# k-sheridan/ekf_vio

Hardware: AMD Instinct MI355X
Metric: filter steps/sec (predict+update) (higher is better)
Workload: dtype f32

## Files before the change

### ekf_vio_amd/capi.py

```python
import ctypes as C
import os

from . import _build

OK, EINVAL, ENUMERIC, ECAPACITY, EDEVICE, ESTATE, EABORTED = range(7)
_ERR = {EINVAL: "EKFVIO_EINVAL", ENUMERIC: "EKFVIO_ENUMERIC", ECAPACITY: "EKFVIO_ECAPACITY",
        EDEVICE: "EKFVIO_EDEVICE", ESTATE: "EKFVIO_ESTATE", EABORTED: "EKFVIO_EABORTED"}
PREDICT_STRUCTURED, PREDICT_DENSE = 0, 1


class Config(C.Structure):
    _fields_ = [("max_features", C.c_int32), ("default_point_depth", C.c_float),
                ("default_point_depth_variance", C.c_float), ("default_point_homogenous_variance", C.c_float),
                ("predict_mode", C.c_int32), ("klt_window_size", C.c_int32), ("klt_max_pyramid_level", C.c_int32),
                ("klt_max_iterations", C.c_int32), ("klt_epsilon", C.c_float), ("klt_min_eigen", C.c_float),
                ("kill_pad", C.c_int32), ("max_image_width", C.c_int32), ("max_image_height", C.c_int32),
                ("use_principal_point", C.c_int32), ("inverse_image_scale", C.c_int32), ("fast_threshold", C.c_int32),
                ("min_new_feature_dist", C.c_int32), ("fast_blur_sigma", C.c_float), ("replenish", C.c_int32),
                ("sample_based_uncertainty", C.c_int32), ("use_imu", C.c_int32), ("imu_gyro_variance", C.c_float),
                ("imu_accel_variance", C.c_float), ("gravity", C.c_float * 3),
                ("klt_fb_max_px", C.c_float), ("remove_lost", C.c_int32)]


class EkfvioError(RuntimeError):
    def __init__(self, code, msg=""):
        super().__init__("%s %s" % (_ERR.get(code, str(code)), msg))
        self.code = code


SYMBOLS = ["ekfvio_default_config", "ekfvio_create", "ekfvio_destroy", "ekfvio_reset", "ekfvio_last_error",
           "ekfvio_add_features", "ekfvio_process", "ekfvio_linearize", "ekfvio_update", "ekfvio_measurement_map",
           "ekfvio_num_features", "ekfvio_dim", "ekfvio_get_base_mu", "ekfvio_get_features", "ekfvio_get_sigma",
           "ekfvio_get_feature_cov", "ekfvio_get_depth_variance", "ekfvio_set_feature_cov", "ekfvio_metric2pixel_map",
           "ekfvio_pixel2metric_map", "ekfvio_get_odometry", "ekfvio_get_points", "ekfvio_check_sigma", "ekfvio_set_state",
           "ekfvio_remove_features", "ekfvio_klt_push_frame", "ekfvio_klt_track", "ekfvio_klt_track_points", "ekfvio_klt_get_level",
           "ekfvio_klt_uncertainty_points", "ekfvio_step_image", "ekfvio_replenish", "ekfvio_fast_detect", "ekfvio_imu", "ekfvio_imu_update",
           "ekfvio_upload_measurements", "ekfvio_run_uploaded", "ekfvio_synchronize", "ekfvio_profile_enable",
           "ekfvio_profile_reset", "ekfvio_profile_count", "ekfvio_profile_name", "ekfvio_profile_get",
           "ekfvio_profile_update_gemms", "ekfvio_get_counters", "ekfvio_set_gate", "ekfvio_get_gate",
           "ekfvio_set_klt_fb", "ekfvio_get_klt_fb", "ekfvio_klt_track_points_fb", "ekfvio_set_distortion", "ekfvio_rectify_map"]
HOOK_SYMBOLS = ["ekfvio_test_klt_padded_level", "ekfvio_test_blurred_level0", "ekfvio_test_gemm", "ekfvio_test_gemm_bench", "ekfvio_test_potrf_stamps",
                "ekfvio_test_sweep_stamps", "ekfvio_test_sweep_fault", "ekfvio_test_sweep_delay", "ekfvio_test_cholesky_solve", "ekfvio_test_plan", "ekfvio_test_persist_grid", "ekfvio_test_t2_pair"]

_libs = {}


def lib_path():
    return _build.LIB_PATH


def load(build_if_missing=True, hooks=False):
    if hooks in _libs:
        return _libs[hooks]
    path = _build.HOOKS_LIB_PATH if hooks else _build.LIB_PATH
    if build_if_missing:
        _build.build(hooks=hooks)
    elif not os.path.exists(path):
        raise FileNotFoundError(path + " not built; run python -m ekf_vio_amd._build")
    lib = C.CDLL(path)
    vp, i32, f32 = C.c_void_p, C.c_int32, C.c_float
    fp, u8p, ip = C.POINTER(C.c_float), C.POINTER(C.c_uint8), C.POINTER(C.c_int32)
    sig = {
        "ekfvio_default_config": [C.POINTER(Config)],
        "ekfvio_create": [C.POINTER(Config), C.c_int, vp, C.POINTER(vp)],
        "ekfvio_destroy": [vp], "ekfvio_reset": [vp],
        "ekfvio_add_features": [vp, fp, i32], "ekfvio_process": [vp, f32], "ekfvio_linearize": [vp, f32, fp],
        "ekfvio_update": [vp, fp, fp, u8p, i32], "ekfvio_measurement_map": [vp, u8p, i32, ip, ip],
        "ekfvio_num_features": [vp], "ekfvio_dim": [vp], "ekfvio_get_base_mu": [vp, fp],
        "ekfvio_get_features": [vp, fp, fp, u8p], "ekfvio_get_sigma": [vp, fp, i32],
        "ekfvio_get_feature_cov": [vp, i32, fp], "ekfvio_get_depth_variance": [vp, i32, fp],
        "ekfvio_set_feature_cov": [vp, i32, fp], "ekfvio_metric2pixel_map": [fp, fp], "ekfvio_pixel2metric_map": [fp, fp],
        "ekfvio_get_odometry": [vp, fp, fp, fp, fp], "ekfvio_get_points": [vp, fp, fp],
        "ekfvio_check_sigma": [vp, fp, fp], "ekfvio_set_state": [vp, i32, fp, fp, fp, u8p, fp, i32],
        "ekfvio_remove_features": [vp, u8p, i32, ip],
        "ekfvio_klt_push_frame": [vp, u8p, i32, i32, i32, fp], "ekfvio_klt_track": [vp, fp, fp, u8p],
        "ekfvio_klt_track_points": [vp, fp, fp, i32, fp, u8p],
        "ekfvio_klt_uncertainty_points": [vp, fp, fp, i32, fp],
        "ekfvio_klt_get_level": [vp, i32, ip, ip, u8p, C.POINTER(C.c_int16)],
        "ekfvio_step_image": [vp, C.c_double, u8p, i32, i32, i32, fp], "ekfvio_imu": [vp, C.c_double, fp, fp], "ekfvio_imu_update": [vp, fp, fp],
        "ekfvio_replenish": [vp, ip, ip], "ekfvio_fast_detect": [vp, i32, i32, i32, ip, ip, ip],
        "ekfvio_upload_measurements": [vp, i32, fp, fp, u8p], "ekfvio_run_uploaded": [vp, i32, i32, f32],
        "ekfvio_synchronize": [vp], "ekfvio_profile_enable": [vp, i32], "ekfvio_profile_reset": [vp],
        "ekfvio_profile_count": [], "ekfvio_profile_name": [i32],
        "ekfvio_profile_get": [vp, i32, C.POINTER(C.c_double), C.POINTER(C.c_int64), C.POINTER(C.c_double)],
        "ekfvio_profile_update_gemms": [vp, i32, C.POINTER(C.c_double), C.POINTER(C.c_double)],
        "ekfvio_get_counters": [vp, C.POINTER(C.c_int64)],
        "ekfvio_set_gate": [vp, f32], "ekfvio_get_gate": [vp, fp, u8p, ip, ip, C.POINTER(C.c_int64)],
        "ekfvio_set_klt_fb": [vp, f32], "ekfvio_get_klt_fb": [vp, fp, u8p, ip, ip, C.POINTER(C.c_int64)],
        "ekfvio_klt_track_points_fb": [vp, fp, fp, i32, fp, u8p, fp, fp, u8p],
        "ekfvio_set_distortion": [vp, C.POINTER(C.c_double), i32],
        "ekfvio_rectify_map": [fp, C.POINTER(C.c_double), i32, i32, i32, ip, ip],
    }
    if hooks:
        sig.update({
            "ekfvio_test_klt_padded_level": [vp, i32, ip, u8p, C.POINTER(C.c_int16)],
            "ekfvio_test_blurred_level0": [vp, u8p],
            "ekfvio_test_gemm": [vp, i32, i32, i32, i32, f32, fp, i32, fp, i32, f32, fp, i32, i32],
            "ekfvio_test_cholesky_solve": [vp, i32, i32, fp, fp, fp, fp, ip],
            "ekfvio_test_potrf_stamps": [vp, C.POINTER(C.c_int64)],
            "ekfvio_test_sweep_stamps": [vp, C.c_int, C.POINTER(C.c_int64)],
            "ekfvio_test_sweep_fault": [vp, i32, i32],
            "ekfvio_test_sweep_delay": [vp, i32, i32, i32],
            "ekfvio_test_gemm_bench": [vp, i32, i32, i32, i32, i32, i32, i32, C.POINTER(C.c_double)],
            "ekfvio_test_plan": [i32] * 8 + [f32, ip],
            "ekfvio_test_persist_grid": [i32] * 8 + [f32, ip, i32, ip],
            "ekfvio_test_t2_pair": [i32, ip],
        })
    for name, args in sig.items():
        fn = getattr(lib, name)
        fn.argtypes = args
        fn.restype = C.c_int
    lib.ekfvio_last_error.argtypes = [vp]
    lib.ekfvio_last_error.restype = C.c_char_p
    lib.ekfvio_profile_name.restype = C.c_char_p
    _libs[hooks] = lib
    return lib
```

### ekf_vio_amd/csrc/api.hip

```cpp
#include <math.h>
#include <stdio.h>
#include <string.h>

#include <algorithm>
#include <atomic>
#include <chrono>

#include <unistd.h>

#include "common.h"

#define HIPC(f, expr)                                                                              \
    do {                                                                                           \
        hipError_t e__ = (expr);                                                                   \
        if (e__ != hipSuccess) {                                                                   \
            (f)->last_error = std::string(#expr) + ": " + hipGetErrorString(e__);                  \
            return EKFVIO_EDEVICE;                                                                 \
        }                                                                                          \
    } while (0)

namespace {
template <class T>
hipError_t dev_alloc(hipStream_t s, T** p, size_t count) {
    hipError_t e = hipMalloc((void**)p, sizeof(T) * (count ? count : 1));
// ... 138 lines not shown
    c->imu_accel_variance = 1e-2f;
    c->gravity[0] = 0.f;
    c->gravity[1] = 9.81f;
    c->gravity[2] = 0.f;
    c->klt_fb_max_px = 0.f;
    c->remove_lost = 0;
    return EKFVIO_OK;
}

static int create_body(ekfvio_filter* f, const ekfvio_config* cfg, int device, void* stream) {
    HIPC(f, hipSetDevice(device));
    if (stream) {
        f->stream = (hipStream_t)stream;
    } else {
        HIPC(f, hipStreamCreateWithFlags(&f->stream, hipStreamNonBlocking));
        f->own_stream = true;
    }
    const int maxf = cfg->max_features;
    const FilterDims dims = filter_dims(maxf);
    f->n_cap = dims.n_cap, f->ldp = dims.ldp, f->m_cap = dims.m_cap, f->ld_aug = dims.ld_aug, f->sweep_sync_words = dims.sweep_sync_words;
    f->tune = tuning_from_env();
    const size_t pp = (size_t)f->ldp * f->ldp, pm = (size_t)f->ldp * f->m_cap;
    HIPC(f, dev_alloc(f->stream, &f->mu, f->ldp));
    HIPC(f, dev_alloc(f->stream, &f->mu_next, f->ldp));
    HIPC(f, dev_alloc(f->stream, &f->last_klt, 2 * (size_t)maxf));
    HIPC(f, dev_alloc(f->stream, &f->del_flag, (size_t)maxf));
    HIPC(f, dev_alloc(f->stream, &f->P, pp));
    HIPC(f, dev_alloc(f->stream, &f->P2, pp));
    HIPC(f, dev_alloc(f->stream, &f->FA, EKF_BASE * EKF_BASE));
    HIPC(f, dev_alloc(f->stream, &f->FB, 27 * (size_t)maxf));
    HIPC(f, dev_alloc(f->stream, &f->FD, 9 * (size_t)maxf));
    HIPC(f, dev_alloc(f->stream, &f->Fdense, pp));
    HIPC(f, dev_alloc(f->stream, &f->idx, (size_t)f->m_cap));
    HIPC(f, dev_alloc(f->stream, &f->inv_idx, (size_t)f->ldp));
    HIPC(f, dev_alloc(f->stream, &f->zmeas, 2 * (size_t)maxf));
    HIPC(f, dev_alloc(f->stream, &f->Rmeas, 4 * (size_t)maxf));
    HIPC(f, dev_alloc(f->stream, &f->pass, (size_t)maxf));
    HIPC(f, dev_alloc(f->stream, &f->yres, (size_t)f->m_cap));
    HIPC(f, dev_alloc(f->stream, &f->Rm, 2 * (size_t)f->m_cap));
    HIPC(f, dev_alloc(f->stream, &f->Saug, (size_t)f->ld_aug * f->m_cap));
    HIPC(f, dev_alloc(f->stream, &f->Laug, (size_t)f->ld_aug * f->m_cap));
    HIPC(f, dev_alloc(f->stream, &f->Linv, 64 * (size_t)f->m_cap));
    HIPC(f, dev_alloc(f->stream, &f->Lsign, (size_t)(f->m_cap / 64 > 256 ? f->m_cap / 64 : 256)));
    HIPC(f, dev_alloc(f->stream, &f->sweep_sync, f->sweep_sync_words));
    {
        hipDeviceProp_t prop;
        HIPC(f, hipGetDeviceProperties(&prop, device));
        f->num_cus = prop.multiProcessorCount;
    }
    HIPC(f, dev_alloc(f->stream, &f->Km, pm));
    HIPC(f, dev_alloc(f->stream, &f->Wt, pm));
    HIPC(f, dev_alloc(f->stream, &f->Gm, pm));
    HIPC(f, dev_alloc(f->stream, &f->info, 4));
    HIPC(f, dev_alloc(f->stream, &f->remove_words, 4));
    HIPC(f, hipHostMalloc((void**)&f->h_info, 16 * sizeof(int), hipHostMallocMapped | hipHostMallocCoherent));
    memset(f->h_info, 0, 16 * sizeof(int));
    HIPC(f, hipHostGetDevicePointer((void**)&f->d_hinfo, f->h_info, 0));
    {
        const size_t words = EKF_BASE + 4 * (size_t)(f->cfg.max_features > 0 ? f->cfg.max_features : 1);
        HIPC(f, hipHostMalloc((void**)&f->h_out, words * sizeof(float), hipHostMallocMapped | hipHostMallocCoherent));
        HIPC(f, hipHostGetDevicePointer((void**)&f->d_out, f->h_out, 0));
    }
    {
        const size_t cap = (size_t)(f->cfg.max_features > 0 ? f->cfg.max_features : 1);
        HIPC(f, hipHostMalloc((void**)&f->h_meas, 25 * cap, hipHostMallocDefault));
        HIPC(f, hipMalloc((void**)&f->d_meas, 25 * cap));
    }
    HIPC(f, hipEventCreate(&f->ev0));
    HIPC(f, hipEventCreate(&f->ev1));
    int rc = klt_alloc(f);
    if (rc != EKFVIO_OK) return rc;
    rc = fast_alloc(f);
    if (rc != EKFVIO_OK) return rc;
    return ekfvio_reset(f);
}

}

static std::atomic<int>* live_registry() {
    static std::atomic<int>* reg = [] {
        char name[64], val[32];
        snprintf(name, sizeof(name), "EKFVIO_LIVE_HANDLES_%ld", (long)getpid());
        if (const char* e = getenv(name)) {
            void* p = nullptr;
            if (sscanf(e, "%p", &p) == 1 && p) return static_cast<std::atomic<int>*>(p);
        }
        auto* a = new std::atomic<int>[64];
        for (int i = 0; i < 64; i++) a[i].store(0, std::memory_order_relaxed);
        snprintf(val, sizeof(val), "%p", static_cast<void*>(a));
        setenv(name, val, 1);
        return a;
    }();
    return reg;
}
int live_handles_on(int device) { return (device >= 0 && device < 64) ? live_registry()[device].load(std::memory_order_relaxed) : 2; }

extern "C" {

int ekfvio_create(const ekfvio_config* cfg, int device, void* stream, ekfvio_filter** out) {
    if (!out) return EKFVIO_EINVAL;
    *out = nullptr;
    if (!cfg || cfg->max_features < 0) return EKFVIO_EINVAL;
    if (cfg->remove_lost != 0 && cfg->remove_lost != 1) return EKFVIO_EINVAL;
    if (cfg->remove_lost && (size_t)cfg->max_features * 17 > 64 * 1024) return EKFVIO_ECAPACITY;
    if (!(cfg->klt_fb_max_px >= 0.f)) return EKFVIO_EINVAL;
    int ndev = 0;
    if (hipGetDeviceCount(&ndev) != hipSuccess || device < 0 || device >= ndev) return EKFVIO_EDEVICE;
    ekfvio_filter* f = new ekfvio_filter();
    f->cfg = *cfg;
    f->device = device;
    if (device < 64) live_registry()[device].fetch_add(1, std::memory_order_relaxed);
    const int rc = create_body(f, cfg, device, stream);
    if (rc != EKFVIO_OK) {
        fprintf(stderr, "ekfvio_create: %s\n", f->last_error.c_str());
        (void)ekfvio_destroy(f);
        return rc;
    }
    *out = f;
    return EKFVIO_OK;
}

int ekfvio_destroy(ekfvio_filter* f) {
    if (!f) return EKFVIO_EINVAL;
    (void)hipSetDevice(f->device);
    if (f->stream) (void)hipStreamSynchronize(f->stream);
    void* ptrs[] = {f->mu, f->mu_next, f->last_klt, f->del_flag, f->P,  f->P2, f->FA, f->FB, f->FD,   f->Fdense,
                    f->idx, f->inv_idx, f->zmeas,  f->Rmeas,    f->pass,     f->yres, f->Rm, f->Saug,  f->Laug,  f->Linv, f->Lsign, f->Km, f->sweep_sync, f->sweep_dbg,
                    f->Wt,  f->Gm,     f->info,     f->remove_words, f->seq_z,    f->seq_R, f->seq_pass, f->gate_words, f->fb_words};
    for (void* p : ptrs)
        if (p) hipFree(p);
    if (f->h_info) hipHostFree(f->h_info);
    if (f->h_out) hipHostFree(f->h_out);
    if (f->h_meas) hipHostFree(f->h_meas);
    if (f->d_meas) (void)hipFree(f->d_meas);
    klt_free(f);
    fast_free(f);
    drop_graph(f);
    if (f->ev0) hipEventDestroy(f->ev0);
    if (f->ev1) hipEventDestroy(f->ev1);
    if (f->own_stream && f->stream) hipStreamDestroy(f->stream);
    if (f->device >= 0 && f->device < 64) live_registry()[f->device].fetch_sub(1, std::memory_order_relaxed);
    delete f;
    return EKFVIO_OK;
}

const char* ekfvio_last_error(const ekfvio_filter* f) {
    return f ? f->last_error.c_str() : "null handle (a failed ekfvio_create leaves none behind: its return code says why)";
}

int ekfvio_reset(ekfvio_filter* f) {
    if (!f) return EKFVIO_EINVAL;
    f->out_fresh = false;
    HIPC(f, hipSetDevice(f->device));
    f->N = 0;
    f->n = EKF_BASE;
    HIPC(f, hipMemsetAsync(f->P, 0, sizeof(float) * (size_t)f->ldp * f->ldp, f->stream));
    HIPC(f, hipMemsetAsync(f->P2, 0, sizeof(float) * (size_t)f->ldp * f->ldp, f->stream));
    HIPC(f, hipMemsetAsync(f->mu, 0, sizeof(float) * f->ldp, f->stream));
    const float one = 1.f;
    HIPC(f, hipMemcpyAsync(f->mu + 3, &one, sizeof(float), hipMemcpyHostToDevice, f->stream));
    hipLaunchKernelGGL(init_sigma_kernel, dim3(1), dim3(32), 0, f->stream, f->P, f->ldp);
    HIPC(f, hipMemsetAsync(f->info, 0, 4 * sizeof(int), f->stream));
    if (f->gate_words) HIPC(f, hipMemsetAsync(f->gate_words, 0, 4 * sizeof(int), f->stream));
    if (f->fb_words) HIPC(f, hipMemsetAsync(f->fb_words, 0, 8 * sizeof(int), f->stream));
    HIPC(f, hipStreamSynchronize(f->stream));
    f->have_stamp = false;
    f->frames[0].valid = f->frames[1].valid = false;
    return EKFVIO_OK;
}

int ekfvio_add_features(ekfvio_filter* f, const float* uv, int32_t count) {
    if (!f || count < 0 || (count > 0 && !uv)) return EKFVIO_EINVAL;
    f->out_fresh = false;
    if (count == 0) return EKFVIO_OK;
    if (f->N + count > f->cfg.max_features) return EKFVIO_ECAPACITY;
    HIPC(f, hipSetDevice(f->device));
    HIPC(f, hipMemcpyAsync(f->zmeas, uv, sizeof(float) * 2 * count, hipMemcpyHostToDevice, f->stream));
    return add_features_device(f, count);
}

int ekfvio_process(ekfvio_filter* f, float dt) {
// ... 270 lines not shown

int ekfvio_upload_measurements(ekfvio_filter* f, int32_t frames, const float* z, const float* R, const uint8_t* pass) {
    if (!f || frames <= 0 || !z || !R || !pass || f->N <= 0) return EKFVIO_EINVAL;
    HIPC(f, hipSetDevice(f->device));
    HIPC(f, hipStreamSynchronize(f->stream));
    drop_graph(f);
    if (f->seq_z) hipFree(f->seq_z);
    if (f->seq_R) hipFree(f->seq_R);
    if (f->seq_pass) hipFree(f->seq_pass);
    f->seq_z = f->seq_R = nullptr;
    f->seq_pass = nullptr;
    const size_t N = f->N;
    HIPC(f, dev_alloc(f->stream, &f->seq_z, frames * 2 * N));
    HIPC(f, dev_alloc(f->stream, &f->seq_R, frames * 4 * N));
    HIPC(f, dev_alloc(f->stream, &f->seq_pass, frames * N));
    HIPC(f, hipMemcpyAsync(f->seq_z, z, sizeof(float) * frames * 2 * N, hipMemcpyHostToDevice, f->stream));
    HIPC(f, hipMemcpyAsync(f->seq_R, R, sizeof(float) * frames * 4 * N, hipMemcpyHostToDevice, f->stream));
    HIPC(f, hipMemcpyAsync(f->seq_pass, pass, frames * N, hipMemcpyHostToDevice, f->stream));
    HIPC(f, hipStreamSynchronize(f->stream));
    f->seq_frames = frames;
    f->seq_N = (int)N;
    f->seq_m.resize(frames);
    for (int i = 0; i < frames; i++) f->seq_m[i] = count_rows(pass + (size_t)i * N, (int)N);
    return EKFVIO_OK;
}

#ifndef EKF_GRAPH_STEPS
#define EKF_GRAPH_STEPS 8
#endif
#define EKF_GRAPH_STEPS_BIG 32

static void drop_graph(ekfvio_filter* f) {
    if (f->step_graph) {
        (void)hipGraphExecDestroy(f->step_graph);
        f->step_graph = nullptr;
    }
    if (f->step_graph_big) {
        (void)hipGraphExecDestroy(f->step_graph_big);
        f->step_graph_big = nullptr;
    }
    if (f->step_graph_pair) {
        (void)hipGraphExecDestroy(f->step_graph_pair);
        f->step_graph_pair = nullptr;
    }
}

static UpdateInputs uploaded_update(ekfvio_filter* f, int m, int i, int* counter) {
    UpdateInputs in;
    in.m = m, in.z = f->seq_z + (size_t)i * 2 * f->N, in.R = f->seq_R + (size_t)i * 4 * f->N, in.pass = f->seq_pass + (size_t)i * f->N;
    in.frame_counter = counter, in.frames = counter ? f->seq_frames : 0;
    in.recoverable = false;
    return in;
}
static int capture_steps(ekfvio_filter* f, int steps, int m, float dt, int* counter, hipGraphExec_t* out, int* pre_out) {
    hipGraph_t g = nullptr;
    HIPC(f, hipStreamSynchronize(f->stream));
    const bool mirror = f->sweep_flags_clean;
    f->sweep_flags_clean = false;
    const long long pre0 = f->prelinearized_steps;
    HIPC(f, hipStreamBeginCapture(f->stream, hipStreamCaptureModeThreadLocal));
    const bool gate = f->gate_chi2 > 0.f;
    for (int k = 0; k < steps; k++) {
        const BookArgs bk = make_book_args(f, m, f->seq_z, f->seq_R, f->seq_pass, counter);
        launch_predict(f, dt, gate ? nullptr : &bk);
        UpdateInputs in = uploaded_update(f, m, 0, counter);
        in.bookkeeping_done = !gate;
        in.next_dt = (k + 1 < steps) ? dt : -1.f;
        launch_update(f, in);
    }
    f->prelinearized = false;
    *pre_out = (int)(f->prelinearized_steps - pre0);
    f->prelinearized_steps = pre0;
    hipError_t ce = hipStreamEndCapture(f->stream, &g);
    f->graph_leaves_flags_clean = f->sweep_flags_clean;
    f->sweep_flags_clean = mirror;
    if (ce != hipSuccess || !g) {
        f->last_error = std::string("graph capture: ") + hipGetErrorString(ce);
        return EKFVIO_EDEVICE;
    }
    HIPC(f, hipGraphInstantiate(out, g, nullptr, nullptr, 0));
    (void)hipGraphDestroy(g);
    return EKFVIO_OK;
}

int ekfvio_run_uploaded(ekfvio_filter* f, int32_t first, int32_t count, float dt) {
    if (!f || f->seq_frames <= 0 || f->seq_N != f->N || count < 0 || first < 0 || !(dt >= 0.f)) return EKFVIO_EINVAL;
    f->out_fresh = false;
    HIPC(f, hipSetDevice(f->device));
    int s = 0;
    const bool gate = f->gate_chi2 > 0.f;
    auto geometry = [&](int i) { return gate && f->seq_m[i] > 0 ? 2 * f->N : f->seq_m[i]; };
    bool uniform = !f->prof_on && (count >= 2 || count == 0);
    for (int i = 0; uniform && i < f->seq_frames; i++) uniform = geometry(i) == geometry(0);
    if (uniform) {
        const int m = geometry(0);
        int* counter = f->info + 1;
        HIPC(f, hipMemsetD32Async((hipDeviceptr_t)counter, first % f->seq_frames, 1, f->stream));
        if (!f->step_graph || f->graph_N != f->N || f->graph_m != m || f->graph_dt != dt || f->graph_mu != f->mu || f->graph_P != f->P ||
            f->graph_seq != f->seq_z || f->graph_frames != f->seq_frames || f->graph_sole != (live_handles_on(f->device) <= 1)) {
            drop_graph(f);
            int rc = capture_steps(f, EKF_GRAPH_STEPS, m, dt, counter, &f->step_graph, &f->graph_pre);
            if (rc != EKFVIO_OK) return rc;
            rc = capture_steps(f, 2, m, dt, counter, &f->step_graph_pair, &f->graph_pre_pair);
            if (rc != EKFVIO_OK) return rc;
            f->graph_N = f->N; f->graph_m = m; f->graph_dt = dt; f->graph_mu = f->mu; f->graph_P = f->P; f->graph_seq = f->seq_z;
            f->graph_frames = f->seq_frames;
            f->graph_sole = live_handles_on(f->device) <= 1;
        }
        if (f->seq_frames >= 2 * EKF_GRAPH_STEPS_BIG && !f->step_graph_big) {
            int rc = capture_steps(f, EKF_GRAPH_STEPS_BIG, m, dt, counter, &f->step_graph_big, &f->graph_pre_big);
            if (rc != EKFVIO_OK) return rc;
        }
        auto replay = [&](hipGraphExec_t g, int steps, int pre) {
            const hipError_t e = hipGraphLaunch(g, f->stream);
            if (e == hipSuccess) s += steps, f->graph_steps += steps, f->prelinearized_steps += pre;
            return e;
        };
        if (f->step_graph_big)
            while (s + EKF_GRAPH_STEPS_BIG <= count) HIPC(f, replay(f->step_graph_big, EKF_GRAPH_STEPS_BIG, f->graph_pre_big));
        while (s + EKF_GRAPH_STEPS <= count) HIPC(f, replay(f->step_graph, EKF_GRAPH_STEPS, f->graph_pre));
        while (s + 2 <= count) HIPC(f, replay(f->step_graph_pair, 2, f->graph_pre_pair));
        if (s > 0) f->sweep_flags_clean = f->graph_leaves_flags_clean;
        for (; s < count; s++) {
            launch_predict(f, dt);
            launch_update(f, uploaded_update(f, m, 0, counter));
        }
        HIPC(f, hipGetLastError());
        return EKFVIO_OK;
    }
    for (; s < count; s++) {
        const int i = (first + s) % f->seq_frames;
        launch_predict(f, dt);
        launch_update(f, uploaded_update(f, f->seq_m[i], i, nullptr));
    }
    HIPC(f, hipGetLastError());
    return EKFVIO_OK;
}

int ekfvio_synchronize(ekfvio_filter* f) {
    if (!f) return EKFVIO_EINVAL;
    HIPC(f, hipSetDevice(f->device));
    return finish_update(f);
}

int ekfvio_profile_enable(ekfvio_filter* f, int32_t on) {
    if (!f) return EKFVIO_EINVAL;
    hipStreamSynchronize(f->stream);
    f->prof_on = on != 0;
    if (f->prof_on) {
        double acc = 0;
        const int reps = 32;
        for (int i = 0; i < reps + 4; i++) {
            (void)hipEventRecord(f->ev0, f->stream);
            (void)hipEventRecord(f->ev1, f->stream);
            (void)hipEventSynchronize(f->ev1);
            float ms = 0;
            (void)hipEventElapsedTime(&ms, f->ev0, f->ev1);
            if (i >= 4) acc += ms;
        }
        f->prof_overhead_ms = (float)(acc / reps);
    }
    return EKFVIO_OK;
}
int ekfvio_profile_update_gemms(ekfvio_filter* f, int32_t reps, double* avg_launch_us, double* flops_per_launch) {
    if (!f || reps <= 0 || !avg_launch_us) return EKFVIO_EINVAL;
    if (f->last_m <= 0 || f->N <= 0) return EKFVIO_ESTATE;
    HIPC(f, hipSetDevice(f->device));
    HIPC(f, hipStreamSynchronize(f->stream));
    hipGraph_t g = nullptr;
    hipGraphExec_t ge = nullptr;
    HIPC(f, hipStreamBeginCapture(f->stream, hipStreamCaptureModeThreadLocal));
    const int per_rep = launch_update_gemms_scratch(f, plan_update(f, f->last_m), reps);
    hipError_t ce = hipStreamEndCapture(f->stream, &g);
    if (ce != hipSuccess || !g) {
        f->last_error = std::string("graph capture: ") + hipGetErrorString(ce);
        return EKFVIO_EDEVICE;
    }
    HIPC(f, hipGraphInstantiate(&ge, g, nullptr, nullptr, 0));
    (void)hipGraphDestroy(g);
    HIPC(f, hipGraphLaunch(ge, f->stream));
    HIPC(f, hipEventRecord(f->ev0, f->stream));
    HIPC(f, hipGraphLaunch(ge, f->stream));
    HIPC(f, hipEventRecord(f->ev1, f->stream));
    HIPC(f, hipEventSynchronize(f->ev1));
    float ms = 0;
    HIPC(f, hipEventElapsedTime(&ms, f->ev0, f->ev1));
// ... 49 lines not shown
    int w[4] = {0, 0, 0, 0};
    if (f->gate_words) {
        HIPC(f, hipMemcpyAsync(w, f->gate_words, sizeof(w), hipMemcpyDeviceToHost, f->stream));
        HIPC(f, hipStreamSynchronize(f->stream));
    }
    const int seen = std::min(std::max(w[1], 0), f->cfg.max_features);
    if (seen > 0) {
        if (d2) HIPC(f, hipMemcpyAsync(d2, f->gate_d2, sizeof(float) * seen, hipMemcpyDeviceToHost, f->stream));
        if (gated) HIPC(f, hipMemcpyAsync(gated, f->gate_flag, seen, hipMemcpyDeviceToHost, f->stream));
        HIPC(f, hipStreamSynchronize(f->stream));
    }
    if (n_landmarks) *n_landmarks = seen;
    if (gated_last) *gated_last = w[0];
    if (gated_total) memcpy(gated_total, w + 2, sizeof(int64_t));
    return EKFVIO_OK;
}

int ekfvio_set_klt_fb(ekfvio_filter* f, float max_px) {
    if (!f || !(max_px >= 0.f)) return EKFVIO_EINVAL;
    f->cfg.klt_fb_max_px = max_px;
    return EKFVIO_OK;
}

int ekfvio_get_klt_fb(ekfvio_filter* f, float* err2, uint8_t* rejected, int32_t* n_landmarks, int32_t* rejected_last, int64_t* rejected_total) {
    if (!f) return EKFVIO_EINVAL;
    HIPC(f, hipSetDevice(f->device));
    int w[4] = {0, 0, 0, 0};
    if (f->fb_words) {
        HIPC(f, hipMemcpyAsync(w, f->fb_words, sizeof(w), hipMemcpyDeviceToHost, f->stream));
        HIPC(f, hipStreamSynchronize(f->stream));
    }
    const int seen = std::min(std::max(w[1], 0), f->cfg.max_features);
    if (seen > 0) {
        if (err2) HIPC(f, hipMemcpyAsync(err2, f->fb_err2, sizeof(float) * seen, hipMemcpyDeviceToHost, f->stream));
        if (rejected) HIPC(f, hipMemcpyAsync(rejected, f->fb_flag, seen, hipMemcpyDeviceToHost, f->stream));
        HIPC(f, hipStreamSynchronize(f->stream));
    }
    if (n_landmarks) *n_landmarks = seen;
    if (rejected_last) *rejected_last = w[0];
    if (rejected_total) memcpy(rejected_total, w + 2, sizeof(int64_t));
    return EKFVIO_OK;
}

int ekfvio_get_counters(ekfvio_filter* f, int64_t counters[8]) {
    if (!f || !counters) return EKFVIO_EINVAL;
    counters[0] = f->persistent_sweeps;
    counters[1] = f->schur_sweeps;
    counters[2] = f->sweep_recoveries;
    counters[3] = (f->tune.persist_sweep && !f->sweep_latched_off) ? 2 : 0;
    counters[4] = f->early_output_frames;
    counters[5] = f->t2_updates;
    counters[6] = f->graph_steps;
    counters[7] = f->prelinearized_steps;
    return EKFVIO_OK;
}

#ifdef EKFVIO_TEST_HOOKS
int ekfvio_test_gemm(ekfvio_filter* f, int32_t transB, int32_t M, int32_t N, int32_t K, float alpha, const float* A,
                     int32_t lda, const float* B, int32_t ldb, float beta, float* C, int32_t ldc, int32_t variant) {
    if (!f || M <= 0 || N <= 0 || K <= 0 || !A || !B || !C) return EKFVIO_EINVAL;
    HIPC(f, hipSetDevice(f->device));
    const int Mp = round_up(M, 64), Np = round_up(N, 64), Kp = round_up(K, 64);
    const int brows = transB ? Np : Kp, bcols = transB ? Kp : Np;
    std::vector<float> hA((size_t)Mp * Kp, 0.f), hB((size_t)brows * bcols, 0.f), hC((size_t)Mp * Np, 0.f);
    for (int k = 0; k < K; k++)
        for (int i = 0; i < M; i++) hA[(size_t)k * Mp + i] = A[(size_t)k * lda + i];
    for (int c = 0; c < (transB ? K : N); c++)
        for (int r = 0; r < (transB ? N : K); r++) hB[(size_t)c * brows + r] = B[(size_t)c * ldb + r];
    for (int j = 0; j < N; j++)
        for (int i = 0; i < M; i++) hC[(size_t)j * Mp + i] = C[(size_t)j * ldc + i];
    float *dA, *dB, *dC;
    HIPC(f, dev_alloc(f->stream, &dA, hA.size()));
    HIPC(f, dev_alloc(f->stream, &dB, hB.size()));
    HIPC(f, dev_alloc(f->stream, &dC, hC.size()));
    HIPC(f, hipMemcpyAsync(dA, hA.data(), sizeof(float) * hA.size(), hipMemcpyHostToDevice, f->stream));
    HIPC(f, hipMemcpyAsync(dB, hB.data(), sizeof(float) * hB.size(), hipMemcpyHostToDevice, f->stream));
    HIPC(f, hipMemcpyAsync(dC, hC.data(), sizeof(float) * hC.size(), hipMemcpyHostToDevice, f->stream));
    launch_gemm_variant(f, variant, transB, M, N, Kp, alpha, dA, Mp, dB, brows, beta, dC, Mp, dC, Mp, 0, 0);
    HIPC(f, hipMemcpyAsync(hC.data(), dC, sizeof(float) * hC.size(), hipMemcpyDeviceToHost, f->stream));
    HIPC(f, hipStreamSynchronize(f->stream));
    for (int j = 0; j < N; j++)
        for (int i = 0; i < M; i++) C[(size_t)j * ldc + i] = hC[(size_t)j * Mp + i];
    hipFree(dA);
    hipFree(dB);
    hipFree(dC);
    return EKFVIO_OK;
}

int ekfvio_test_gemm_bench(ekfvio_filter* f, int32_t transB, int32_t lowerB, int32_t M, int32_t N, int32_t K,
                           int32_t reps, int32_t variant, double* mean_us) {
    if (!f || M <= 0 || N <= 0 || K <= 0 || reps <= 0 || !mean_us) return EKFVIO_EINVAL;
    HIPC(f, hipSetDevice(f->device));
    const int Mp = round_up(M, 128), Np = round_up(N, 128), Kp = round_up(K, 64);
    const int brows = transB ? Np : Kp, bcols = transB ? Kp : Np;
    std::vector<float> hA((size_t)Mp * Kp), hB((size_t)brows * bcols), hC((size_t)Mp * Np);
    uint32_t st = 12345u;
    auto rnd = [&]() { st = st * 1664525u + 1013904223u; return ((st >> 8) & 0xffff) / 32768.0f - 1.0f; };
    for (auto& v : hA) v = rnd();
    for (auto& v : hB) v = rnd();
    for (auto& v : hC) v = rnd();
    float *dA, *dB, *dC;
    HIPC(f, dev_alloc(f->stream, &dA, hA.size()));
    HIPC(f, dev_alloc(f->stream, &dB, hB.size()));
    HIPC(f, dev_alloc(f->stream, &dC, hC.size()));
    HIPC(f, hipMemcpyAsync(dA, hA.data(), sizeof(float) * hA.size(), hipMemcpyHostToDevice, f->stream));
    HIPC(f, hipMemcpyAsync(dB, hB.data(), sizeof(float) * hB.size(), hipMemcpyHostToDevice, f->stream));
// ... 111 lines not shown
    UpdatePlan plan = plan_raw_sweep(f->tune, plan_shape(f), mp, rp);
    launch_chol_sweep(f, plan, dS, dL, dLi, ld, plan.persistent() && !f->sweep_flags_clean);
    if (plan.persistent()) f->sweep_flags_clean = false;
    std::vector<unsigned long long> hsign(mp / 64);
    HIPC(f, hipMemcpyAsync(hsign.data(), f->Lsign, sizeof(unsigned long long) * hsign.size(), hipMemcpyDeviceToHost, f->stream));
    HIPC(f, hipStreamSynchronize(f->stream));
    int refine = 1;
    for (unsigned long long v : hsign) refine &= (v == 0ull);
    if (refine) plan.gain = GAIN_GEMM;
    launch_gain_from_sweep(f, plan, dL, ld, nrhs, dK, dW, rp, refine);
    std::vector<float> hl(hs.size()), hk((size_t)rp * mp);
    HIPC(f, hipMemcpyAsync(hl.data(), dL, sizeof(float) * hl.size(), hipMemcpyDeviceToHost, f->stream));
    HIPC(f, hipMemcpyAsync(hk.data(), dK, sizeof(float) * hk.size(), hipMemcpyDeviceToHost, f->stream));
    if (info) {
        HIPC(f, hipMemcpyAsync(info, f->info, sizeof(int), hipMemcpyDeviceToHost, f->stream));
        HIPC(f, hipMemsetAsync(f->info, 0, sizeof(int), f->stream));
    }
    HIPC(f, hipStreamSynchronize(f->stream));
    if (const char* dp = getenv("EKFVIO_DEBUG_DUMP_LAUG")) {
        if (FILE* fp = fopen(dp, "wb")) {
            const int hdr[3] = {ld, mp, rp};
            fwrite(hdr, sizeof(int), 3, fp);
            fwrite(hl.data(), sizeof(float), hl.size(), fp);
            fclose(fp);
        }
    }
    if (L_out)
        for (int c = 0; c < m; c++)
            for (int r = 0; r < m; r++) L_out[(size_t)c * m + r] = (r >= c) ? hl[(size_t)c * ld + r] : 0.f;
    if (X_out)
        for (int c = 0; c < m; c++)
            for (int r = 0; r < nrhs; r++) X_out[(size_t)c * nrhs + r] = hk[(size_t)c * rp + r];
    hipFree(dS);
    hipFree(dL);
    hipFree(dLi);
    hipFree(dK);
    hipFree(dW);
    return EKFVIO_OK;
}

int ekfvio_test_plan(int32_t num_cus, int32_t max_features, int32_t N, int32_t m, int32_t m_on_device, int32_t sole_handle,
                     int32_t latched_off, int32_t dense_predict, float next_dt, int32_t plan[12]) {
    if (!plan || max_features < 0 || N < 0 || N > max_features) return EKFVIO_EINVAL;
    const FilterDims d = filter_dims(max_features);
    PlanShape s;
    s.num_cus = num_cus, s.ldp = d.ldp, s.sweep_sync_words = d.sweep_sync_words, s.N = N, s.n = EKF_BASE + 3 * N;
    s.dense_predict = dense_predict != 0, s.sole_handle = sole_handle != 0, s.latched_off = latched_off != 0;
    const UpdatePlan p = plan_update(tuning_from_env(), s, m, m_on_device != 0, next_dt);
    const int32_t out[12] = {p.m, p.m_pad, p.n_pad, p.sweep, p.fused_gather, p.with_wt, p.gain, p.tail, p.t2_skip, p.t2_by_sweep, p.compact, p.lin_blocks};
    std::copy(out, out + 12, plan);
    return EKFVIO_OK;
}

int ekfvio_test_persist_grid(int32_t num_cus, int32_t max_features, int32_t N, int32_t m, int32_t m_on_device, int32_t sole_handle,
                             int32_t latched_off, int32_t dense_predict, float next_dt, int32_t* roles, int32_t max_blocks, int32_t out[10]) {
    if (!out || max_features < 0 || N < 0 || N > max_features) return EKFVIO_EINVAL;
    const FilterDims d = filter_dims(max_features);
    PlanShape s;
    s.num_cus = num_cus, s.ldp = d.ldp, s.sweep_sync_words = d.sweep_sync_words, s.N = N, s.n = EKF_BASE + 3 * N;
    s.dense_predict = dense_predict != 0, s.sole_handle = sole_handle != 0, s.latched_off = latched_off != 0;
    const UpdatePlan p = plan_update(tuning_from_env(), s, m, m_on_device != 0, next_dt);
    std::fill(out, out + 10, 0);
    if (!p.persistent()) return EKFVIO_OK;
    const PersistGrid g = persist_grid(p, d.ldp);
    const PersistFlags fl(p.m_pad, p.n_pad);
    const int32_t res[10] = {g.total(), g.kind, g.owners(), fl.ready(), fl.fin(), fl.pan(), fl.abort_word(), (int32_t)fl.words(), fl.zero_words(),
                             (int32_t)d.sweep_sync_words};
    std::copy(res, res + 10, out);
    if (!roles) return EKFVIO_OK;
    if (max_blocks < g.total()) return EKFVIO_ECAPACITY;
    for (int b = 0; b < g.total(); b++) {
        const PersistRole r = g.role(b);
        roles[4 * b] = r.kind, roles[4 * b + 1] = r.a, roles[4 * b + 2] = r.b;
        roles[4 * b + 3] = r.kind == ROLE_OWNER ? g.owner_block(r.n) : -1;
    }
    return EKFVIO_OK;
}
int ekfvio_test_t2_pair(int32_t p, int32_t pair[2]) {
    if (p < 0 || !pair) return EKFVIO_EINVAL;
    int ta, tb;
    t2_pair(p, ta, tb);
    pair[0] = ta, pair[1] = tb;
    return EKFVIO_OK;
}
#endif

}
```

### ekf_vio_amd/csrc/chol.hip

```cpp
#include "common.h"

#include <type_traits>

namespace {

typedef float f32x16 __attribute__((ext_vector_type(16)));
typedef float f32x4 __attribute__((ext_vector_type(4)));

#define PB 64
#ifndef PLD
#define PLD 68
#endif
#define ILD 17
#define INV_LDS (4 * 16 * ILD)

__device__ __forceinline__ float lane_bcast(float v, int src_lane) {
    return __int_as_float(__builtin_amdgcn_readlane(__float_as_int(v), src_lane));
}
__device__ __forceinline__ double lane_bcast_d(double v, int src_lane) {
    const int lo = __builtin_amdgcn_readlane(__double2loint(v), src_lane);
    const int hi = __builtin_amdgcn_readlane(__double2hiint(v), src_lane);
    return __hiloint2double(hi, lo);
}

template <int B, int E, class F>
__device__ __forceinline__ void static_for(F&& f) {
    if constexpr (B < E) {
        f(std::integral_constant<int, B>{});
        static_for<B + 1, E>(f);
    }
}
template <int R>
__device__ __forceinline__ void dpp_fnma(float& acc, float a, float b) {
    asm volatile("v_fmac_f32_dpp %0, -%1, %2 row_newbcast:%3 row_mask:0xf bank_mask:0xf" : "+v"(acc) : "v"(a), "v"(b), "n"(R));
}
template <int R>
__device__ __forceinline__ float dpp_mul(float a, float b) {
    float r;
    asm volatile("s_nop 1\n\tv_mul_f32_dpp %0, %1, %2 row_newbcast:%3 row_mask:0xf bank_mask:0xf" : "=v"(r) : "v"(a), "v"(b), "n"(R));
    return r;
}

__device__ __forceinline__ void load_tile(float* T, const float* __restrict__ G, int ld, int tid) {
#pragma unroll
    for (int it = 0; it < 4; it++) {
        const int e = tid + it * 256;
        const int c = e >> 4, r4 = (e & 15) * 4;
        const float4 v = *reinterpret_cast<const float4*>(G + (size_t)c * ld + r4);
        float* t = T + c * PLD + r4;
#if PLD % 4 == 0
        *reinterpret_cast<float4*>(t) = v;
#else
        t[0] = v.x; t[1] = v.y; t[2] = v.z; t[3] = v.w;
#endif
    }
}
__device__ __forceinline__ void store_tile(const float* T, float* __restrict__ G, int ld, int tid) {
#pragma unroll
    for (int it = 0; it < 4; it++) {
        const int e = tid + it * 256;
        const int c = e >> 4, r4 = (e & 15) * 4;
        const float* t = T + c * PLD + r4;
#if PLD % 4 == 0
        *reinterpret_cast<float4*>(G + (size_t)c * ld + r4) = *reinterpret_cast<const float4*>(t);
#else
        *reinterpret_cast<float4*>(G + (size_t)c * ld + r4) = make_float4(t[0], t[1], t[2], t[3]);
#endif
    }
}
__device__ __forceinline__ unsigned long long sign_mask_request(const unsigned long long* p) {
    unsigned z;
    asm volatile("v_mov_b32 %0, 0" : "=v"(z));
    return p[z];
}
__device__ __forceinline__ unsigned long long sign_mask_value(unsigned long long v) {
    const unsigned lo = __builtin_amdgcn_readfirstlane((unsigned)v), hi = __builtin_amdgcn_readfirstlane((unsigned)(v >> 32));
    return ((unsigned long long)hi << 32) | lo;
}
__device__ __forceinline__ void store_tile_signed(const float* T, float* __restrict__ G, int ld, int tid, unsigned long long neg) {
#pragma unroll
    for (int it = 0; it < 4; it++) {
        const int e = tid + it * 256;
        const int c = e >> 4, r4 = (e & 15) * 4;
        const float* t = T + c * PLD + r4;
        const float sg = ((neg >> c) & 1ull) ? -1.f : 1.f;
        *reinterpret_cast<float4*>(G + (size_t)c * ld + r4) = make_float4(sg * t[0], sg * t[1], sg * t[2], sg * t[3]);
    }
}
__device__ __forceinline__ void store_tile_lower(const float* T, float* __restrict__ G, int ld, int tid) {
#pragma unroll
    for (int it = 0; it < 4; it++) {
        const int e = tid + it * 256;
        const int c = e >> 4, r4 = (e & 15) * 4;
        const float* t = T + c * PLD + r4;
#if PLD % 4 == 0
        const float4 q = *reinterpret_cast<const float4*>(t);
        *reinterpret_cast<float4*>(G + (size_t)c * ld + r4) =
            make_float4(r4 >= c ? q.x : 0.f, r4 + 1 >= c ? q.y : 0.f, r4 + 2 >= c ? q.z : 0.f, r4 + 3 >= c ? q.w : 0.f);
#else
        *reinterpret_cast<float4*>(G + (size_t)c * ld + r4) =
            make_float4(r4 >= c ? t[0] : 0.f, r4 + 1 >= c ? t[1] : 0.f, r4 + 2 >= c ? t[2] : 0.f, r4 + 3 >= c ? t[3] : 0.f);
#endif
    }
}
template <int C0, int NC, int NT, bool LOWER>
__device__ __forceinline__ void store_cols(const float* T, float* __restrict__ G, int ld, int t) {
    static_assert(PLD % 4 == 0, "vector LDS reads");
#pragma unroll
    for (int it = 0; it < (NC * 16 + NT - 1) / NT; it++) {
        const int e = t + it * NT;
        if ((NC * 16) % NT != 0 && e >= NC * 16) break;
        const int c = C0 + (e >> 4), r4 = (e & 15) * 4;
        const float4 q = *reinterpret_cast<const float4*>(T + c * PLD + r4);
        *reinterpret_cast<float4*>(G + (size_t)c * ld + r4) =
            LOWER ? make_float4(r4 >= c ? q.x : 0.f, r4 + 1 >= c ? q.y : 0.f, r4 + 2 >= c ? q.z : 0.f, r4 + 3 >= c ? q.w : 0.f) : q;
    }
}
__device__ __forceinline__ void store_inv_blocks(const float* Tinv, float* __restrict__ G, int p0, int t) {
    const int p = p0 + (t >> 6), c = (t >> 2) & 15, r4 = (t & 3) * 4;
    const float* s = Tinv + p * 16 * ILD + c * ILD + r4;
    *reinterpret_cast<float4*>(G + (p0 * 64 + t) * 4) = make_float4(s[0], s[1], s[2], s[3]);
}
struct NoIdleWork {
    template <class PC>
    __device__ __forceinline__ void operator()(PC, int) const {}
};
__device__ __forceinline__ void load_inv(float* Tinv, const float* __restrict__ G, int tid) {
    const float4 v = *reinterpret_cast<const float4*>(G + tid * 4);
    const int p = tid >> 6, c = (tid >> 2) & 15, r4 = (tid & 3) * 4;
    float* t = Tinv + p * 16 * ILD + c * ILD + r4;
    t[0] = v.x; t[1] = v.y; t[2] = v.z; t[3] = v.w;
}
__device__ __forceinline__ void store_inv(const float* Tinv, float* __restrict__ G, int tid) {
    const int p = tid >> 6, c = (tid >> 2) & 15, r4 = (tid & 3) * 4;
    const float* t = Tinv + p * 16 * ILD + c * ILD + r4;
    *reinterpret_cast<float4*>(G + tid * 4) = make_float4(t[0], t[1], t[2], t[3]);
}

__device__ __forceinline__ f32x16 mma64(const float* As, int a_si, int a_sq, const float* Bs, int b_sj, int b_sq, int wr, int wc,
                               int lane) {
    f32x16 acc;
#pragma unroll
    for (int r = 0; r < 16; r++) acc[r] = 0.f;
    const int li = lane & 31, lk = lane >> 5;
    const float* ap = As + (wr * 32 + li) * a_si + lk * a_sq;
    const float* bp = Bs + (wc * 32 + li) * b_sj + lk * b_sq;
#pragma unroll
    for (int q = 0; q < PB; q += 2) {
        const float a = ap[q * a_sq];
        const float b = bp[q * b_sq];
        acc = __builtin_amdgcn_mfma_f32_32x32x2f32(b, a, acc, 0, 0, 0);
    }
    return acc;
}
__device__ __forceinline__ int mma64_col(int wc, int lane, int reg) { return wc * 32 + (reg & 3) + 8 * (reg >> 2) + 4 * (lane >> 5); }
__device__ __attribute__((noinline)) f32x16 mma64_signed(const float* As, int a_si, int a_sq, const float* Bs, int b_sj, int b_sq, int wr,
                                                         int wc, int lane, unsigned long long neg) {
    f32x16 acc;
#pragma unroll
    for (int r = 0; r < 16; r++) acc[r] = 0.f;
    const int li = lane & 31, lk = lane >> 5;
    const float* ap = As + (wr * 32 + li) * a_si + lk * a_sq;
    const float* bp = Bs + (wc * 32 + li) * b_sj + lk * b_sq;
#pragma unroll 8
    for (int q = 0; q < PB; q += 2) {
        float a = ap[q * a_sq];
        if ((neg >> (q + lk)) & 1ull) a = -a;
        const float b = bp[q * b_sq];
        acc = __builtin_amdgcn_mfma_f32_32x32x2f32(b, a, acc, 0, 0, 0);
    }
    return acc;
}

__device__ __forceinline__ f32x4 mma16(const float* As, int a_si, int a_sq, const float* Bs, int b_sj, int b_sq, int lane) {
    f32x4 acc = {0.f, 0.f, 0.f, 0.f};
    const int li = lane & 15, lk = lane >> 4;
    const float* ap = As + li * a_si + lk * a_sq;
    const float* bp = Bs + li * b_sj + lk * b_sq;
#pragma unroll
    for (int q = 0; q < 16; q += 4) acc = __builtin_amdgcn_mfma_f32_16x16x4f32(bp[q * b_sq], ap[q * a_sq], acc, 0, 0, 0);
    return acc;
}

struct TriOps {
    float binv[4][4];
    float nl[6][4];
};
__device__ __forceinline__ void tri_solve_preload(TriOps& o, const float* Tl, const float* Tinv, int lane) {
    const int li = lane & 15, g = lane >> 4;
#pragma unroll
    for (int p = 0; p < 4; p++)
#pragma unroll
        for (int v = 0; v < 4; v++) o.binv[p][v] = Tinv[p * 16 * ILD + (4 * g + v) * ILD + li];
    {
        int e = 0;
#pragma unroll
        for (int p = 0; p < 3; p++)
#pragma unroll
            for (int t = p + 1; t < 4; t++, e++)
#pragma unroll
                for (int v = 0; v < 4; v++) o.nl[e][v] = -Tl[(16 * p + 4 * g + v) * PLD + 16 * t + li];
    }
}
__device__ __forceinline__ void tri_solve_pin(TriOps& o) {
#pragma unroll
    for (int p = 0; p < 4; p++)
#pragma unroll
        for (int v = 0; v < 4; v++) asm volatile("" : "+v"(o.binv[p][v]));
#pragma unroll
    for (int q = 0; q < 6; q++)
#pragma unroll
        for (int v = 0; v < 4; v++) asm volatile("" : "+v"(o.nl[q][v]));
}
template <int NT>
__device__ __forceinline__ void tri_solve_load_x(f32x4 (&x)[NT][4], float* const (&Txs)[NT], int wave, int lane) {
    const int r0 = 16 * wave, li = lane & 15, g = lane >> 4;
#pragma unroll
    for (int n = 0; n < NT; n++)
#pragma unroll
        for (int b = 0; b < 4; b++)
#pragma unroll
            for (int v = 0; v < 4; v++) x[n][b][v] = Txs[n][(16 * b + 4 * g + v) * PLD + r0 + li];
}
template <int NT>
__device__ __forceinline__ void tri_solve_run(f32x4 (&x)[NT][4], float* const (&Txs)[NT], const TriOps& o, int wave, int lane) {
    const int r0 = 16 * wave, li = lane & 15, g = lane >> 4;
    int e0 = 0;
#pragma unroll
    for (int p = 0; p < 4; p++) {
        f32x4 y[NT];
#pragma unroll
        for (int n = 0; n < NT; n++) y[n] = f32x4{0.f, 0.f, 0.f, 0.f};
#pragma unroll
        for (int v = 0; v < 4; v++)
#pragma unroll
// ... 40 lines not shown
#pragma unroll
        for (int p = 0; p < 3; p++)
#pragma unroll
            for (int t = p + 1; t < 4; t++, e++)
#pragma unroll
                for (int v = 0; v < 4; v++) nl[e][v] = -Tl[(16 * p + 4 * g + v) * PLD + 16 * t + li];
    }
#pragma unroll
    for (int p = 0; p < 4; p++)
#pragma unroll
        for (int v = 0; v < 4; v++) asm volatile("" : "+v"(binv[p][v]));
#pragma unroll
    for (int q = 0; q < 6; q++)
#pragma unroll
        for (int v = 0; v < 4; v++) asm volatile("" : "+v"(nl[q][v]));
    TSTAMP(1);
    int e0 = 0;
#pragma unroll
    for (int p = 0; p < 4; p++) {
        f32x4 y[NT];
#pragma unroll
        for (int n = 0; n < NT; n++) y[n] = f32x4{0.f, 0.f, 0.f, 0.f};
#pragma unroll
        for (int v = 0; v < 4; v++)
#pragma unroll
            for (int n = 0; n < NT; n++) y[n] = __builtin_amdgcn_mfma_f32_16x16x4f32(binv[p][v], x[n][p][v], y[n], 0, 0, 0);
#pragma unroll
        for (int n = 0; n < NT; n++) x[n][p] = y[n];
        int e = e0;
#pragma unroll
        for (int t = p + 1; t < 4; t++, e++)
#pragma unroll
            for (int v = 0; v < 4; v++)
#pragma unroll
                for (int n = 0; n < NT; n++) x[n][t] = __builtin_amdgcn_mfma_f32_16x16x4f32(nl[e][v], y[n][v], x[n][t], 0, 0, 0);
        e0 = e;
    }
    TSTAMP(2);
#pragma unroll
    for (int n = 0; n < NT; n++)
#pragma unroll
        for (int b = 0; b < 4; b++)
#pragma unroll
            for (int v = 0; v < 4; v++) Txs[n][(16 * b + 4 * g + v) * PLD + r0 + li] = x[n][b][v];
    TSTAMP(3);
}
__device__ __forceinline__ void tri_solve_fwd(float* Tx, const float* Tl, const float* Tinv, int wave, int lane, long long* st = nullptr) {
    float* const t[1] = {Tx};
    tri_solve_fwd_n<1>(t, Tl, Tinv, wave, lane, st);
}
__device__ __forceinline__ void tri_solve_fwd2(float* Tx, float* Ty, const float* Tl, const float* Tinv, int wave, int lane) {
    float* const t[2] = {Tx, Ty};
    tri_solve_fwd_n<2>(t, Tl, Tinv, wave, lane);
}
#define POTRF_STAMP(i)                                                         \
    do {                                                                       \
        if (stamps && tid == 0) stamps[i] = (long long)__builtin_amdgcn_s_memtime(); \
    } while (0)

#define POTRF_WSTAMP(i)                                                                               \
    do {                                                                                              \
        if (stamps && lane == 0) stamps[16 + wave * 16 + (i)] = (long long)__builtin_amdgcn_s_memtime(); \
    } while (0)

__device__ __forceinline__ void potrf_tile_update(float* A, int c0, int ti, int tj, int lane) {
    const int li = lane & 15, lk = lane >> 4;
    const int rb = c0 + 16 + 16 * ti, cb = c0 + 16 + 16 * tj;
    const f32x4 u = mma16(A + c0 * PLD + rb, 1, PLD, A + c0 * PLD + cb, 1, PLD, lane);
    float t[4];
#pragma unroll
    for (int g = 0; g < 4; g++) t[g] = A[(cb + 4 * lk + g) * PLD + rb + li];
#pragma unroll
    for (int g = 0; g < 4; g++) A[(cb + 4 * lk + g) * PLD + rb + li] = t[g] - u[g];
}

__device__ __forceinline__ void potrf_inverse16(const float* A, float* Tinv, int b, int lane) {
    const int o = 16 * b, li = lane & 15;
    float lrow[16], acc[16], x[16];
#pragma unroll
    for (int q = 0; q < 16; q++) lrow[q] = A[(o + q) * PLD + o + li];
    const float dd = A[(o + li) * PLD + o + li];
    float dinv_own = __builtin_amdgcn_rcpf(dd);
    dinv_own = __builtin_fmaf(__builtin_fmaf(-dd, dinv_own, 1.f), dinv_own, dinv_own);
#pragma unroll
    for (int r = 0; r < 16; r++) acc[r] = (r == li) ? 1.f : 0.f;
    static_for<0, 16>([&](auto qc) {
        constexpr int q = decltype(qc)::value;
        const float xq = dpp_mul<q>(dinv_own, acc[q]);
        x[q] = xq;
        static_for<q + 1, 16>([&](auto rc) {
            constexpr int r = decltype(rc)::value;
            dpp_fnma<r>(acc[r], lrow[q], xq);
        });
    });
    if (lane < 16) {
#pragma unroll
        for (int r = 0; r < 16; r++) Tinv[b * 16 * ILD + li * ILD + r] = x[r];
    }
}

#include "potrf_chain.inc"

template <int FV = EKF_POTRF_FV, class Idle = NoIdleWork, bool RAW_BARRIER = false>
__device__ __forceinline__ bool potrf64_lds(float* A, float* Tinv, int tid, long long* stamps = nullptr, Idle idle = Idle()) {
#define POTRF_BAR()                                                                                  \
    do {                                                                                             \
        if constexpr (RAW_BARRIER) asm volatile("s_waitcnt lgkmcnt(0)\n\ts_barrier" ::: "memory");   \
        else __syncthreads();                                                                        \
    } while (0)
    const int lane = tid & 63;
    const int wave = tid >> 6;
    bool bad = false;
    POTRF_STAMP(1);
    static_for<0, 4>([&](auto pc) {
        constexpr int P = decltype(pc)::value;
        constexpr int p = P;
        constexpr int c0 = 16 * p;
        if (FV >= 10 && wave == 0) {
            const unsigned lb = static_cast<unsigned>(reinterpret_cast<size_t>(A + c0 * PLD + lane));
            const bool inv_lane = p >= 1 && lane < 16;
            const unsigned sb = inv_lane ? static_cast<unsigned>(reinterpret_cast<size_t>(Tinv + p * 16 * ILD + lane * ILD)) : lb;
            if constexpr (FV == 12) potrf_panel16_chain_ls3<c0>(lb, sb, inv_lane ? 4u : (unsigned)(PLD * 4), (c0 + (lane & 15)) << 2);
            else if constexpr (FV == 13) potrf_panel16_chain_ls3w<c0>(lb, sb, inv_lane ? 4u : (unsigned)(PLD * 4), (c0 + (lane & 15)) << 2);
            else potrf_panel16_chain_ls<c0>(lb, sb, inv_lane ? 4u : (unsigned)(PLD * 4), (c0 + (lane & 15)) << 2);
        } else if (wave == 0) {
            float a[16];
#pragma unroll
            for (int j = 0; j < 16; j++) a[j] = A[(c0 + j) * PLD + lane];
#pragma unroll
            for (int j = 0; j < 16; j++) asm volatile("" : "+v"(a[j]));
            if (stamps && p == 0 && lane == 0) stamps[14] = (long long)__builtin_amdgcn_s_memtime();
            if constexpr (FV == 8) {
                potrf_panel16_chain<c0>(a, (c0 + (lane & 15)) << 2);
            } else {
                static_for<0, 16>([&](auto kc) {
                    constexpr int k = decltype(kc)::value;
                    const float d = lane_bcast(fmaxf(a[k], 1e-20f), c0 + k);
                    const float inv = __builtin_amdgcn_rsqf(d);
                    a[k] *= inv;
                    static_for<k + 1, 16>([&](auto jc) {
                        constexpr int j = decltype(jc)::value;
                        a[j] = __builtin_fmaf(-a[k], lane_bcast(a[k], c0 + j), a[j]);
                    });
                });
            }
            if (stamps && p == 0 && lane == 0) stamps[15] = (long long)__builtin_amdgcn_s_memtime();
            if (lane >= c0) {
#pragma unroll
                for (int j = 0; j < 16; j++) A[(c0 + j) * PLD + lane] = (lane - c0 >= j) ? a[j] : 0.f;
            }
            if constexpr (p >= 1) {
                if (lane < 16) {
#pragma unroll
                    for (int j = 0; j < 16; j++) Tinv[p * 16 * ILD + lane * ILD + j] = a[j];
                }
            }
        } else if (p == 0) {
#pragma unroll
            for (int q = 0; q < 4; q++) {
                const int e = (tid - 64) + 192 * q;
                const int c = 16 + (e >> 4), r = e & 15;
                A[c * PLD + r] = ((c & 15) == r) ? 1.f : 0.f;
            }
        } else if (p == 1) {
            if (wave == 1) potrf_inverse16(A, Tinv, 0, lane);
            if (wave == 2) potrf_tile_update(A, 0, 1, 1, lane);
            if (wave == 3) {
                potrf_tile_update(A, 0, 2, 1, lane);
                potrf_tile_update(A, 0, 2, 2, lane);
            }
        } else if (p == 2) {
            if (wave == 1) potrf_tile_update(A, 16, 1, 1, lane);
        }
        if (wave != 0) idle(pc, wave);
        POTRF_WSTAMP(2 * p);
        POTRF_BAR();
        POTRF_STAMP(2 + 2 * p);
        if (p < 3) {
            if (wave < 3 - p) potrf_tile_update(A, c0, wave, 0, lane);
            POTRF_WSTAMP(2 * p + 1);
            POTRF_BAR();
        }
        POTRF_STAMP(3 + 2 * p);
    });
    POTRF_STAMP(10);
    bad = __ballot(!(A[lane * PLD + lane] > 2e-10f)) != 0ull;
    return bad;
#undef POTRF_BAR
}

__device__ __attribute__((noinline)) unsigned long long potrf64_signed(float* A, float* Tinv, int tid) {
    const int lane = tid & 63, wave = tid >> 6;
    __syncthreads();
    if (wave == 0) {
        for (int k = 0; k < PB; k++) {
            const float d = A[k * PLD + k];
            const float inv = __builtin_amdgcn_rsqf(fmaxf(fabsf(d), 1e-20f));
            const float u = (lane >= k) ? A[k * PLD + lane] * inv : 0.f;
            if (lane >= k) A[k * PLD + lane] = u;
            const float su = (d < 0.f) ? -u : u;
            for (int j = k + 1; j < PB; j++) {
                const float uj = lane_bcast(u, j);
                if (lane >= j) A[j * PLD + lane] = __builtin_fmaf(-su, uj, A[j * PLD + lane]);
            }
        }
    }
    __syncthreads();
    const unsigned long long neg = __ballot(A[lane * PLD + lane] < 0.f);
    potrf_inverse16(A, Tinv, wave, lane);
    __syncthreads();
    return neg;
}

#ifdef EKFVIO_TEST_HOOKS
template <int FV>
__global__ __launch_bounds__(256) void potrf64_stamp_kernel(const float* __restrict__ S, int lds, float* __restrict__ L,
                                                            int ldl, float* __restrict__ Linv, long long* stamps, int passes) {
    __shared__ __attribute__((aligned(16))) float A[PB * PLD];
    __shared__ float Tinv[INV_LDS];
    const int tid = threadIdx.x;
#pragma unroll 1
    for (int pass = 0; pass < passes; pass++) {
        __syncthreads();
        if (tid == 0) stamps[0] = (long long)__builtin_amdgcn_s_memtime();
        load_tile(A, S, lds, tid);
        __syncthreads();
        potrf64_lds<FV>(A, Tinv, tid, stamps);
        store_tile_lower(A, L, ldl, tid);
        store_inv(Tinv, Linv, tid);
        __syncthreads();
        if (tid == 0) stamps[11] = (long long)__builtin_amdgcn_s_memtime();
    }
}
#endif

__global__ __launch_bounds__(256) void potrf64_kernel(const float* __restrict__ S, int lds, float* __restrict__ L,
                                                      int ldl, float* __restrict__ Linv, int* info, unsigned long long* Lsign) {
    __shared__ __attribute__((aligned(16))) float A[PB * PLD];
    __shared__ float Tinv[INV_LDS];
    const int tid = threadIdx.x;
    load_tile(A, S, lds, tid);
// ... 354 lines not shown
#ifdef EKFVIO_TEST_HOOKS
void launch_potrf_stamps(ekfvio_filter* f, const float* S, int ld, float* L, float* Linv, long long* d_stamps) {
    const char* e = getenv("EKFVIO_POTRF_FV");
    const int fv = e ? atoi(e) : EKF_POTRF_FV;
    auto kern = fv == 0 ? potrf64_stamp_kernel<0> : fv == 10 ? potrf64_stamp_kernel<10> : fv == 12 ? potrf64_stamp_kernel<12>
              : fv == 13 ? potrf64_stamp_kernel<13> : potrf64_stamp_kernel<8>;
    const char* w = getenv("EKFVIO_POTRF_WARM");
    hipLaunchKernelGGL(kern, dim3(1), dim3(256), 0, f->stream, S, ld, L, ld, Linv, d_stamps, (w && atoi(w)) ? 2 : 1);
}
#endif

#define EKF_GATHER_POTRF_LDS (84 * 1024)
void launch_gather_potrf(ekfvio_filter* f, const UpdatePlan& p) {
    if (!f->gather_attr_set) {
        (void)hipFuncSetAttribute(reinterpret_cast<const void*>(gather_potrf_kernel), hipFuncAttributeMaxDynamicSharedMemorySize,
                                  EKF_GATHER_POTRF_LDS);
        f->gather_attr_set = true;
    }
    GatherArgs ga = make_gather_args(f, p);
    if (p.persistent()) {
        ga.zero_words = f->sweep_sync;
        ga.n_zero = (int)persist_flag_words(p.m_pad, p.n_pad);
    }
    const int nb2 = p.with_wt ? (p.m_pad / 64) * (f->ldp / 64) : 0;
    hipLaunchKernelGGL(gather_potrf_kernel, dim3(1 + ga.nb1 + nb2), dim3(256), EKF_GATHER_POTRF_LDS, f->stream, ga, f->Laug, f->ld_aug,
                       f->Linv, f->info, f->Lsign, f->sweep_dbg);
}

static PersistArgs persist_args(ekfvio_filter* f, const UpdatePlan& p, float* L, int ldl, float* K, int ldk, float* S = nullptr,
                                float* Linv = nullptr) {
    PersistArgs pa = PersistArgs();
    const PersistGrid g = persist_grid(p, f->ldp);
    const PersistFlags fl(p.m_pad, p.n_pad);
    const int mb = g.mb, nX = g.nX;
    pa.L = L, pa.ldl = ldl, pa.mb = mb, pa.idb0 = mb + nX, pa.grid = g;
    pa.K = K, pa.ldk = ldk, pa.Lsign = f->Lsign;
    pa.Sg = f->P, pa.ldsg = f->ldp, pa.T2 = t2_buffer(f), pa.ldt = f->ldp, pa.nstate = f->n;
    if (!S) return pa;
    pa.S = S, pa.lds = ldl, pa.Linv = Linv, pa.info = f->info;
    pa.ready = f->sweep_sync + fl.ready(), pa.fin = f->sweep_sync + fl.fin(), pa.pan = f->sweep_sync + fl.pan(), pa.abort_flag = f->sweep_sync + fl.abort_word();
    pa.dbg = f->sweep_dbg;
    pa.bound.spin_limit = f->sweep_spin_limit > 0 ? f->sweep_spin_limit : SWEEP_SPIN_LIMIT;
    pa.bound.wait_ticks = p.recoverable ? f->tune.sweep_wait_ticks : std::max(f->tune.sweep_wait_ticks, SWEEP_WAIT_TICKS_UNRECOVERABLE);
    pa.early_sources = f->tune.persist_early;
    pa.stall_wg = f->sweep_stall_wg >= 0 ? g.owner_block(f->sweep_stall_wg - 1) : -1;
#ifdef EKFVIO_TEST_HOOKS
    pa.delay_wg = f->sweep_delay_wg >= 0 ? g.owner_block(f->sweep_delay_wg - 1) : -1;
    pa.delay_point = f->sweep_delay_point, pa.delay_ticks = f->sweep_delay_ticks;
#endif
    return pa;
}

#define EKF_PERSIST_FUSED_DYN_LDS (28 * 1024)
const int* launch_persist_fused(ekfvio_filter* f, const UpdatePlan& p, bool zero_flags) {
    const int m_pad = p.m_pad, n_pad = p.n_pad;
    ProfScope ps(f, PC_CHOL, (double)m_pad * m_pad * m_pad / 3.0 + (double)(n_pad + m_pad / 2) * m_pad * m_pad);
    if (!f->persist_attr_set) {
        (void)hipFuncSetAttribute(reinterpret_cast<const void*>(chol_persist_kernel), hipFuncAttributeMaxDynamicSharedMemorySize,
                                  EKF_PERSIST_FUSED_DYN_LDS);
        f->persist_attr_set = true;
    }
    PersistArgs pa = persist_args(f, p, f->Laug, f->ld_aug, f->Km, f->ldp, f->Saug, f->Linv);
    pa.gain = p.gain == GAIN_SWEEP, pa.t2 = p.t2_by_sweep;
    if (zero_flags) (void)hipMemsetAsync(f->sweep_sync, 0, sizeof(int) * persist_flag_words(m_pad, n_pad), f->stream);
    hipLaunchKernelGGL(chol_persist_kernel, dim3(pa.grid.total()), dim3(256), EKF_PERSIST_FUSED_DYN_LDS,
                       f->stream, pa, make_gather_args(f, p));
    f->persistent_sweeps++;
    return pa.abort_flag;
}

const int* launch_chol_sweep(ekfvio_filter* f, const UpdatePlan& p, float* Saug, float* Laug, float* Linv, int ld, bool zero_flags) {
    const int m_pad = p.m_pad, n_pad = p.n_pad;
    const bool schur = p.sweep == SWEEP_SCHUR, split = p.sweep == SWEEP_SPLIT || p.sweep == SWEEP_SPLIT_LA;
    ProfScope ps(f, PC_CHOL, (double)m_pad * m_pad * m_pad / 3.0 + (double)(n_pad + m_pad / 2) * m_pad * m_pad +
                                 (schur ? (double)n_pad * n_pad * m_pad + (double)n_pad * m_pad * m_pad : 0.0));
    const int mb = m_pad / PB, idb0 = mb + n_pad / PB;
    const int rb = n_pad / PB + mb;
    if (!p.fused_gather)
        hipLaunchKernelGGL(potrf64_kernel, dim3(1), dim3(256), 0, f->stream, Saug, ld, Laug, ld, Linv, f->info, f->Lsign);
    if (p.sweep == SWEEP_PERSIST) {
        const PersistArgs pa = persist_args(f, p, Laug, ld, nullptr, 0, Saug, Linv);
        if (zero_flags) (void)hipMemsetAsync(f->sweep_sync, 0, sizeof(int) * persist_flag_words(m_pad, n_pad), f->stream);
        hipLaunchKernelGGL(chol_persist_kernel, dim3(pa.grid.total()), dim3(256), 0, f->stream, pa, GatherArgs());
        f->persistent_sweeps++;
        return pa.abort_flag;
    }
    SchurArgs sc;
    if (schur) {
        f->schur_sweeps++;
        sc.P = f->P, sc.ldp = f->ldp, sc.K = f->Km, sc.ldk = f->ldp, sc.nb = n_pad / PB;
        const int nT = sc.nb * (sc.nb + 1) / 2;
        for (int k = 0; k < mb; k++) {
            const int r = mb - 1 - k;
            const dim3 grid(r * (r + 1) / 2 + rb * r + nT + sc.nb * (k + 1));
            hipLaunchKernelGGL((chol_step_kernel<true, true>), grid, dim3(256), 0, f->stream, Saug, ld, Laug, ld, Linv, k, mb, idb0,
                               f->info, f->Lsign, f->sweep_dbg, sc);
        }
        return nullptr;
    }
    if (p.sweep == SWEEP_SPLIT_LA) {
        LaArgs la;
        la.S = Saug, la.lds = ld, la.L = Laug, la.ldl = ld, la.Linv = Linv;
        la.mb = mb, la.rb = rb, la.idb0 = idb0, la.info = f->info, la.Lsign = f->Lsign;
        {
            for (int l = 0; l + 1 < mb; l++) {
                const int grid = la_near_tasks(mb, idb0, rb, l) + la_far_tasks(mb, idb0, rb, l);
                hipLaunchKernelGGL(chol_step_la_kernel, dim3(grid), dim3(256), 0, f->stream, la, l);
            }
        }
        hipLaunchKernelGGL(chol_panel_kernel, dim3(rb), dim3(256), 0, f->stream, Saug, ld, Laug, ld, Linv, mb - 1, mb, 0, idb0, f->Lsign, 0);
        hipLaunchKernelGGL(sign_irows_kernel, dim3((m_pad + 255) / 256, mb), dim3(256), 0, f->stream, Laug, ld, idb0 * PB, m_pad,
                           f->Lsign);
        return nullptr;
    }
    for (int k = 0; k + 1 < mb; k++) {
        const int r = mb - 1 - k;
// ... 106 lines not shown
```

### ekf_vio_amd/csrc/chol_persist.inc

```

#ifndef PERSIST_POLL_SLEEP_LAZY
#define PERSIST_POLL_SLEEP_LAZY 12
#endif
#ifndef PERSIST_POLL_SLEEP
#define PERSIST_POLL_SLEEP 2
#endif

struct PollBound {
    int spin_limit, wait_ticks;
};
struct PersistArgs {
    float* S;
    int lds;
    float* L;
    int ldl;
    float* Linv;
    int mb, idb0;
    int* info;
    unsigned long long* Lsign;
    int* ready;
    int* fin;
    int* abort_flag;
    long long* dbg;
    PersistGrid grid;
    int gain;
    float* K;
    int ldk;
    int* pan;
    int early_sources;
    PollBound bound;
    int stall_wg;
    int t2;
    const float* Sg;
    int ldsg;
    float* T2;
    int ldt;
    int nstate;
#ifdef EKFVIO_TEST_HOOKS
    int delay_wg;
    int delay_point;
    int delay_ticks;
#endif
};

typedef unsigned int u32x4 __attribute__((ext_vector_type(4)));
__device__ __forceinline__ __amdgpu_buffer_rsrc_t persist_rsrc(const float* p, unsigned floats) {
    return __builtin_amdgcn_make_buffer_rsrc(const_cast<float*>(p), 0, floats * 4u, 0x00020000);
}
__device__ __forceinline__ float4 ld_sc1(__amdgpu_buffer_rsrc_t b, unsigned off) {
    const f32x4 v = __builtin_bit_cast(f32x4, __builtin_amdgcn_raw_buffer_load_b128(b, off * 4u, 0, 16));
    return make_float4(v[0], v[1], v[2], v[3]);
}
__device__ __forceinline__ void st_sc1(__amdgpu_buffer_rsrc_t b, unsigned off, float4 q) {
    const f32x4 v = {q.x, q.y, q.z, q.w};
    __builtin_amdgcn_raw_buffer_store_b128(__builtin_bit_cast(u32x4, v), b, off * 4u, 0, 16);
}
__device__ __forceinline__ void wait_vm0() { asm volatile("s_waitcnt vmcnt(0)" ::: "memory"); }

struct RegTile {
    float4 v[4];
    __device__ __forceinline__ void request(__amdgpu_buffer_rsrc_t b, unsigned base, int ld, int tid) {
#pragma unroll
        for (int it = 0; it < 4; it++) {
            const int e = tid + it * 256;
            v[it] = ld_sc1(b, base + (unsigned)(e >> 4) * (unsigned)ld + (unsigned)(e & 15) * 4u);
        }
    }
    __device__ __forceinline__ void put(float* T, int tid) const {
#pragma unroll
        for (int it = 0; it < 4; it++) {
            const int e = tid + it * 256;
            *reinterpret_cast<float4*>(T + (e >> 4) * PLD + (e & 15) * 4) = v[it];
        }
    }
};
__device__ __forceinline__ void inv_put(float4 v, float* Tinv, int tid) {
    const int p = tid >> 6, c = (tid >> 2) & 15, r4 = (tid & 3) * 4;
    float* t = Tinv + p * 16 * ILD + c * ILD + r4;
    t[0] = v.x; t[1] = v.y; t[2] = v.z; t[3] = v.w;
}
__device__ __forceinline__ void load_tile_sc1(float* T, __amdgpu_buffer_rsrc_t b, unsigned base, int ld, int tid) {
    RegTile t;
    t.request(b, base, ld, tid);
    t.put(T, tid);
}
__device__ __forceinline__ void load_inv_sc1(float* Tinv, __amdgpu_buffer_rsrc_t b, unsigned base, int tid) {
    inv_put(ld_sc1(b, base + tid * 4), Tinv, tid);
}
template <bool LOWER>
__device__ __forceinline__ void store_tile_sc1(const float* T, __amdgpu_buffer_rsrc_t b, unsigned base, int ld, int tid) {
// ... 564 lines not shown
    for (int q = 0; q < 16; q++) off[q] = (base + (unsigned)(16 * (q >> 2) + 4 * g + (q & 3)) * (unsigned)ld + (unsigned)(16 * wave + li)) * 4u;
#pragma unroll
    for (int q = 0; q < 16; q++) asm volatile("" : "+v"(off[q]));
#pragma unroll
    for (int q = 0; q < 16; q++) x[q >> 2][q & 3] = __builtin_bit_cast(float, __builtin_amdgcn_raw_buffer_load_b32(b, off[q], 0, 16));
}

__global__ __launch_bounds__(256) void chol_persist_kernel(PersistArgs a, GatherArgs ga) {
    extern __shared__ __attribute__((aligned(16))) float persist_dyn_lds[];
    __shared__ __attribute__((aligned(16))) float Ti[PB * PLD];
    __shared__ __attribute__((aligned(16))) float Tj[PB * PLD];
    __shared__ __attribute__((aligned(16))) float Tl[PB * PLD];
    __shared__ float Tinv[INV_LDS];
    const int tid = threadIdx.x, lane = tid & 63, wave = tid >> 6;
    const int wr = wave & 1, wc = wave >> 1;
    const int r = wr * 32 + (lane & 31);
    const int mb = a.mb, lds = a.lds, ldl = a.ldl;
    const bool fused = a.grid.fused(), compact = a.grid.compact();
    const PersistRole role = a.grid.role((int)blockIdx.x);
    float* S = a.S;
    float* L = a.L;
    const __amdgpu_buffer_rsrc_t bS = persist_rsrc(S, (unsigned)lds * (unsigned)(mb * PB));
    const __amdgpu_buffer_rsrc_t bL = persist_rsrc(L, (unsigned)ldl * (unsigned)(mb * PB));
    const __amdgpu_buffer_rsrc_t bI = persist_rsrc(a.Linv, (unsigned)(mb * PB * PB));
#define PSTAMP(slot)                                                                               \
    do {                                                                                           \
        if (a.dbg && tid == 0) a.dbg[(slot)] = (long long)__builtin_amdgcn_s_memtime();            \
    } while (0)

#define PEXIT()                                                                                                         \
    do {                                                                                                                \
        if (a.dbg && tid == 0) {                                                                                        \
            const unsigned long long t_ = __builtin_amdgcn_s_memrealtime();                                             \
            if (atomicMax(reinterpret_cast<unsigned long long*>(a.dbg + 898), t_) < t_) a.dbg[899] = (long long)blockIdx.x; \
        }                                                                                                               \
        return;                                                                                                         \
    } while (0)
    if (a.dbg && tid == 0 && blockIdx.x >= 252 && blockIdx.x < 268) {
        a.dbg[160 + blockIdx.x - 252] = (long long)__builtin_amdgcn_s_memrealtime();
        unsigned xcc;
        asm volatile("s_getreg_b32 %0, hwreg(HW_REG_XCC_ID)" : "=s"(xcc));
        a.dbg[176 + blockIdx.x - 252] = (long long)(xcc & 15);
    }
    if (role.kind == ROLE_CHAIN) {
        PSTAMP(0);
        if (a.dbg && tid == 0) a.dbg[896] = (long long)__builtin_amdgcn_s_memrealtime();
        float* Lk = Tl;
        float* Dn = Tj;
        unsigned long long neg;
        if (fused) {
            unsigned zoff = 0;
            asm volatile("" : "+v"(zoff));
            const int m = ga.m_dev ? ga.m_dev[zoff] : ga.m;
            {
                GTile t0;
                int all_hit = 0;
                {
                    const int c0 = tid & 63;
                    const int gib = EKF_BASE + 3 * (c0 >> 1) + (c0 & 1);
                    t0.ib = ga.idx[c0];
                    bool hit = true;
#pragma unroll
                    for (int ps = 0; ps < 16; ps++) {
                        const int r0 = (tid >> 6) + 4 * ps;
                        t0.ia[ps] = ga.idx[r0];
                        t0.rd[ps] = ga.Rm[2 * r0];
                        t0.ro[ps] = ga.Rm[2 * r0 + 1];
                        t0.v[ps] = ga.P[(size_t)(EKF_BASE + 3 * (r0 >> 1) + (r0 & 1)) * ga.ld + gib];
                    }
#pragma unroll
                    for (int ps = 0; ps < 16; ps++) {
                        const int r0 = (tid >> 6) + 4 * ps;
                        hit = hit && t0.ia[ps] == EKF_BASE + 3 * (r0 >> 1) + (r0 & 1);
                    }
                    hit = hit && t0.ib == gib && m >= PB;
                    all_hit = __syncthreads_and(hit);
                }
                if (a.dbg && tid == 0) a.dbg[900] = all_hit;
                if (!all_hit) {
                    gtile_idx(t0, ga, m, 0, 0, mb, a.idb0, tid);
                    gtile_pin(t0);
                    gtile_val(t0, ga, m, 0, 0, mb, a.idb0, tid);
                    gtile_pinv(t0);
                }
                gtile_put(t0, Lk, ga, m, 0, 0, mb, a.idb0, tid);
            }
            __syncthreads();
            PSTAMP(1);
            const bool bad0 = potrf64_lds<EKF_POTRF_FV>(Lk, Tinv, tid);
            neg = 0ull;
            if (bad0) {
                __syncthreads();
                GTile t0;
                gtile_idx(t0, ga, m, 0, 0, mb, a.idb0, tid);
                gtile_val(t0, ga, m, 0, 0, mb, a.idb0, tid);
                gtile_put(t0, Lk, ga, m, 0, 0, mb, a.idb0, tid);
                neg = potrf64_signed(Lk, Tinv, tid);
            }
            PSTAMP(2);
            store_tile_sc1<true>(Lk, bL, 0u, ldl, tid);
            store_inv_sc1(Tinv, bI, 0u, tid);
            if (tid == 0) {
                __hip_atomic_store(a.Lsign, neg, __ATOMIC_RELAXED, __HIP_MEMORY_SCOPE_AGENT);
                if (bad0) atomicOr(a.info, 1);
            }
            asm volatile("" ::: "memory");
            PSTAMP(3);
        } else {
            load_tile(Lk, L, ldl, tid);
            load_inv(Tinv, a.Linv, tid);
            neg = a.Lsign[0];
            __syncthreads();
        }
        const int li = lane & 15, g = lane >> 4;
        int seen = 1;
        const int kf = fused ? 0 : 1;
        if (fused && lane < 2) seen = __hip_atomic_load(lane == 0 ? a.fin + 1 * mb + 0 : a.fin + 1 * mb + 1, __ATOMIC_RELAXED, __HIP_MEMORY_SCOPE_AGENT);
        for (int k = 0; k + 1 < mb; k++) {
            const int i = k + 1;
            PSTAMP(32 + 8 * k + 0);
            TriOps ops;
            tri_solve_preload(ops, Lk, Tinv, lane);
            const unsigned oik = (unsigned)(k * PB) * (unsigned)lds + (unsigned)(i * PB);
            const unsigned oii = (unsigned)(i * PB) * (unsigned)lds + (unsigned)(i * PB);
            f32x4 x[1][4];
            RegTile dt;
            const bool hit = k >= kf && __ballot(lane < 2 && seen == 0) == 0ull;
            if (a.dbg && tid == 0 && k >= kf) a.dbg[500 + k] = hit ? 100 : 101;
            if (hit) {
                unsigned od[4];
#pragma unroll
                for (int it = 0; it < 4; it++) {
                    const int e = tid + it * 256;
                    od[it] = oii + (unsigned)(e >> 4) * (unsigned)lds + (unsigned)(e & 15) * 4u;
                    asm volatile("" : "+v"(od[it]));
                }
                persist_tile_x_buf(x[0], bS, oik, lds, wave, lane);
#pragma unroll
                for (int it = 0; it < 4; it++) dt.v[it] = ld_sc1(bS, od[it]);
                asm volatile("s_waitcnt vmcnt(20)" ::: "memory");
                if (lane == 0) __hip_atomic_fetch_add(a.ready + k, 1, __ATOMIC_RELAXED, __HIP_MEMORY_SCOPE_AGENT);
            } else if (k >= kf) {
                persist_publish_wave(a.ready + k, lane);
                persist_poll(a, a.fin + i * mb + k, a.fin + i * mb + i, nullptr, lane);
                persist_tile_x<true>(x[0], S + oik, lds, wave, lane);
                dt.request(bS, oii, lds, tid);
            } else {
                persist_tile_x<false>(x[0], S + oik, lds, wave, lane);
#pragma unroll
                for (int it = 0; it < 4; it++) {
                    const int e = tid + it * 256;
                    dt.v[it] = *reinterpret_cast<const float4*>(S + oii + (size_t)(e >> 4) * lds + (e & 15) * 4);
                }
            }
            PSTAMP(32 + 8 * k + 1);
            tri_solve_pin(ops);
            PSTAMP(32 + 8 * k + 2);
            float* const txs[1] = {Ti};
            tri_solve_run<1>(x, txs, ops, wave, lane);
// ... 338 lines not shown
```

### ekf_vio_amd/csrc/common.h

```cpp
#pragma once
#include <hip/hip_runtime.h>
#include <stdint.h>

#include <chrono>
#include <string>
#include <vector>

#include "../../include/ekfvio.h"
#include "plan.h"
#ifdef EKFVIO_TEST_HOOKS
#include "../../include/ekfvio_test_hooks.h"
#endif

#ifndef EKF_POTRF_FV
#define EKF_POTRF_FV 12
#endif
#define EKF_FLUSH_THRESH (1e-8f * 1e-5f)

enum ProfClass {
    PC_LINEARIZE = 0,
    PC_PREDICT,
    PC_GEMM_PREDICT,
    PC_GATHER,
    PC_CHOL,
// ... 43 lines not shown
    float* mu_next = nullptr;
    float* last_klt = nullptr;
    uint8_t* del_flag = nullptr;
    float* P = nullptr;
    float* P2 = nullptr;
    float* FA = nullptr;
    float* FB = nullptr;
    float* FD = nullptr;
    float* Fdense = nullptr;
    int* idx = nullptr;
    int* inv_idx = nullptr;
    float* zmeas = nullptr;
    float* Rmeas = nullptr;
    uint8_t* pass = nullptr;
    float* yres = nullptr;
    float* Rm = nullptr;
    float* Saug = nullptr;
    float* Laug = nullptr;
    int ld_aug = 0;
    float* Linv = nullptr;
    unsigned long long* Lsign = nullptr;
    int* sweep_sync = nullptr;
    size_t sweep_sync_words = 0;
    bool sweep_latched_off = false;
    bool prelinearized = false;
    long long persistent_sweeps = 0;
    long long schur_sweeps = 0;
    long long sweep_recoveries = 0;
    long long early_output_frames = 0;
    int sweep_spin_limit = 0;
    int sweep_stall_wg = -1;
#ifdef EKFVIO_TEST_HOOKS
    int sweep_delay_wg = -1, sweep_delay_point = 0, sweep_delay_ticks = 0;
#endif
    bool sweep_retry_armed = false;
    double sweep_retry_pause_s = 0.0;
    int sweep_probation = 0;
    std::chrono::steady_clock::time_point sweep_retry_at;
    bool graph_leaves_flags_clean = false;
    bool sweep_flags_clean = false;
    bool persist_attr_set = false;
    bool gain2_attr_set = false;
    bool gather_attr_set = false;
    long long t2_updates = 0;
    long long graph_steps = 0;
    long long prelinearized_steps = 0;
    int num_cus = 0;
    int last_m = 0;
    long long* sweep_dbg = nullptr;
    long long* gemm_stamps = nullptr;
    float* Km = nullptr;
    float* Wt = nullptr;
    float* Gm = nullptr;
    int* info = nullptr;
    float gate_chi2 = 0.f;
    float* gate_d2 = nullptr;
    uint8_t* gate_flag = nullptr;
    uint8_t* gate_pass = nullptr;
    int* gate_words = nullptr;
    int* fb_words = nullptr;
    float* fb_err2 = nullptr;
    uint8_t* fb_flag = nullptr;
    float* fb_pt_err2 = nullptr;
    float* fb_pt_back = nullptr;
    uint8_t* fb_pt_flag = nullptr;
    int* remove_words = nullptr;
    int* h_info = nullptr;
    int* d_hinfo = nullptr;
    int status_seq = 0;
    float* h_out = nullptr;
    float* d_out = nullptr;
    bool out_fresh = false;
    unsigned char* h_meas = nullptr;
    unsigned char* d_meas = nullptr;
    float* seq_z = nullptr;
    float* seq_R = nullptr;
    uint8_t* seq_pass = nullptr;
    int seq_frames = 0;
    int seq_N = 0;
    std::vector<int> seq_m;
    std::vector<std::vector<uint8_t>> seq_pass_host;

    KltFrame frames[2];
    int cur = 0;
    int klt_border = 0;
    float* klt_prev_px = nullptr;
    float* klt_next_px = nullptr;
    uint8_t* klt_status = nullptr;
    float* klt_cov_px = nullptr;
    uint8_t* staging = nullptr;
    uint8_t* h_image = nullptr;
    size_t src_cap = 0;
    double dist[5] = {0, 0, 0, 0, 0};
    bool rect_on = false;
    int* rect_sx = nullptr;
    int* rect_sy = nullptr;
    uint8_t* rect_img = nullptr;
    size_t rect_cap = 0;
    RectifyKey rect_key;
    bool rect_key_valid = false;
    uint8_t* blurred = nullptr;
    unsigned* fast_row_kp = nullptr;
    int* fast_kp_xy = nullptr;
    short* fast_kp_score = nullptr;
    int fast_kp_cap = 0;
    uint8_t* occ_mask = nullptr;
// ... 34 lines not shown
    int n = 0;
    int* frame_counter = nullptr;
    int frames = 0;
    long long* stamps = nullptr;
    int* zero_words = nullptr;
    int n_zero = 0;
    int order2d = 0;
    int lin_blocks = 0;
    int lin_N = 0;
    float lin_dt = 0.f;
    float* lin_FA = nullptr;
    float* lin_FB = nullptr;
    float* lin_FD = nullptr;
    float* lin_mu_next = nullptr;
    int mean_keep = 0;
    int sym_w = 1;
    int sym = 0;
    const int* abort = nullptr;
};
void launch_gemm(ekfvio_filter* f, int transB, int M, int N, int K, float alpha, const float* A, int lda, const float* B,
                 int ldb, float beta, const float* Cin, int ldcin, float* C, int ldc, int flush, int lowerB = 0,
                 const GemmEpi* epi = nullptr);

void launch_gemm_variant(ekfvio_filter* f, int variant, int transB, int M, int N, int K, float alpha, const float* A, int lda,
                         const float* B, int ldb, float beta, const float* Cin, int ldcin, float* C, int ldc, int flush,
                         int lowerB);


struct BookArgs {
    int enabled = 0;
    int N = 0, m_pad = 0;
    const float* z = nullptr;
    const float* R = nullptr;
    const uint8_t* pass = nullptr;
    float* last_klt = nullptr;
    uint8_t* del_flag = nullptr;
    int* idx = nullptr;
    int* inv_idx = nullptr;
    float* zrow = nullptr;
    float* Rm = nullptr;
    const int* frame_counter = nullptr;
    int* m_out = nullptr;
    uint8_t* pass_eff = nullptr;
    const float* mu = nullptr;
    const float* P = nullptr;
    int ldp = 0;
    float chi2 = 0.f;
    float* d2 = nullptr;
    uint8_t* gated = nullptr;
    int* gate_words = nullptr;
    int count_total = 0;
};
BookArgs make_book_args(ekfvio_filter* f, int m, const float* d_z, const float* d_R, const uint8_t* d_pass, const int* d_frame_counter);
void launch_linearize(ekfvio_filter* f, float dt, const BookArgs* book = nullptr);
void launch_build_dense_F(ekfvio_filter* f, float* Fdense);
void launch_predict(ekfvio_filter* f, float dt, const BookArgs* book = nullptr);
struct UpdateInputs {
    int m = 0;
    const float *z = nullptr, *R = nullptr;
    const uint8_t* pass = nullptr;
    int* frame_counter = nullptr;
    int frames = 0;
    bool bookkeeping_done = false;
    bool m_on_device = false;
    bool gate_counted = false;
    float next_dt = -1.f;
    int publish_seq = 0;
    int (*between)(ekfvio_filter*, int kyp_blocks) = nullptr;
    bool recoverable = true;
};
struct UpdateResult {
    bool published = false;
    int between_seq = 0;
};
UpdateResult launch_update(ekfvio_filter* f, const UpdateInputs& in);
void launch_check_sigma(ekfvio_filter* f, float* d_out);
int klt_level_pitch(int w);
int klt_border();
void klt_intrinsics(const ekfvio_filter* f, const float* K, float* fx, float* fy, float* cx, float* cy);
void launch_imu_update(ekfvio_filter* f, const float gyro[3], const float accel[3]);
int fast_alloc(ekfvio_filter* f);
void fast_free(ekfvio_filter* f);
int fast_ensure(ekfvio_filter* f, int w, int h);
void launch_publish_status(ekfvio_filter* f, int seq);
int wait_status(ekfvio_filter* f, int* status, const int* extra_dev = nullptr, int* extra_out = nullptr);
int next_status_seq(ekfvio_filter* f);
void sweep_abort_latch(ekfvio_filter* f);
void sweep_clean_update(ekfvio_filter* f);
void sweep_maybe_retry(ekfvio_filter* f);
int poll_status(ekfvio_filter* f, int seq, int* status, int* extra_out);
int add_features_device(ekfvio_filter* f, int k);
void add_features_enqueue_device_count(ekfvio_filter* f, const int* count_dev);
int replenish_enqueue(ekfvio_filter* f, int* enqueued);

int live_handles_on(int device);
inline PlanShape plan_shape(const ekfvio_filter* f) {
    PlanShape s;
    s.num_cus = f->num_cus, s.ldp = f->ldp, s.sweep_sync_words = f->sweep_sync_words, s.N = f->N, s.n = f->n;
    s.dense_predict = f->cfg.predict_mode == EKFVIO_PREDICT_DENSE;
    s.sole_handle = live_handles_on(f->device) <= 1;
    s.latched_off = f->sweep_latched_off;
    return s;
}
inline UpdatePlan plan_update(const ekfvio_filter* f, int m, bool m_on_device = false, float next_dt = -1.f, bool recoverable = true) {
    return plan_update(f->tune, plan_shape(f), m, m_on_device, next_dt, recoverable);
}
int launch_update_gemms_scratch(ekfvio_filter* f, const UpdatePlan& p, int reps);
const int* launch_chol_sweep(ekfvio_filter* f, const UpdatePlan& p, float* Saug, float* Laug, float* Linv, int ld, bool zero_flags);
const int* launch_persist_fused(ekfvio_filter* f, const UpdatePlan& p, bool zero_flags);
void launch_joseph_g(ekfvio_filter* f, int m, int m_pad, int n_pad, bool m_on_device, const float* T = nullptr);
inline float* t2_buffer(ekfvio_filter* f) { return f->Fdense; }
void launch_gain2_tiles(ekfvio_filter* f, const UpdatePlan& p);
void launch_gather_potrf(ekfvio_filter* f, const UpdatePlan& p);
void launch_potrf_stamps(ekfvio_filter* f, const float* S, int ld, float* L, float* Linv, long long* d_stamps);
void launch_gain_from_sweep(ekfvio_filter* f, const UpdatePlan& p, const float* Laug, int ld, int n, float* K, float* scratch, int ldk, int refine);

void launch_remove_features(ekfvio_filter* f, const uint8_t* remove, const int* added, bool abort_aware, int* host_removed);
size_t remove_lds_bytes(const ekfvio_filter* f);
void remove_applied(ekfvio_filter* f, int delta, int removed);
int rectify_ensure(ekfvio_filter* f, size_t src);
void rectify_free(ekfvio_filter* f);
const uint8_t* rectify_enqueue(ekfvio_filter* f, const uint8_t* src, int w, int h, const float K[9], hipStream_t st);
int klt_alloc(ekfvio_filter* f);
void klt_free(ekfvio_filter* f);

struct ProfScope {
    ekfvio_filter* f;
    int cls;
    int launches;
    ProfScope(ekfvio_filter* f_, int cls_, double flops = 0, int launches_ = 1) : f(f_), cls(cls_), launches(launches_) {
        if (f->prof_on) {
            (void)hipEventRecord(f->ev0, f->stream);
            f->prof[cls].flops += flops;
        }
    }
    ~ProfScope() {
        if (f->prof_on) {
            (void)hipEventRecord(f->ev1, f->stream);
            (void)hipEventSynchronize(f->ev1);
            float ms = 0;
            (void)hipEventElapsedTime(&ms, f->ev0, f->ev1);
            f->prof[cls].ms += ms;
            f->prof[cls].launches += launches;
        }
    }
};
```

### ekf_vio_amd/csrc/ekf_kernels.hip

```cpp
#include <algorithm>
#include <utility>

#include "common.h"

namespace {

#include "motion_model.inc"

template <int NT, bool EFF = false>
__device__ __forceinline__ void bookkeeping_body(const BookArgs& a) {
    __shared__ int s_cnt[32];
    __shared__ int s_total;
    const int tid = threadIdx.x;
    const int N = a.N, m_pad = a.m_pad;
    const float* z = a.z;
    const float* R = a.R;
    const uint8_t* pass = a.pass;
    if (a.frame_counter) {
        const int fi = *a.frame_counter;
        z += (size_t)fi * 2 * N;
        R += (size_t)fi * 4 * N;
        pass += (size_t)fi * N;
    }
    if (EFF) pass = a.pass_eff;
    const int per = (N + NT - 1) / NT;
    const int lo = tid * per;
    const int hi = min(N, lo + per);
    int c = 0;
    for (int i = lo; i < hi; i++) c += pass[i] ? 1 : 0;
    const int lane = tid & 63, wv = tid >> 6;
    constexpr int NW = NT / 64;
    int incl = c;
#pragma unroll
    for (int off = 1; off < 64; off <<= 1) {
        const int v = __shfl_up(incl, off, 64);
        if (lane >= off) incl += v;
    }
    if (lane == 63) s_cnt[wv] = incl;
    __syncthreads();
    if (wv == 0) {
        int t = (lane < NW) ? s_cnt[lane] : 0;
        int ti = t;
#pragma unroll
        for (int off = 1; off < NW; off <<= 1) {
            const int v = __shfl_up(ti, off, 64);
            if (lane >= off) ti += v;
        }
        if (lane < NW) s_cnt[16 + lane] = ti - t;
        if (lane == NW - 1) s_total = ti;
    }
    __syncthreads();
    int base = s_cnt[16 + wv] + incl - c;
    for (int i = lo; i < hi; i++) {
        if (pass[i]) {
            const int r = 2 * base;
            const int s = EKF_BASE + 3 * i;
            a.last_klt[2 * i] = z[2 * i];
            a.last_klt[2 * i + 1] = z[2 * i + 1];
            a.idx[r] = s;
            a.idx[r + 1] = s + 1;
// ... 71 lines not shown
        const int c = e - 9;
        float t0 = u, t1 = v, t2 = rho;
        if (c == 0) t0 = plus_delta(t0);
        if (c == 1) t1 = plus_delta(t1);
        if (c == 2) t2 = plus_delta(t2);
        hi = convolve_feature(bm[0], t0, t1, t2);
        if (c == 0) t0 = minus_2delta(t0);
        if (c == 1) t1 = minus_2delta(t1);
        if (c == 2) t2 = minus_2delta(t2);
        lo = convolve_feature(bm[0], t0, t1, t2);
    }
    out[0] = (hi.x - lo.x) / td;
    out[1] = (hi.y - lo.y) / td;
    out[2] = (hi.z - lo.z) / td;
}
__device__ __forceinline__ BaseMotion lin_base_motion(const float* s_base, int v, float dt) {
    float t[EKF_BASE];
#pragma unroll
    for (int i = 0; i < EKF_BASE; i++) t[i] = s_base[i];
    if (v > 0) {
        const int c = 7 + (v - 1) / 2;
#pragma unroll
        for (int i = 7; i < 16; i++) {
            if (i == c) {
                t[i] = plus_delta(t[i]);
                if (((v - 1) & 1) == 1) t[i] = minus_2delta(t[i]);
            }
        }
    }
    return base_motion(t, dt);
}
__device__ __forceinline__ void lin_base_test_point(const float* s_base, int q, float dt, float* out) {
    const int j = q >> 1;
    float t[EKF_BASE], o[EKF_BASE];
#pragma unroll
    for (int i = 0; i < EKF_BASE; i++) t[i] = (i == j) ? plus_delta(s_base[i]) : s_base[i];
    if (q & 1) {
#pragma unroll
        for (int i = 0; i < EKF_BASE; i++) t[i] = (i == j) ? minus_2delta(t[i]) : t[i];
    }
    convolve_base(t, dt, o);
#pragma unroll
    for (int i = 0; i < EKF_BASE; i++) out[i] = o[i];
}

#define PT 16
#define PC 3

__device__ __forceinline__ float predict_finish(float acc, int i, int j, float dt) {
    if (i == j) acc = acc + process_noise(i, dt);
    return (fabsf(acc) > EKF_FLUSH_THRESH) ? acc : 0.f;
}

template <bool LIN>
__global__ __launch_bounds__(256) void predict_fused_kernel(const float* __restrict__ P, int ld, int N, int n,
                                                            const float* __restrict__ FA, const float* __restrict__ FB,
                                                            const float* __restrict__ FD, float dt,
                                                            float* __restrict__ Pout, int tiles_side, int chunks,
                                                            const float* __restrict__ mu, float* __restrict__ mu_next, BookArgs book,
                                                            long long* dbg) {
    const int tid = threadIdx.x;
    const int ntile = tiles_side * tiles_side;
#define PSTAMP_(slot)                                                                                               \
    do {                                                                                                            \
        if (dbg && tid == 0) {                                                                                      \
            const int b_ = (int)blockIdx.x;                                                                         \
            const int w_ = b_ == 0 ? 0 : b_ == 1 ? 1 : b_ == ntile ? 2 : b_ == ntile + 1 ? 3 : b_ == ntile + chunks + 1 ? 4 : -1; \
            if (w_ >= 0) dbg[900 + 8 * w_ + (slot)] = (long long)__builtin_amdgcn_s_memtime();                      \
        }                                                                                                           \
    } while (0)
    PSTAMP_(0);
    __shared__ float sm[4096];
    __shared__ float s_base[EKF_BASE];
    __shared__ BaseMotion s_bm[19];
    const float td = two_delta();
    if (book.enabled && blockIdx.x == gridDim.x - 1) {
        bookkeeping_body<256>(book);
        return;
    }
    if (LIN) {
        if (tid < EKF_BASE) s_base[tid] = mu[tid];
    }
    if ((int)blockIdx.x < ntile) {
        float* sPbb = sm;
        float* sPbg = sm + 96;
        float* sPfb = sPbg + PT * 27;
        float* sBf = sPfb + PT * 27;
        float* sBg = sBf + PT * 27;
        float* sDf = sBg + PT * 27;
        float* sDg = sDf + PT * 9;
        float* sXb = sDg + PT * 9;
        const int tI = blockIdx.x / tiles_side, tJ = blockIdx.x % tiles_side;
        const int f0 = tI * PT, g0 = tJ * PT;
        if (tid < 81) sPbb[tid] = P[(size_t)(7 + tid % 9) * ld + 7 + tid / 9];
        float lu[2] = {0.f, 0.f}, lv[2] = {0.f, 0.f}, lrho[2] = {1.f, 1.f};
        if (LIN) {
#pragma unroll
            for (int sl = 0; sl < 2; sl++) {
                const int task = tid + 256 * sl;
                int lmk = -1;
                if (task < 384) lmk = ((task >= 192) ? g0 : f0) + (task % 192) / 12;
                else if (tI == tJ && tid >= 128 && tid < 128 + PT) lmk = f0 + tid - 128;
                if (lmk >= 0 && lmk < N) {
                    lu[sl] = mu[EKF_BASE + 3 * lmk];
                    lv[sl] = mu[EKF_BASE + 3 * lmk + 1];
                    lrho[sl] = mu[EKF_BASE + 3 * lmk + 2];
                }
            }
        }
#ifndef EKF_PREDICT_LIN_TWO_BARRIERS
        if (LIN) {
            float pg[2], pf[2];
#pragma unroll
            for (int it = 0; it < 2; it++) {
                const int e = tid + 256 * it;
                const int l = e / 27, w = e % 27;
                const int f = f0 + l, g = g0 + l;
                const bool in = e < PT * 27;
                pg[it] = (in && g < N) ? P[(size_t)(EKF_BASE + 3 * g + w % 3) * ld + 7 + w / 3] : 0.f;
                pf[it] = (in && f < N) ? P[(size_t)(7 + w % 9) * ld + EKF_BASE + 3 * f + w / 9] : 0.f;
            }
            if (tid >= 192 && tid < 192 + 19) {
                float b[EKF_BASE];
#pragma unroll
                for (int i = 0; i < EKF_BASE; i++) b[i] = mu[i];
                s_bm[tid - 192] = lin_base_motion(b, tid - 192, dt);
            }
#pragma unroll
            for (int it = 0; it < 2; it++) {
                const int e = tid + 256 * it;
                if (e < PT * 27) {
                    sPbg[e] = pg[it];
                    sPfb[e] = pf[it];
                }
            }
        } else
#endif
        for (int e = tid; e < PT * 27; e += 256) {
            const int l = e / 27, w = e % 27;
            const int f = f0 + l, g = g0 + l;
            sPbg[e] = (g < N) ? P[(size_t)(EKF_BASE + 3 * g + w % 3) * ld + 7 + w / 3] : 0.f;
            sPfb[e] = (f < N) ? P[(size_t)(7 + w % 9) * ld + EKF_BASE + 3 * f + w / 9] : 0.f;
            if (!LIN) {
                sBf[e] = (f < N) ? FB[(size_t)f * 27 + w] : 0.f;
                sBg[e] = (g < N) ? FB[(size_t)g * 27 + w] : 0.f;
            }
        }
        if (!LIN) {
            for (int e = tid; e < PT * 9; e += 256) {
                const int l = e / 9, w = e % 9;
                sDf[e] = (f0 + l < N) ? FD[(size_t)(f0 + l) * 9 + w] : 0.f;
                sDg[e] = (g0 + l < N) ? FD[(size_t)(g0 + l) * 9 + w] : 0.f;
            }
        }
        __syncthreads();
        PSTAMP_(1);
        if (LIN) {
#ifdef EKF_PREDICT_LIN_TWO_BARRIERS
            if (tid < 19) s_bm[tid] = lin_base_motion(s_base, tid, dt);
            __syncthreads();
#endif
#pragma unroll
            for (int sl = 0; sl < 2; sl++) {
                const int task = tid + 256 * sl;
                if (task < 384) {
                    const int side = task >= 192, l = (task % 192) / 12, e = task % 12;
                    const int lmk = (side ? g0 : f0) + l;
                    float o[3] = {0.f, 0.f, 0.f};
                    if (lmk < N) lin_column(s_bm, lu[sl], lv[sl], lrho[sl], e, td, o);
                    float* dst = (e < 9) ? ((side ? sBg : sBf) + l * 27 + e * 3) : ((side ? sDg : sDf) + l * 9 + (e - 9) * 3);
                    dst[0] = o[0];
                    dst[1] = o[1];
                    dst[2] = o[2];
                } else if (tI == tJ && tid >= 128 && tid < 128 + PT && f0 + tid - 128 < N) {
                    const V3 o = convolve_feature(s_bm[0], lu[sl], lv[sl], lrho[sl]);
                    const int lmk = f0 + tid - 128;
                    mu_next[EKF_BASE + 3 * lmk] = o.x;
                    mu_next[EKF_BASE + 3 * lmk + 1] = o.y;
                    mu_next[EKF_BASE + 3 * lmk + 2] = o.z;
                }
            }
            __syncthreads();
        }
        PSTAMP_(2);
        for (int e = tid; e < PT * 27; e += 256) {
            const int l = e / 27, r = (e % 27) / 9, b = e % 9;
            float acc = 0.f;
#pragma unroll
            for (int c = 0; c < 9; c++) acc = acc + sBf[l * 27 + c * 3 + r] * sPbb[c * 9 + b];
#pragma unroll
            for (int q = 0; q < 3; q++) acc = acc + sDf[l * 9 + q * 3 + r] * sPfb[l * 27 + q * 9 + b];
            sXb[e] = acc;
        }
        __syncthreads();
        PSTAMP_(3);
        const int lf = tid % PT, lg = tid / PT;
        const int f = f0 + lf, g = g0 + lg;
        if (f >= N || g >= N) return;
        float Pfg[3][3];
#pragma unroll
        for (int sIdx = 0; sIdx < 3; sIdx++) {
            const float3 c3 = *reinterpret_cast<const float3*>(P + (size_t)(EKF_BASE + 3 * g + sIdx) * ld + EKF_BASE + 3 * f);
            Pfg[0][sIdx] = c3.x;
            Pfg[1][sIdx] = c3.y;
            Pfg[2][sIdx] = c3.z;
        }
        float Xg[3][3];
#pragma unroll
        for (int r = 0; r < 3; r++)
#pragma unroll
            for (int sIdx = 0; sIdx < 3; sIdx++) {
                float acc = 0.f;
#pragma unroll
                for (int c = 0; c < 9; c++) acc = acc + sBf[lf * 27 + c * 3 + r] * sPbg[lg * 27 + c * 3 + sIdx];
#pragma unroll
                for (int q = 0; q < 3; q++) acc = acc + sDf[lf * 9 + q * 3 + r] * Pfg[q][sIdx];
                Xg[r][sIdx] = acc;
            }
#pragma unroll
        for (int sIdx = 0; sIdx < 3; sIdx++) {
            float o3[3];
#pragma unroll
            for (int r = 0; r < 3; r++) {
                float acc = 0.f;
#pragma unroll
                for (int c = 0; c < 9; c++) acc = acc + sXb[lf * 27 + r * 9 + c] * sBg[lg * 27 + c * 3 + sIdx];
#pragma unroll
                for (int q = 0; q < 3; q++) acc = acc + Xg[r][q] * sDg[lg * 9 + q * 3 + sIdx];
                const int i = EKF_BASE + 3 * f + r, j = EKF_BASE + 3 * g + sIdx;
                o3[r] = predict_finish(acc, i, j, dt);
            }
            *reinterpret_cast<float3*>(Pout + (size_t)(EKF_BASE + 3 * g + sIdx) * ld + EKF_BASE + 3 * f) = make_float3(o3[0], o3[1], o3[2]);
        }
        PSTAMP_(4);
        return;
    }
    const int wb = (int)blockIdx.x - ntile;
    float* sA = sm;
    float* sLB = sm + 3072;
    float* sLD = sLB + PC * 27;
    const float* FBp = FB;
    const float* FDp = FD;
    int lm0 = 0;
    if (LIN) {
        float* s_hi = sm + 2048;
        float* s_lo = s_hi + 16 * EKF_BASE;
        lm0 = (wb == 0) ? 0 : ((wb <= chunks) ? (wb - 1) * PC : (wb - chunks - 1) * PC);
        const int lt = tid - 128;
        float u = 0.f, v = 0.f, rho = 1.f;
        const bool ltask = wb > 0 && lt >= 0 && lt < PC * 12 && lm0 + lt / 12 < N;
        if (ltask) {
            const int lmk = lm0 + lt / 12;
            u = mu[EKF_BASE + 3 * lmk];
            v = mu[EKF_BASE + 3 * lmk + 1];
            rho = mu[EKF_BASE + 3 * lmk + 2];
        }
        __syncthreads();
        if (tid < 32) {
            lin_base_test_point(s_base, tid, dt, ((tid & 1) ? s_lo : s_hi) + (tid >> 1) * EKF_BASE);
        } else if (tid == 32 && wb == 0) {
            float o[EKF_BASE];
            convolve_base(s_base, dt, o);
#pragma unroll
            for (int i = 0; i < EKF_BASE; i++) mu_next[i] = o[i];
        } else if (tid >= 64 && tid < 64 + 19) {
            s_bm[tid - 64] = lin_base_motion(s_base, tid - 64, dt);
        }
        __syncthreads();
        for (int e = tid; e < EKF_BASE * EKF_BASE; e += 256) {
            const int j = e / EKF_BASE, i = e % EKF_BASE;
            sA[e] = (j < 16) ? (s_hi[j * EKF_BASE + i] - s_lo[j * EKF_BASE + i]) / td : ((i == j) ? 1.f : 0.f);
        }
        if (wb > 0 && lt >= 0 && lt < PC * 12) {
            float o[3] = {0.f, 0.f, 0.f};
            const int l = lt / 12, e = lt % 12;
            if (ltask) lin_column(s_bm, u, v, rho, e, td, o);
            float* dst = (e < 9) ? (sLB + l * 27 + e * 3) : (sLD + l * 9 + (e - 9) * 3);
            dst[0] = o[0];
            dst[1] = o[1];
            dst[2] = o[2];
        }
        FBp = sLB;
        FDp = sLD;
        __syncthreads();
        PSTAMP_(1);
    } else {
        for (int e = tid; e < EKF_BASE * EKF_BASE; e += 256) sA[e] = FA[e];
    }
    if (wb <= chunks) {
        float* sX1 = sm + 512;
// ... 81 lines not shown
__global__ __launch_bounds__(1024) void update_bookkeeping_kernel(BookArgs a) { bookkeeping_body<1024>(a); }

__global__ __launch_bounds__(1024) void gate_bookkeeping_kernel(BookArgs a) {
    __shared__ int s_gated;
    const int tid = threadIdx.x, N = a.N;
    const float* z = a.z;
    const float* R = a.R;
    const uint8_t* pass = a.pass;
    if (a.frame_counter) {
        const int fi = *a.frame_counter;
        z += (size_t)fi * 2 * N;
        R += (size_t)fi * 4 * N;
        pass += (size_t)fi * N;
    }
    if (tid == 0) s_gated = 0;
    __syncthreads();
    const int per = (N + 1023) / 1024;
    const int lo = tid * per, hi = min(N, lo + per);
    int rejected = 0;
    for (int i = lo; i < hi; i++) {
        float d2 = -1.f;
        uint8_t eff = 0, rej = 0;
        if (pass[i]) {
            const int s = EKF_BASE + 3 * i;
            const float* Ps = a.P + (size_t)s * a.ldp + s;
            const float y0 = z[2 * i] - a.mu[s], y1 = z[2 * i + 1] - a.mu[s + 1];
            const float ca = Ps[0] + R[4 * i];
            const float cb = Ps[1] + R[4 * i + 1];
            const float cc = Ps[a.ldp + 1] + R[4 * i + 3];
            const float det = ca * cc - cb * cb;
            const float q = ((cc * y0) * y0 - ((2.f * cb) * y0) * y1) + (ca * y1) * y1;
            d2 = q / det;
            eff = (det > 0.f && d2 <= a.chi2) ? 1 : 0;
            rej = eff ^ 1;
            rejected += rej;
        }
        a.d2[i] = d2;
        a.gated[i] = rej;
        a.pass_eff[i] = eff;
    }
    if (rejected) atomicAdd(&s_gated, rejected);
    __syncthreads();
    if (tid == 0) {
        a.gate_words[0] = s_gated;
        a.gate_words[1] = N;
        if (a.count_total) {
            long long* total = reinterpret_cast<long long*>(a.gate_words + 2);
            *total = *total + s_gated;
        }
    }
    bookkeeping_body<1024, true>(a);
}

#include "gather_body.inc"

__global__ __launch_bounds__(256) void gather_kernel(GatherArgs a) {
    __shared__ float tile[64 * 65];
    gather_body(a, blockIdx.x, tile);
}

__global__ __launch_bounds__(256) void mean_update_kernel(const float* __restrict__ K, int ld, int n, int m,
                                                          const float* __restrict__ y, float* mu, int* frame_counter,
                                                          int frames) {
    __shared__ float s_part[4][64];
    __shared__ float s_q[4];
    const int rl = threadIdx.x & 63, w = threadIdx.x >> 6;
    const int i = blockIdx.x * 64 + rl;
    const int chunk = (m + 3) / 4;
    const int r0 = w * chunk, r1 = min(m, r0 + chunk);
    float acc = 0.f;
    if (i < n) {
#pragma unroll 8
        for (int r = r0; r < r1; r++) acc = acc + K[(size_t)r * ld + i] * y[r];
    }
    s_part[w][rl] = acc;
    __syncthreads();
    float v = 0.f;
    if (w == 0 && i < n) v = mu[i] + (((s_part[0][rl] + s_part[1][rl]) + s_part[2][rl]) + s_part[3][rl]);
    if (blockIdx.x == 0) {
        if (w == 0 && rl >= 3 && rl <= 6) s_q[rl - 3] = v;
        __syncthreads();
        if (w == 0 && rl >= 3 && rl <= 6) {
            float qn = sqrtf(s_q[0] * s_q[0] + s_q[1] * s_q[1] + s_q[2] * s_q[2] + s_q[3] * s_q[3]);
            v = v / qn;
        }
    }
    if (w == 0 && i < n) mu[i] = v;
    if (frame_counter && blockIdx.x == 0 && threadIdx.x == 0) {
        const int fi = *frame_counter + 1;
        *frame_counter = (fi >= frames) ? 0 : fi;
    }
}

__global__ void check_sigma_kernel(const float* P, int ld, int n, float* out) {
    __shared__ float s_min[256], s_max[256];
    float mn = 3.4e38f, mx = 0.f;
    for (size_t e = threadIdx.x; e < (size_t)n * n; e += 256) {
        int i = e % n, j = e / n;
        if (i == j) mn = fminf(mn, P[(size_t)j * ld + i]);
        if (i > j) mx = fmaxf(mx, fabsf(P[(size_t)j * ld + i] - P[(size_t)i * ld + j]));
    }
    s_min[threadIdx.x] = mn;
    s_max[threadIdx.x] = mx;
    __syncthreads();
    for (int s = 128; s > 0; s >>= 1) {
        if (threadIdx.x < s) {
            s_min[threadIdx.x] = fminf(s_min[threadIdx.x], s_min[threadIdx.x + s]);
            s_max[threadIdx.x] = fmaxf(s_max[threadIdx.x], s_max[threadIdx.x + s]);
        }
        __syncthreads();
    }
    if (threadIdx.x == 0) {
        out[0] = s_min[0];
        out[1] = s_max[0];
    }
}

}

void launch_linearize(ekfvio_filter* f, float dt, const BookArgs* book) {
    ProfScope ps(f, PC_LINEARIZE);
    BookArgs b;
    if (book) b = *book;
    const int blocks = (f->N + LIN_LM - 1) / LIN_LM + 1 + (b.enabled ? 1 : 0);
    hipLaunchKernelGGL(linearize_kernel, dim3(blocks), dim3(256), 0, f->stream, f->mu, f->N, dt, f->FA, f->FB, f->FD,
                       f->mu_next, b);
}

BookArgs make_book_args(ekfvio_filter* f, int m, const float* d_z, const float* d_R, const uint8_t* d_pass, const int* d_frame_counter) {
    BookArgs a;
    a.enabled = 1;
    a.N = f->N;
    a.m_pad = round_up(m > 0 ? m : 1, EKF_TILE);
    a.z = d_z;
    a.R = d_R;
    a.pass = d_pass;
    a.last_klt = f->last_klt;
    a.del_flag = f->del_flag;
    a.idx = f->idx;
    a.inv_idx = f->inv_idx;
    a.zrow = f->yres;
    a.Rm = f->Rm;
    a.frame_counter = d_frame_counter;
    return a;
}

void launch_build_dense_F(ekfvio_filter* f, float* Fdense) {
    dim3 grid((f->ldp + 255) / 256, f->ldp);
    hipLaunchKernelGGL(build_dense_F_kernel, grid, dim3(256), 0, f->stream, f->FA, f->FB, f->FD, f->N, f->n, f->ldp,
                       Fdense);
}

void launch_predict(ekfvio_filter* f, float dt, const BookArgs* book) {
    const int tiles_side = (f->N + PT - 1) / PT;
    const bool pre = f->prelinearized && f->cfg.predict_mode != EKFVIO_PREDICT_DENSE;
    f->prelinearized = false;
    if (pre) f->prelinearized_steps++;
    const bool lin_in_predict = !pre && f->cfg.predict_mode != EKFVIO_PREDICT_DENSE && f->tune.fuse_linearize && tiles_side * tiles_side <= 4 * f->num_cus;
    if (!lin_in_predict && !pre) launch_linearize(f, dt, book);
    const int n = f->n, ld = f->ldp;
    dim3 grid((n + 255) / 256, n);
    if (f->cfg.predict_mode == EKFVIO_PREDICT_DENSE) {
        launch_build_dense_F(f, f->Fdense);
        const int np = round_up(n, 32);
        {
            ProfScope ps(f, PC_GEMM_PREDICT, 4.0 * n * (double)n * n);
            launch_gemm(f, 0, n, n, np, 1.f, f->Fdense, ld, f->P, ld, 0.f, nullptr, 0, f->P2, ld, 0);
            launch_gemm(f, 1, n, n, np, 1.f, f->P2, ld, f->Fdense, ld, 0.f, nullptr, 0, f->P, ld, 0);
        }
        ProfScope ps(f, PC_PREDICT);
        hipLaunchKernelGGL(add_noise_flush_kernel, grid, dim3(256), 0, f->stream, f->P, ld, n, dt);
    } else {
        ProfScope ps(f, PC_PREDICT, 4.0 * n * (358.0 + 36.0 * f->N));
        const int ts = (f->N + PT - 1) / PT;
        const int chunks = (f->N + PC - 1) / PC;
        BookArgs b;
        if (book && (lin_in_predict || pre)) b = *book;
        if (lin_in_predict)
            hipLaunchKernelGGL(predict_fused_kernel<true>, dim3(ts * ts + 1 + 2 * chunks + (b.enabled ? 1 : 0)), dim3(256), 0, f->stream,
                               f->P, ld, f->N, n, f->FA, f->FB, f->FD, dt, f->P2, ts, chunks, f->mu, f->mu_next, b, f->sweep_dbg);
        else
            hipLaunchKernelGGL(predict_fused_kernel<false>, dim3(ts * ts + 1 + 2 * chunks + (b.enabled ? 1 : 0)), dim3(256), 0, f->stream, f->P, ld, f->N, n,
                               f->FA, f->FB, f->FD, dt, f->P2, ts, chunks, f->mu, f->mu_next, b, f->sweep_dbg);
        std::swap(f->P, f->P2);
    }
    std::swap(f->mu, f->mu_next);
}

UpdateResult launch_update(ekfvio_filter* f, const UpdateInputs& in) {
    const bool gate = f->gate_chi2 > 0.f && f->N > 0;
    const UpdatePlan p = plan_update(f, in.m, in.m_on_device || (gate && in.m > 0), in.next_dt, in.recoverable);
    const int m = p.m, m_pad = p.m_pad, n_pad = p.n_pad, n = f->n, ld = f->ldp;
    UpdateResult out;
    f->last_m = m;
    {
        ProfScope ps(f, PC_GATHER);
        if (!in.bookkeeping_done) {
            BookArgs bk = make_book_args(f, m, in.z, in.R, in.pass, in.frame_counter);
            if (p.m_on_device) bk.m_out = f->info + 2;
            if (gate) {
                bk.pass_eff = f->gate_pass, bk.mu = f->mu, bk.P = f->P, bk.ldp = ld, bk.chi2 = f->gate_chi2;
                bk.d2 = f->gate_d2, bk.gated = f->gate_flag, bk.gate_words = f->gate_words, bk.count_total = in.gate_counted ? 0 : 1;
                hipLaunchKernelGGL(gate_bookkeeping_kernel, dim3(1), dim3(1024), 0, f->stream, bk);
            } else
                hipLaunchKernelGGL(update_bookkeeping_kernel, dim3(1), dim3(1024), 0, f->stream, bk);
        }
        if (p.fused_gather) {
            launch_gather_potrf(f, p);
        } else if (m > 0 && p.sweep != SWEEP_PERSIST_FUSED) {
            const GatherArgs ga = make_gather_args(f, p);
            const int nb2 = p.with_wt ? (m_pad / 64) * (ld / 64) : 0;
            hipLaunchKernelGGL(gather_kernel, dim3(ga.nb1 + nb2), dim3(256), 0, f->stream, ga);
        }
    }
    if (m <= 0) {
        ProfScope ps(f, PC_UPDATE_MISC);
        hipLaunchKernelGGL(mean_update_kernel, dim3((n + 63) / 64), dim3(256), 0, f->stream, f->Km, ld, n, 0, f->yres, f->mu,
                           in.frame_counter, in.frames);
        return out;
    }
    const bool zero_flags = p.persistent() && !p.fused_gather && !f->sweep_flags_clean;
    const int* abort = p.sweep == SWEEP_PERSIST_FUSED ? launch_persist_fused(f, p, zero_flags)
                                                      : launch_chol_sweep(f, p, f->Saug, f->Laug, f->Linv, f->ld_aug, zero_flags);
    if (in.publish_seq) launch_publish_status(f, in.publish_seq), out.published = true;
    GemmEpi e2;
    e2.mode = 2, e2.mu = f->mu, e2.Pcol = f->P + (size_t)n * ld, e2.n = n;
    e2.frame_counter = in.frame_counter, e2.frames = in.frames;
    e2.sym = f->tune.sym_joseph;
    e2.abort = abort;
    if (p.persistent()) {
        e2.zero_words = f->sweep_sync, e2.n_zero = persist_zero_words(m_pad, n_pad);
        f->sweep_flags_clean = true;
    }
    if (p.tail == TAIL_T2) f->t2_updates++;
    if (p.gain == GAIN_SCHUR) launch_joseph_g(f, m, m_pad, n_pad, p.m_on_device);
    else if (p.gain == GAIN2_T2_TILES) launch_gain2_tiles(f, p);
    else if (p.gain != GAIN_SWEEP) launch_gain_from_sweep(f, p, f->Laug, f->ld_aug, n, f->Km, f->Gm, ld, 0);
    if (p.tail == TAIL_JOSEPH) {
        GemmEpi e1;
        e1.mode = 1, e1.inv_idx = f->inv_idx, e1.Rm = f->Rm, e1.G = f->Gm, e1.ldg = ld, e1.abort = abort;
        ProfScope ps(f, PC_GEMM_UPDATE, 2.0 * n * (double)(n + 1) * m_pad + 2.0 * n * (double)n * m_pad, 2);
        launch_gemm(f, 1, n, n + 1, m_pad, -1.f, f->Km, ld, f->Wt, ld, 1.f, f->P, ld, f->P, ld, 0, 0, &e1);
        if (in.between) out.between_seq = in.between(f, 0);
        launch_gemm(f, 1, n, n, m_pad, 1.f, f->Gm, ld, f->Km, ld, 1.f, f->P, ld, f->P, ld, 1, 0, &e2);
        return out;
    }
    if (p.tail == TAIL_T2 && in.between) out.between_seq = in.between(f, m_pad / 64);
    ProfScope ps(f, PC_GEMM_UPDATE, 2.0 * n * (double)n * m_pad, 1);
    e2.mode = 3;
    e2.Kyp = f->Wt, e2.kyp_blocks = m_pad / 64, e2.kyp_ld = ld;
    if (p.lin_blocks) {
        e2.lin_blocks = p.lin_blocks, e2.lin_N = f->N, e2.lin_dt = in.next_dt;
        e2.lin_FA = f->FA, e2.lin_FB = f->FB, e2.lin_FD = f->FD, e2.lin_mu_next = f->mu_next;
        f->prelinearized = true;
    }
    launch_gemm(f, 1, n, n, m_pad, 1.f, f->Km, ld, f->Gm, ld, 1.f, p.tail == TAIL_T2 ? t2_buffer(f) : f->P, ld, f->P, ld, 1, 0, &e2);
    return out;
}

int launch_update_gemms_scratch(ekfvio_filter* f, const UpdatePlan& p, int reps) {
    const int n = f->n, ld = f->ldp, m_pad = p.m_pad;
    GemmEpi e1, e2;
    if (p.tail != TAIL_JOSEPH) {
        e2.mode = 2;
        for (int r = 0; r < reps; r++)
            launch_gemm(f, 1, n, n, m_pad, 1.f, f->Km, ld, f->Gm, ld, 1.f, f->P, ld, f->P2, ld, 1, 0, &e2);
        return 1;
    }
    e1.mode = 1, e1.inv_idx = f->inv_idx, e1.Rm = f->Rm, e1.G = f->Gm, e1.ldg = ld;
    e2.mode = 2;
    e2.sym = f->tune.sym_joseph;
    for (int r = 0; r < reps; r++) {
        launch_gemm(f, 1, n, n + 1, m_pad, -1.f, f->Km, ld, f->Wt, ld, 1.f, f->P, ld, f->P2, ld, 0, 0, &e1);
        launch_gemm(f, 1, n, n, m_pad, 1.f, f->Gm, ld, f->Km, ld, 1.f, f->P2, ld, f->P2, ld, 1, 0, &e2);
    }
// ... 7 lines not shown
```

### ekf_vio_amd/csrc/plan.h

```cpp
#ifndef EKFVIO_PLAN_H_
#define EKFVIO_PLAN_H_
#include <stddef.h>
#include <stdlib.h>

#include <algorithm>

#define EKF_BASE 22
#define EKF_TILE 64
#ifndef EKF_SWEEP_SPLIT_MB
#define EKF_SWEEP_SPLIT_MB 16
#endif
#define LIN_LM 8
#define GC 4
#define GCI 4

static inline int round_up(int x, int m) { return (x + m - 1) / m * m; }

struct Tuning {
    int early_status = 1;
    int upload_kernel = 1;
    int sweep_wait_ticks = 300000;
    double sweep_retry_first_s = 2.0;
    int persist_sweep = 1;
    int sweep_la = 1;
    int fuse_gather = 1;
    int fuse_sweep = 1;
    int t2_flow = 1;
    int schur = 0;
    int persist_oversub = 0;
    int persist_gain = 1;
    int persist_early = 1;
    int frame_outputs = 1;
    int early_outputs = 1;
    int gemm_order2d = 1;
    int lin_overlap = 1;
    int sym_joseph = 1;
    int fuse_linearize = 1;
};

inline Tuning tuning_from_env() {
    enum Kind { FLAG, RAW, WAIT_MS, POSITIVE };
    struct Entry {
        const char* name;
        Kind kind;
        int Tuning::*i;
        double Tuning::*d;
    };
    static const Entry table[] = {
        {"EKFVIO_EARLY_STATUS", FLAG, &Tuning::early_status, nullptr},
        {"EKFVIO_UPLOAD_KERNEL", FLAG, &Tuning::upload_kernel, nullptr},
        {"EKFVIO_SWEEP_WAIT_MS", WAIT_MS, &Tuning::sweep_wait_ticks, nullptr},
        {"EKFVIO_SWEEP_RETRY_S", POSITIVE, nullptr, &Tuning::sweep_retry_first_s},
        {"EKFVIO_SWEEP", FLAG, &Tuning::persist_sweep, nullptr},
        {"EKFVIO_SWEEP_LA", FLAG, &Tuning::sweep_la, nullptr},
        {"EKFVIO_FUSE_GATHER", FLAG, &Tuning::fuse_gather, nullptr},
        {"EKFVIO_FUSE_SWEEP", FLAG, &Tuning::fuse_sweep, nullptr},
        {"EKFVIO_T2", FLAG, &Tuning::t2_flow, nullptr},
        {"EKFVIO_SCHUR", FLAG, &Tuning::schur, nullptr},
        {"EKFVIO_PERSIST_OVERSUB", RAW, &Tuning::persist_oversub, nullptr},
        {"EKFVIO_PERSIST_GAIN", FLAG, &Tuning::persist_gain, nullptr},
        {"EKFVIO_PERSIST_EARLY", FLAG, &Tuning::persist_early, nullptr},
        {"EKFVIO_FRAME_OUTPUTS", FLAG, &Tuning::frame_outputs, nullptr},
        {"EKFVIO_EARLY_OUTPUTS", FLAG, &Tuning::early_outputs, nullptr},
        {"EKFVIO_GEMM_ORDER2D", FLAG, &Tuning::gemm_order2d, nullptr},
        {"EKFVIO_LIN_OVERLAP", FLAG, &Tuning::lin_overlap, nullptr},
        {"EKFVIO_SYM_JOSEPH", FLAG, &Tuning::sym_joseph, nullptr},
        {"EKFVIO_FUSE_LINEARIZE", FLAG, &Tuning::fuse_linearize, nullptr},
    };
    Tuning t;
    for (const Entry& k : table) {
        const char* e = getenv(k.name);
        if (!e) continue;
        if (k.kind == FLAG) t.*k.i = atoi(e) ? 1 : 0;
        else if (k.kind == RAW) t.*k.i = atoi(e);
        else if (atof(e) > 0) {
            if (k.kind == WAIT_MS) t.*k.i = (int)std::min(2.0e9, 1e5 * atof(e));
            else t.*k.d = atof(e);
        }
    }
    return t;
}

#ifdef __HIPCC__
#define PLAN_HD __host__ __device__ __forceinline__
#else
#define PLAN_HD inline
#endif
struct PersistFlags {
    int mb, rows;
    PersistFlags(int m_pad, int n_pad) : mb(m_pad / EKF_TILE), rows(2 * (m_pad / EKF_TILE) + n_pad / EKF_TILE) {}
    int ready() const { return 0; }
    int fin() const { return mb; }
    int pan() const { return fin() + rows * mb; }
    int abort_word() const { return pan() + rows * mb + 1; }
    int zero_words() const { return abort_word(); }
    size_t words() const { return ((size_t)abort_word() + 1 + 3) & ~(size_t)3; }
};
inline size_t persist_flag_words(int m_pad, int n_pad) { return PersistFlags(m_pad, n_pad).words(); }
inline int persist_zero_words(int m_pad, int n_pad) { return PersistFlags(m_pad, n_pad).zero_words(); }
#define PERSIST_POLL_FLAGS 63

struct FilterDims {
    int n_cap;
    int ldp;
    int m_cap;
    int ld_aug;
    size_t sweep_sync_words;
};
inline FilterDims filter_dims(int max_features) {
    FilterDims d;
    d.n_cap = EKF_BASE + 3 * max_features;
    d.ldp = round_up(d.n_cap + 1, 64);
    d.m_cap = round_up(2 * max_features > 0 ? 2 * max_features : 1, 64);
    d.ld_aug = d.m_cap + d.ldp + d.m_cap;
    d.sweep_sync_words = std::max((size_t)1024, (size_t)PersistFlags(d.m_cap, d.ldp + EKF_TILE).abort_word() + 7);
    return d;
}

struct PlanShape {
    int num_cus = 0;
// ... 114 lines not shown
inline int t2_skip_owners(const Tuning& t, const PlanShape& s, int m_pad, int n_pad) {
    if (!t.t2_flow || !t.persist_gain || t.schur || !gain_in_sweep_shape(t, s, m_pad, n_pad)) return -1;
    const PersistGrid g{GRID_COMPACT, m_pad / EKF_TILE, n_pad / EKF_TILE, s.ldp / 64};
    if (g.total() > s.num_cus) return -1;
    if (g.nX + 2 > PERSIST_POLL_FLAGS) return -1;
    return (t2_pairs(g.nX) <= g.owners()) ? 0 : -1;
}
inline PersistGrid persist_grid(const UpdatePlan& p, int ldp) {
    return {p.sweep != SWEEP_PERSIST_FUSED ? GRID_PLAIN : p.compact ? GRID_COMPACT : GRID_FUSED, p.m_pad / EKF_TILE, p.n_pad / EKF_TILE, ldp / 64, p.t2_skip};
}
inline SweepKind choose_sweep(const Tuning& t, const PlanShape& s, int m_pad, int n_pad, bool filter_update) {
    const int mb = m_pad / EKF_TILE;
    const bool schur_shape = t.schur && mb < EKF_SWEEP_SPLIT_MB;
    if (schur_shape && filter_update) return SWEEP_SCHUR;
    if (t.persist_sweep && !s.latched_off && !schur_shape && s.sole_handle && persist_shape(t, s, m_pad, n_pad))
        return (filter_update && t.fuse_sweep && t.fuse_gather) ? SWEEP_PERSIST_FUSED : SWEEP_PERSIST;
    return mb < EKF_SWEEP_SPLIT_MB ? SWEEP_STEP : t.sweep_la ? SWEEP_SPLIT_LA : SWEEP_SPLIT;
}
inline bool gain_tiles_shape(const Tuning& t, const PlanShape& s, int m_pad, int n_pad) { return t.persist_gain && gain_in_sweep_shape(t, s, m_pad, n_pad); }

inline UpdatePlan plan_raw_sweep(const Tuning& t, const PlanShape& s, int m_pad, int n_pad) {
    UpdatePlan p;
    p.m = p.m_pad = m_pad, p.n_pad = n_pad;
    p.sweep = choose_sweep(t, s, m_pad, n_pad, false);
    p.gain = gain_tiles_shape(t, s, m_pad, n_pad) ? GAIN_TILES : GAIN_GEMM;
    return p;
}

inline UpdatePlan plan_update(const Tuning& t, const PlanShape& s, int m, bool m_on_device = false, float next_dt = -1.f, bool recoverable = true) {
    UpdatePlan p;
    if (m_on_device) m = 2 * s.N;
    const int n = s.n, ld = s.ldp, m_pad = round_up(m > 0 ? m : 1, EKF_TILE), n_pad = round_up(n, EKF_TILE);
    p.m = m, p.m_pad = m_pad, p.n_pad = n_pad, p.m_on_device = m_on_device, p.recoverable = recoverable;
    if (m <= 0) return p;
    p.sweep = choose_sweep(t, s, m_pad, n_pad, true);
    const bool schur = p.sweep == SWEEP_SCHUR, fused = p.sweep == SWEEP_PERSIST_FUSED;
    p.with_wt = !schur;
    if (t.fuse_gather && !fused)
        p.fused_gather = 1 + gather_element_wgs(ld, m_pad) + (schur ? 0 : (m_pad / 64) * (ld / 64)) <= s.num_cus;
    if (schur) return p.gain = GAIN_SCHUR, p.tail = TAIL_SCHUR, p;
    p.t2_skip = t2_skip_owners(t, s, m_pad, n_pad);
    if (p.t2_skip < 0) {
        p.gain = !gain_tiles_shape(t, s, m_pad, n_pad) ? GAIN_GEMM : fused ? GAIN_SWEEP : GAIN_TILES;
        return p.tail = TAIL_JOSEPH, p;
    }
    p.tail = TAIL_T2;
    p.t2_by_sweep = p.compact = fused;
    p.gain = fused ? GAIN_SWEEP : GAIN2_T2_TILES;
    const int lin_blocks = (s.N + LIN_LM - 1) / LIN_LM + 1;
    if (next_dt >= 0.f && t.lin_overlap && !s.dense_predict && t.fuse_linearize && gemm_single_round_with(s.num_cus, n, n, m_pad, 1 + lin_blocks))
        p.lin_blocks = lin_blocks;
    return p;
}
#endif
```

### ekf_vio_amd/filter.py

```python
import ctypes as C

import numpy as np

from . import capi

BASE_STATE_SIZE = 22


def _fp(a):
    return a.ctypes.data_as(C.POINTER(C.c_float))


def _u8(a):
    return a.ctypes.data_as(C.POINTER(C.c_uint8))


class TightlyCoupledEKF:
    def __init__(self, max_features=100, device=0, stream=None, predict_mode=capi.PREDICT_STRUCTURED,
                 default_point_depth=0.5, default_point_depth_variance=100.0,
                 default_point_homogenous_variance=1e-5, hooks=False, gate_chi2=0.0, klt_fb_max_px=0.0, distortion=None, **cfg_overrides):
        self.hooks = bool(hooks)
        self.lib = capi.load(hooks=self.hooks)
        cfg = capi.Config()
        self._chk(self.lib.ekfvio_default_config(C.byref(cfg)))
# ... 178 lines not shown
        N = feat.shape[0]
        klt = np.ascontiguousarray(st["last_klt"], dtype=np.float32).reshape(N, 2)
        dele = np.ascontiguousarray(st["del_flag"], dtype=np.uint8).reshape(N)
        sig = np.ascontiguousarray(np.asarray(st["Sigma"], dtype=np.float32).T)
        n = BASE_STATE_SIZE + 3 * N
        self._chk(self.lib.ekfvio_set_state(self.h, N, _fp(base), _fp(feat), _fp(klt), _u8(dele), _fp(sig), n))

    def upload_measurements(self, z, R, passed):
        z = np.ascontiguousarray(z, dtype=np.float32)
        R = np.ascontiguousarray(R, dtype=np.float32)
        p = np.ascontiguousarray(passed, dtype=np.uint8)
        frames = p.shape[0]
        self._chk(self.lib.ekfvio_upload_measurements(self.h, frames, _fp(z), _fp(R), _u8(p)))

    def run_uploaded(self, first, count, dt):
        self._chk(self.lib.ekfvio_run_uploaded(self.h, first, count, float(dt)))

    def synchronize(self):
        return self._chk(self.lib.ekfvio_synchronize(self.h), allow=(capi.ENUMERIC,))

    def profile(self, on):
        self._chk(self.lib.ekfvio_profile_enable(self.h, int(on)))
        if on:
            self._chk(self.lib.ekfvio_profile_reset(self.h))

    def profile_report(self):
        out = {}
        for c in range(self.lib.ekfvio_profile_count()):
            ms, n, fl = C.c_double(0), C.c_int64(0), C.c_double(0)
            self._chk(self.lib.ekfvio_profile_get(self.h, c, C.byref(ms), C.byref(n), C.byref(fl)))
            out[self.lib.ekfvio_profile_name(c).decode()] = dict(ms=ms.value, launches=n.value, flops=fl.value)
        return out

    def profile_update_gemms(self, reps=50):
        us, fl = C.c_double(0), C.c_double(0)
        self._chk(self.lib.ekfvio_profile_update_gemms(self.h, int(reps), C.byref(us), C.byref(fl)))
        return us.value, fl.value

    def test_gemm(self, A, B, C0, alpha=1.0, beta=0.0, transB=True, variant=0):
        self._need_hooks()
        A = np.asarray(A, np.float32)
        B = np.asarray(B, np.float32)
        M, K = A.shape
        N = B.shape[0] if transB else B.shape[1]
        Ac, Bc = np.array(A.T, order="C", copy=True), np.array(B.T, order="C", copy=True)
        Cc = np.array(np.asarray(C0, np.float32).T, order="C", copy=True)
        self._chk(self.lib.ekfvio_test_gemm(self.h, int(transB), M, N, K, alpha, _fp(Ac), M, _fp(Bc), B.shape[0], beta,
                                            _fp(Cc), M, int(variant)))
        return Cc.T.copy()

    def counters(self):
        c = (C.c_int64 * 8)()
        self._chk(self.lib.ekfvio_get_counters(self.h, c))
        return dict(persistent=int(c[0]), schur=int(c[1]), recoveries=int(c[2]), mode=int(c[3]), early_output_frames=int(c[4]), t2_updates=int(c[5]),
                    graph_steps=int(c[6]), prelinearized_steps=int(c[7]))

    def _need_hooks(self):
        if not self.hooks:
            raise RuntimeError("this entry point exists only in the hooks build: construct the filter with hooks=True")

    def persistent_sweeps(self):
        return self.counters()["persistent"]

    def sweep_counts(self):
        c = self.counters()
        return {k: c[k] for k in ("persistent", "schur", "recoveries", "mode")}

    def sweep_fault(self, spin_limit=0, stall_workgroup=-1):
        self._need_hooks()
        self._chk(self.lib.ekfvio_test_sweep_fault(self.h, int(spin_limit), int(stall_workgroup)))

    def sweep_delay(self, workgroup=-1, point=0, ticks=0):
        self._need_hooks()
        self._chk(self.lib.ekfvio_test_sweep_delay(self.h, int(workgroup), int(point), int(ticks)))

    def test_cholesky_solve(self, S, Crhs):
        self._need_hooks()
        S = np.asarray(S, np.float32)
        Crhs = np.asarray(Crhs, np.float32)
        m, nr = S.shape[0], Crhs.shape[0]
        Sc, Cc = np.array(S.T, order="C", copy=True), np.array(Crhs.T, order="C", copy=True)
        L = np.zeros((m, m), np.float32)
        X = np.zeros((m, nr), np.float32)
        info = C.c_int32(0)
        self._chk(self.lib.ekfvio_test_cholesky_solve(self.h, m, nr, _fp(Sc), _fp(Cc), _fp(L), _fp(X), C.byref(info)))
        return L.T.copy(), X.T.copy(), info.value


class KLTTracker:

    def __init__(self, ekf):
        self.ekf = ekf
        self.lib = ekf.lib

    def push_frame(self, img, K):
        img = np.ascontiguousarray(img, dtype=np.uint8)
        h, w = img.shape
        K = np.ascontiguousarray(K, dtype=np.float32).reshape(9)
        self.ekf._chk(self.lib.ekfvio_klt_push_frame(self.ekf.h, _u8(img), w, h, w, _fp(K)))

    def findNewFeaturePositions(self):
        N = self.ekf.num_features
        z = np.zeros((N, 2), np.float32)
        R = np.zeros((N, 4), np.float32)
        p = np.zeros(N, np.uint8)
        self.ekf._chk(self.lib.ekfvio_klt_track(self.ekf.h, _fp(z), _fp(R), _u8(p)))
        return z, R, p

# ... 163 lines not shown
```

### include/ekfvio.h

```cpp
#ifndef EKFVIO_H_
#define EKFVIO_H_

#include <stdint.h>

#ifndef EKFVIO_API
#define EKFVIO_API __attribute__((visibility("default")))
#endif

#ifdef __cplusplus
extern "C" {
#endif

#define EKFVIO_BASE_STATE_SIZE 22

enum {
    EKFVIO_OK = 0,
    EKFVIO_EINVAL = 1,
    EKFVIO_ENUMERIC = 2,
    EKFVIO_ECAPACITY = 3,
    EKFVIO_EDEVICE = 4,
    EKFVIO_ESTATE = 5,
    EKFVIO_EABORTED = 6
};

// ... 62 lines not shown
EKFVIO_API int ekfvio_get_points(ekfvio_filter* f, float* xyz3N, float* intensityN);
EKFVIO_API int ekfvio_check_sigma(ekfvio_filter* f, float* min_diag, float* max_asym);

EKFVIO_API int ekfvio_set_state(ekfvio_filter* f, int32_t n_features, const float* base_mu, const float* mu3N,
                     const float* last_klt2N, const uint8_t* delete_flagN, const float* sigma, int32_t ld);

EKFVIO_API int ekfvio_remove_features(ekfvio_filter* f, const uint8_t* remove, int32_t count, int32_t* removed);

EKFVIO_API int ekfvio_set_gate(ekfvio_filter* f, float chi2);
EKFVIO_API int ekfvio_get_gate(ekfvio_filter* f, float* d2, uint8_t* gated, int32_t* n_landmarks, int32_t* gated_last,
                               int64_t* gated_total);

EKFVIO_API int ekfvio_set_distortion(ekfvio_filter* f, const double* D, int32_t count);
EKFVIO_API int ekfvio_rectify_map(const float K[9], const double* D, int32_t count, int32_t width, int32_t height, int32_t* sx,
                                  int32_t* sy);

EKFVIO_API int ekfvio_klt_push_frame(ekfvio_filter* f, const uint8_t* image, int32_t width, int32_t height, int32_t stride,
                          const float K[9]);
EKFVIO_API int ekfvio_klt_track(ekfvio_filter* f, float* z2N, float* R4N, uint8_t* passN);
EKFVIO_API int ekfvio_klt_track_points(ekfvio_filter* f, const float* prev_px, const float* init_px, int32_t count,
                            float* out_px, uint8_t* status);

EKFVIO_API int ekfvio_set_klt_fb(ekfvio_filter* f, float max_px);
EKFVIO_API int ekfvio_get_klt_fb(ekfvio_filter* f, float* err2, uint8_t* rejected, int32_t* n_landmarks, int32_t* rejected_last,
                                 int64_t* rejected_total);
EKFVIO_API int ekfvio_klt_track_points_fb(ekfvio_filter* f, const float* prev_px, const float* init_px, int32_t count, float* out_px,
                                          uint8_t* status, float* back_px, float* err2, uint8_t* fb_ok);

EKFVIO_API int ekfvio_klt_uncertainty_points(ekfvio_filter* f, const float* ref_px, const float* cur_px, int32_t count, float* cov4);

EKFVIO_API int ekfvio_klt_get_level(ekfvio_filter* f, int32_t level, int32_t* w, int32_t* h, uint8_t* img, int16_t* deriv);

EKFVIO_API int ekfvio_step_image(ekfvio_filter* f, double stamp, const uint8_t* image, int32_t width, int32_t height,
                      int32_t stride, const float K[9]);

EKFVIO_API int ekfvio_replenish(ekfvio_filter* f, int32_t* added, int32_t* new_px_xy);
EKFVIO_API int ekfvio_fast_detect(ekfvio_filter* f, int32_t threshold, int32_t nonmax, int32_t cap, int32_t* xy, int32_t* score,
                       int32_t* count);
EKFVIO_API int ekfvio_imu(ekfvio_filter* f, double stamp, const float gyro[3], const float accel[3]);
EKFVIO_API int ekfvio_imu_update(ekfvio_filter* f, const float gyro[3], const float accel[3]);

EKFVIO_API int ekfvio_upload_measurements(ekfvio_filter* f, int32_t frames, const float* z, const float* R, const uint8_t* pass);
EKFVIO_API int ekfvio_run_uploaded(ekfvio_filter* f, int32_t first, int32_t count, float dt);
EKFVIO_API int ekfvio_synchronize(ekfvio_filter* f);

EKFVIO_API int ekfvio_profile_enable(ekfvio_filter* f, int32_t on);
EKFVIO_API int ekfvio_profile_reset(ekfvio_filter* f);
EKFVIO_API int ekfvio_profile_count(void);
EKFVIO_API const char* ekfvio_profile_name(int32_t cls);
EKFVIO_API int ekfvio_profile_get(ekfvio_filter* f, int32_t cls, double* total_ms, int64_t* launches, double* flops);
EKFVIO_API int ekfvio_profile_update_gemms(ekfvio_filter* f, int32_t reps, double* avg_launch_us, double* flops_per_launch);

EKFVIO_API int ekfvio_get_counters(ekfvio_filter* f, int64_t counters[8]);

#ifdef __cplusplus
}
#endif
#endif
```

### include/ekfvio_test_hooks.h

```cpp
#ifndef EKFVIO_TEST_HOOKS_H_
#define EKFVIO_TEST_HOOKS_H_
#include "ekfvio.h"
#ifdef __cplusplus
extern "C" {
#endif

EKFVIO_API int ekfvio_test_klt_padded_level(ekfvio_filter* f, int32_t level, int32_t* border, uint8_t* img, int16_t* deriv);
EKFVIO_API int ekfvio_test_blurred_level0(ekfvio_filter* f, uint8_t* out);
EKFVIO_API int ekfvio_test_gemm(ekfvio_filter* f, int32_t transB, int32_t M, int32_t N, int32_t K, float alpha, const float* A,
                     int32_t lda, const float* B, int32_t ldb, float beta, float* C, int32_t ldc, int32_t variant);
EKFVIO_API int ekfvio_test_gemm_bench(ekfvio_filter* f, int32_t transB, int32_t lowerB, int32_t M, int32_t N, int32_t K,
                           int32_t reps, int32_t variant, double* mean_us);
EKFVIO_API int ekfvio_test_potrf_stamps(ekfvio_filter* f, int64_t stamps[80]);
EKFVIO_API int ekfvio_test_sweep_stamps(ekfvio_filter* f, int enable, int64_t stamps[1024]);
EKFVIO_API int ekfvio_test_sweep_fault(ekfvio_filter* f, int32_t spin_limit, int32_t stall_workgroup);
#define EKFVIO_TEST_SWEEP_DELAY_MAX_TICKS 100000
EKFVIO_API int ekfvio_test_sweep_delay(ekfvio_filter* f, int32_t workgroup, int32_t point, int32_t ticks);
EKFVIO_API int ekfvio_test_cholesky_solve(ekfvio_filter* f, int32_t m, int32_t nrhs, const float* S, const float* Crhs,
                               float* L_out, float* X_out, int32_t* info);
EKFVIO_API int ekfvio_test_plan(int32_t num_cus, int32_t max_features, int32_t N, int32_t m, int32_t m_on_device, int32_t sole_handle,
                                int32_t latched_off, int32_t dense_predict, float next_dt, int32_t plan[12]);
EKFVIO_API int ekfvio_test_persist_grid(int32_t num_cus, int32_t max_features, int32_t N, int32_t m, int32_t m_on_device, int32_t sole_handle,
                                        int32_t latched_off, int32_t dense_predict, float next_dt, int32_t* roles, int32_t max_blocks,
                                        int32_t out[10]);
EKFVIO_API int ekfvio_test_t2_pair(int32_t p, int32_t pair[2]);

#ifdef __cplusplus
}
#endif
#endif
```

Measured before the change: 11070.

## Fold first Cholesky tile of update into predict kernel launch

Lets the predict kernel take on the first (0,0) block of the update's Cholesky factorization (the 'pre00' role) when a planner decides it fits, so the update can begin with that tile already done. The 64-wide potrf code is moved into a shared include so the predict kernel can use it, and the eager step path now also folds bookkeeping into predict. The aim is to shorten the critical path between predict and update within each step, at the cost of extra planning logic, a device counter word and a larger predict kernel.

```diff
diff --git a/ekf_vio_amd/capi.py b/ekf_vio_amd/capi.py
--- a/ekf_vio_amd/capi.py
+++ b/ekf_vio_amd/capi.py
@@ -37,10 +37,10 @@
            "ekfvio_klt_uncertainty_points", "ekfvio_step_image", "ekfvio_replenish", "ekfvio_fast_detect", "ekfvio_imu", "ekfvio_imu_update",
            "ekfvio_upload_measurements", "ekfvio_run_uploaded", "ekfvio_synchronize", "ekfvio_profile_enable",
            "ekfvio_profile_reset", "ekfvio_profile_count", "ekfvio_profile_name", "ekfvio_profile_get",
-           "ekfvio_profile_update_gemms", "ekfvio_get_counters", "ekfvio_set_gate", "ekfvio_get_gate",
+           "ekfvio_profile_update_gemms", "ekfvio_get_counters", "ekfvio_get_pre00_updates", "ekfvio_set_gate", "ekfvio_get_gate",
            "ekfvio_set_klt_fb", "ekfvio_get_klt_fb", "ekfvio_klt_track_points_fb", "ekfvio_set_distortion", "ekfvio_rectify_map"]
 HOOK_SYMBOLS = ["ekfvio_test_klt_padded_level", "ekfvio_test_blurred_level0", "ekfvio_test_gemm", "ekfvio_test_gemm_bench", "ekfvio_test_potrf_stamps",
-                "ekfvio_test_sweep_stamps", "ekfvio_test_sweep_fault", "ekfvio_test_sweep_delay", "ekfvio_test_cholesky_solve", "ekfvio_test_plan", "ekfvio_test_persist_grid", "ekfvio_test_t2_pair"]
+                "ekfvio_test_sweep_stamps", "ekfvio_test_sweep_fault", "ekfvio_test_sweep_delay", "ekfvio_test_cholesky_solve", "ekfvio_test_plan", "ekfvio_test_pre00_plan", "ekfvio_test_persist_grid", "ekfvio_test_t2_pair"]
 
 _libs = {}
 
@@ -85,6 +85,7 @@
         "ekfvio_profile_get": [vp, i32, C.POINTER(C.c_double), C.POINTER(C.c_int64), C.POINTER(C.c_double)],
         "ekfvio_profile_update_gemms": [vp, i32, C.POINTER(C.c_double), C.POINTER(C.c_double)],
         "ekfvio_get_counters": [vp, C.POINTER(C.c_int64)],
+        "ekfvio_get_pre00_updates": [vp, C.POINTER(C.c_int64)],
         "ekfvio_set_gate": [vp, f32], "ekfvio_get_gate": [vp, fp, u8p, ip, ip, C.POINTER(C.c_int64)],
         "ekfvio_set_klt_fb": [vp, f32], "ekfvio_get_klt_fb": [vp, fp, u8p, ip, ip, C.POINTER(C.c_int64)],
         "ekfvio_klt_track_points_fb": [vp, fp, fp, i32, fp, u8p, fp, fp, u8p],
@@ -103,6 +104,7 @@
             "ekfvio_test_sweep_delay": [vp, i32, i32, i32],
             "ekfvio_test_gemm_bench": [vp, i32, i32, i32, i32, i32, i32, i32, C.POINTER(C.c_double)],
             "ekfvio_test_plan": [i32] * 8 + [f32, ip],
+            "ekfvio_test_pre00_plan": [i32] * 10 + [ip],
             "ekfvio_test_persist_grid": [i32] * 8 + [f32, ip, i32, ip],
             "ekfvio_test_t2_pair": [i32, ip],
         })
diff --git a/ekf_vio_amd/csrc/api.hip b/ekf_vio_amd/csrc/api.hip
--- a/ekf_vio_amd/csrc/api.hip
+++ b/ekf_vio_amd/csrc/api.hip
@@ -214,6 +214,7 @@
     HIPC(f, dev_alloc(f->stream, &f->Wt, pm));
     HIPC(f, dev_alloc(f->stream, &f->Gm, pm));
     HIPC(f, dev_alloc(f->stream, &f->info, 4));
+    HIPC(f, dev_alloc(f->stream, &f->pre00_words, 4));
     HIPC(f, dev_alloc(f->stream, &f->remove_words, 4));
     HIPC(f, hipHostMalloc((void**)&f->h_info, 16 * sizeof(int), hipHostMallocMapped | hipHostMallocCoherent));
     memset(f->h_info, 0, 16 * sizeof(int));
@@ -288,7 +289,7 @@
     if (f->stream) (void)hipStreamSynchronize(f->stream);
     void* ptrs[] = {f->mu, f->mu_next, f->last_klt, f->del_flag, f->P,  f->P2, f->FA, f->FB, f->FD,   f->Fdense,
                     f->idx, f->inv_idx, f->zmeas,  f->Rmeas,    f->pass,     f->yres, f->Rm, f->Saug,  f->Laug,  f->Linv, f->Lsign, f->Km, f->sweep_sync, f->sweep_dbg,
-                    f->Wt,  f->Gm,     f->info,     f->remove_words, f->seq_z,    f->seq_R, f->seq_pass, f->gate_words, f->fb_words};
+                    f->Wt,  f->Gm,     f->info,     f->pre00_words, f->remove_words, f->seq_z,    f->seq_R, f->seq_pass, f->gate_words, f->fb_words};
     for (void* p : ptrs)
         if (p) hipFree(p);
     if (f->h_info) hipHostFree(f->h_info);
@@ -665,6 +666,19 @@
     in.recoverable = false;
     return in;
 }
+static void eager_step(ekfvio_filter* f, int m, int i, int* counter, float dt) {
+    UpdateInputs in = uploaded_update(f, m, i, counter);
+    const UpdatePlan next = plan_update(f, m, false, -1.f, false);
+    const bool ride = f->gate_chi2 <= 0.f && m > 0 && pre00_role(f->tune, plan_shape(f), next, true, false);
+    if (ride) {
+        const BookArgs bk = make_book_args(f, m, in.z, in.R, in.pass, counter);
+        in.pre00 = launch_predict(f, dt, &bk, &next);
+        in.bookkeeping_done = true;
+    } else {
+        launch_predict(f, dt);
+    }
+    launch_update(f, in);
+}
 static int capture_steps(ekfvio_filter* f, int steps, int m, float dt, int* counter, hipGraphExec_t* out, int* pre_out) {
     hipGraph_t g = nullptr;
     HIPC(f, hipStreamSynchronize(f->stream));
@@ -675,10 +689,12 @@
     const bool gate = f->gate_chi2 > 0.f;
     for (int k = 0; k < steps; k++) {
         const BookArgs bk = make_book_args(f, m, f->seq_z, f->seq_R, f->seq_pass, counter);
-        launch_predict(f, dt, gate ? nullptr : &bk);
+        const UpdatePlan next = plan_update(f, m, false, -1.f, false);
+        const bool pre00 = launch_predict(f, dt, gate ? nullptr : &bk, gate ? nullptr : &next);
         UpdateInputs in = uploaded_update(f, m, 0, counter);
         in.bookkeeping_done = !gate;
         in.next_dt = (k + 1 < steps) ? dt : -1.f;
+        in.pre00 = pre00;
         launch_update(f, in);
     }
     f->prelinearized = false;
@@ -734,17 +750,13 @@
         while (s + EKF_GRAPH_STEPS <= count) HIPC(f, replay(f->step_graph, EKF_GRAPH_STEPS, f->graph_pre));
         while (s + 2 <= count) HIPC(f, replay(f->step_graph_pair, 2, f->graph_pre_pair));
         if (s > 0) f->sweep_flags_clean = f->graph_leaves_flags_clean;
-        for (; s < count; s++) {
-            launch_predict(f, dt);
-            launch_update(f, uploaded_update(f, m, 0, counter));
-        }
+        for (; s < count; s++) eager_step(f, m, 0, counter, dt);
         HIPC(f, hipGetLastError());
         return EKFVIO_OK;
     }
     for (; s < count; s++) {
         const int i = (first + s) % f->seq_frames;
-        launch_predict(f, dt);
-        launch_update(f, uploaded_update(f, f->seq_m[i], i, nullptr));
+        eager_step(f, f->seq_m[i], i, nullptr, dt);
     }
     HIPC(f, hipGetLastError());
     return EKFVIO_OK;
@@ -900,6 +912,16 @@
     counters[5] = f->t2_updates;
     counters[6] = f->graph_steps;
     counters[7] = f->prelinearized_steps;
+    return EKFVIO_OK;
+}
+
+int ekfvio_get_pre00_updates(ekfvio_filter* f, int64_t* updates) {
+    if (!f || !updates) return EKFVIO_EINVAL;
+    HIPC(f, hipSetDevice(f->device));
+    int w[4] = {0, 0, 0, 0};
+    HIPC(f, hipMemcpyAsync(w, f->pre00_words, sizeof(w), hipMemcpyDeviceToHost, f->stream));
+    HIPC(f, hipStreamSynchronize(f->stream));
+    memcpy(updates, w + 2, sizeof(int64_t));
     return EKFVIO_OK;
 }
 
@@ -1117,6 +1139,18 @@
     return EKFVIO_OK;
 }
 
+int ekfvio_test_pre00_plan(int32_t num_cus, int32_t max_features, int32_t N, int32_t m, int32_t m_on_device, int32_t sole_handle,
+                           int32_t latched_off, int32_t dense_predict, int32_t book_in_predict, int32_t gate, int32_t* carried) {
+    if (!carried || max_features < 0 || N < 0 || N > max_features) return EKFVIO_EINVAL;
+    const FilterDims d = filter_dims(max_features);
+    PlanShape s;
+    s.num_cus = num_cus, s.ldp = d.ldp, s.sweep_sync_words = d.sweep_sync_words, s.N = N, s.n = EKF_BASE + 3 * N;
+    s.dense_predict = dense_predict != 0, s.sole_handle = sole_handle != 0, s.latched_off = latched_off != 0;
+    const Tuning t = tuning_from_env();
+    *carried = pre00_role(t, s, plan_update(t, s, m, m_on_device != 0), book_in_predict != 0, gate != 0) ? 1 : 0;
+    return EKFVIO_OK;
+}
+
 int ekfvio_test_persist_grid(int32_t num_cus, int32_t max_features, int32_t N, int32_t m, int32_t m_on_device, int32_t sole_handle,
                              int32_t latched_off, int32_t dense_predict, float next_dt, int32_t* roles, int32_t max_blocks, int32_t out[10]) {
     if (!out || max_features < 0 || N < 0 || N > max_features) return EKFVIO_EINVAL;
diff --git a/ekf_vio_amd/csrc/chol.hip b/ekf_vio_amd/csrc/chol.hip
--- a/ekf_vio_amd/csrc/chol.hip
+++ b/ekf_vio_amd/csrc/chol.hip
@@ -4,138 +4,7 @@
 
 namespace {
 
-typedef float f32x16 __attribute__((ext_vector_type(16)));
-typedef float f32x4 __attribute__((ext_vector_type(4)));
-
-#define PB 64
-#ifndef PLD
-#define PLD 68
-#endif
-#define ILD 17
-#define INV_LDS (4 * 16 * ILD)
-
-__device__ __forceinline__ float lane_bcast(float v, int src_lane) {
-    return __int_as_float(__builtin_amdgcn_readlane(__float_as_int(v), src_lane));
-}
-__device__ __forceinline__ double lane_bcast_d(double v, int src_lane) {
-    const int lo = __builtin_amdgcn_readlane(__double2loint(v), src_lane);
-    const int hi = __builtin_amdgcn_readlane(__double2hiint(v), src_lane);
-    return __hiloint2double(hi, lo);
-}
-
-template <int B, int E, class F>
-__device__ __forceinline__ void static_for(F&& f) {
-    if constexpr (B < E) {
-        f(std::integral_constant<int, B>{});
-        static_for<B + 1, E>(f);
-    }
-}
-template <int R>
-__device__ __forceinline__ void dpp_fnma(float& acc, float a, float b) {
-    asm volatile("v_fmac_f32_dpp %0, -%1, %2 row_newbcast:%3 row_mask:0xf bank_mask:0xf" : "+v"(acc) : "v"(a), "v"(b), "n"(R));
-}
-template <int R>
-__device__ __forceinline__ float dpp_mul(float a, float b) {
-    float r;
-    asm volatile("s_nop 1\n\tv_mul_f32_dpp %0, %1, %2 row_newbcast:%3 row_mask:0xf bank_mask:0xf" : "=v"(r) : "v"(a), "v"(b), "n"(R));
-    return r;
-}
-
-__device__ __forceinline__ void load_tile(float* T, const float* __restrict__ G, int ld, int tid) {
-#pragma unroll
-    for (int it = 0; it < 4; it++) {
-        const int e = tid + it * 256;
-        const int c = e >> 4, r4 = (e & 15) * 4;
-        const float4 v = *reinterpret_cast<const float4*>(G + (size_t)c * ld + r4);
-        float* t = T + c * PLD + r4;
-#if PLD % 4 == 0
-        *reinterpret_cast<float4*>(t) = v;
-#else
-        t[0] = v.x; t[1] = v.y; t[2] = v.z; t[3] = v.w;
-#endif
-    }
-}
-__device__ __forceinline__ void store_tile(const float* T, float* __restrict__ G, int ld, int tid) {
-#pragma unroll
-    for (int it = 0; it < 4; it++) {
-        const int e = tid + it * 256;
-        const int c = e >> 4, r4 = (e & 15) * 4;
-        const float* t = T + c * PLD + r4;
-#if PLD % 4 == 0
-        *reinterpret_cast<float4*>(G + (size_t)c * ld + r4) = *reinterpret_cast<const float4*>(t);
-#else
-        *reinterpret_cast<float4*>(G + (size_t)c * ld + r4) = make_float4(t[0], t[1], t[2], t[3]);
-#endif
-    }
-}
-__device__ __forceinline__ unsigned long long sign_mask_request(const unsigned long long* p) {
-    unsigned z;
-    asm volatile("v_mov_b32 %0, 0" : "=v"(z));
-    return p[z];
-}
-__device__ __forceinline__ unsigned long long sign_mask_value(unsigned long long v) {
-    const unsigned lo = __builtin_amdgcn_readfirstlane((unsigned)v), hi = __builtin_amdgcn_readfirstlane((unsigned)(v >> 32));
-    return ((unsigned long long)hi << 32) | lo;
-}
-__device__ __forceinline__ void store_tile_signed(const float* T, float* __restrict__ G, int ld, int tid, unsigned long long neg) {
-#pragma unroll
-    for (int it = 0; it < 4; it++) {
-        const int e = tid + it * 256;
-        const int c = e >> 4, r4 = (e & 15) * 4;
-        const float* t = T + c * PLD + r4;
-        const float sg = ((neg >> c) & 1ull) ? -1.f : 1.f;
-        *reinterpret_cast<float4*>(G + (size_t)c * ld + r4) = make_float4(sg * t[0], sg * t[1], sg * t[2], sg * t[3]);
-    }
-}
-__device__ __forceinline__ void store_tile_lower(const float* T, float* __restrict__ G, int ld, int tid) {
-#pragma unroll
-    for (int it = 0; it < 4; it++) {
-        const int e = tid + it * 256;
-        const int c = e >> 4, r4 = (e & 15) * 4;
-        const float* t = T + c * PLD + r4;
-#if PLD % 4 == 0
-        const float4 q = *reinterpret_cast<const float4*>(t);
-        *reinterpret_cast<float4*>(G + (size_t)c * ld + r4) =
-            make_float4(r4 >= c ? q.x : 0.f, r4 + 1 >= c ? q.y : 0.f, r4 + 2 >= c ? q.z : 0.f, r4 + 3 >= c ? q.w : 0.f);
-#else
-        *reinterpret_cast<float4*>(G + (size_t)c * ld + r4) =
-            make_float4(r4 >= c ? t[0] : 0.f, r4 + 1 >= c ? t[1] : 0.f, r4 + 2 >= c ? t[2] : 0.f, r4 + 3 >= c ? t[3] : 0.f);
-#endif
-    }
-}
-template <int C0, int NC, int NT, bool LOWER>
-__device__ __forceinline__ void store_cols(const float* T, float* __restrict__ G, int ld, int t) {
-    static_assert(PLD % 4 == 0, "vector LDS reads");
-#pragma unroll
-    for (int it = 0; it < (NC * 16 + NT - 1) / NT; it++) {
-        const int e = t + it * NT;
-        if ((NC * 16) % NT != 0 && e >= NC * 16) break;
-        const int c = C0 + (e >> 4), r4 = (e & 15) * 4;
-        const float4 q = *reinterpret_cast<const float4*>(T + c * PLD + r4);
-        *reinterpret_cast<float4*>(G + (size_t)c * ld + r4) =
-            LOWER ? make_float4(r4 >= c ? q.x : 0.f, r4 + 1 >= c ? q.y : 0.f, r4 + 2 >= c ? q.z : 0.f, r4 + 3 >= c ? q.w : 0.f) : q;
-    }
-}
-__device__ __forceinline__ void store_inv_blocks(const float* Tinv, float* __restrict__ G, int p0, int t) {
-    const int p = p0 + (t >> 6), c = (t >> 2) & 15, r4 = (t & 3) * 4;
-    const float* s = Tinv + p * 16 * ILD + c * ILD + r4;
-    *reinterpret_cast<float4*>(G + (p0 * 64 + t) * 4) = make_float4(s[0], s[1], s[2], s[3]);
-}
-struct NoIdleWork {
-    template <class PC>
-    __device__ __forceinline__ void operator()(PC, int) const {}
-};
-__device__ __forceinline__ void load_inv(float* Tinv, const float* __restrict__ G, int tid) {
-    const float4 v = *reinterpret_cast<const float4*>(G + tid * 4);
-    const int p = tid >> 6, c = (tid >> 2) & 15, r4 = (tid & 3) * 4;
-    float* t = Tinv + p * 16 * ILD + c * ILD + r4;
-    t[0] = v.x; t[1] = v.y; t[2] = v.z; t[3] = v.w;
-}
-__device__ __forceinline__ void store_inv(const float* Tinv, float* __restrict__ G, int tid) {
-    const int p = tid >> 6, c = (tid >> 2) & 15, r4 = (tid & 3) * 4;
-    const float* t = Tinv + p * 16 * ILD + c * ILD + r4;
-    *reinterpret_cast<float4*>(G + tid * 4) = make_float4(t[0], t[1], t[2], t[3]);
-}
+#include "potrf64.inc"
 
 __device__ __forceinline__ f32x16 mma64(const float* As, int a_si, int a_sq, const float* Bs, int b_sj, int b_sq, int wr, int wc,
                                int lane) {
@@ -172,15 +41,6 @@
     return acc;
 }
 
-__device__ __forceinline__ f32x4 mma16(const float* As, int a_si, int a_sq, const float* Bs, int b_sj, int b_sq, int lane) {
-    f32x4 acc = {0.f, 0.f, 0.f, 0.f};
-    const int li = lane & 15, lk = lane >> 4;
-    const float* ap = As + li * a_si + lk * a_sq;
-    const float* bp = Bs + li * b_sj + lk * b_sq;
-#pragma unroll
-    for (int q = 0; q < 16; q += 4) acc = __builtin_amdgcn_mfma_f32_16x16x4f32(bp[q * b_sq], ap[q * a_sq], acc, 0, 0, 0);
-    return acc;
-}
 
 struct TriOps {
     float binv[4][4];
@@ -327,141 +187,6 @@
 __device__ __forceinline__ void tri_solve_fwd2(float* Tx, float* Ty, const float* Tl, const float* Tinv, int wave, int lane) {
     float* const t[2] = {Tx, Ty};
     tri_solve_fwd_n<2>(t, Tl, Tinv, wave, lane);
-}
-#define POTRF_STAMP(i)                                                         \
-    do {                                                                       \
-        if (stamps && tid == 0) stamps[i] = (long long)__builtin_amdgcn_s_memtime(); \
-    } while (0)
-
-#define POTRF_WSTAMP(i)                                                                               \
-    do {                                                                                              \
-        if (stamps && lane == 0) stamps[16 + wave * 16 + (i)] = (long long)__builtin_amdgcn_s_memtime(); \
-    } while (0)
-
-__device__ __forceinline__ void potrf_tile_update(float* A, int c0, int ti, int tj, int lane) {
-    const int li = lane & 15, lk = lane >> 4;
-    const int rb = c0 + 16 + 16 * ti, cb = c0 + 16 + 16 * tj;
-    const f32x4 u = mma16(A + c0 * PLD + rb, 1, PLD, A + c0 * PLD + cb, 1, PLD, lane);
-    float t[4];
-#pragma unroll
-    for (int g = 0; g < 4; g++) t[g] = A[(cb + 4 * lk + g) * PLD + rb + li];
-#pragma unroll
-    for (int g = 0; g < 4; g++) A[(cb + 4 * lk + g) * PLD + rb + li] = t[g] - u[g];
-}
-
-__device__ __forceinline__ void potrf_inverse16(const float* A, float* Tinv, int b, int lane) {
-    const int o = 16 * b, li = lane & 15;
-    float lrow[16], acc[16], x[16];
-#pragma unroll
-    for (int q = 0; q < 16; q++) lrow[q] = A[(o + q) * PLD + o + li];
-    const float dd = A[(o + li) * PLD + o + li];
-    float dinv_own = __builtin_amdgcn_rcpf(dd);
-    dinv_own = __builtin_fmaf(__builtin_fmaf(-dd, dinv_own, 1.f), dinv_own, dinv_own);
-#pragma unroll
-    for (int r = 0; r < 16; r++) acc[r] = (r == li) ? 1.f : 0.f;
-    static_for<0, 16>([&](auto qc) {
-        constexpr int q = decltype(qc)::value;
-        const float xq = dpp_mul<q>(dinv_own, acc[q]);
-        x[q] = xq;
-        static_for<q + 1, 16>([&](auto rc) {
-            constexpr int r = decltype(rc)::value;
-            dpp_fnma<r>(acc[r], lrow[q], xq);
-        });
-    });
-    if (lane < 16) {
-#pragma unroll
-        for (int r = 0; r < 16; r++) Tinv[b * 16 * ILD + li * ILD + r] = x[r];
-    }
-}
-
-#include "potrf_chain.inc"
-
-template <int FV = EKF_POTRF_FV, class Idle = NoIdleWork, bool RAW_BARRIER = false>
-__device__ __forceinline__ bool potrf64_lds(float* A, float* Tinv, int tid, long long* stamps = nullptr, Idle idle = Idle()) {
-#define POTRF_BAR()                                                                                  \
-    do {                                                                                             \
-        if constexpr (RAW_BARRIER) asm volatile("s_waitcnt lgkmcnt(0)\n\ts_barrier" ::: "memory");   \
-        else __syncthreads();                                                                        \
-    } while (0)
-    const int lane = tid & 63;
-    const int wave = tid >> 6;
-    bool bad = false;
-    POTRF_STAMP(1);
-    static_for<0, 4>([&](auto pc) {
-        constexpr int P = decltype(pc)::value;
-        constexpr int p = P;
-        constexpr int c0 = 16 * p;
-        if (FV >= 10 && wave == 0) {
-            const unsigned lb = static_cast<unsigned>(reinterpret_cast<size_t>(A + c0 * PLD + lane));
-            const bool inv_lane = p >= 1 && lane < 16;
-            const unsigned sb = inv_lane ? static_cast<unsigned>(reinterpret_cast<size_t>(Tinv + p * 16 * ILD + lane * ILD)) : lb;
-            if constexpr (FV == 12) potrf_panel16_chain_ls3<c0>(lb, sb, inv_lane ? 4u : (unsigned)(PLD * 4), (c0 + (lane & 15)) << 2);
-            else if constexpr (FV == 13) potrf_panel16_chain_ls3w<c0>(lb, sb, inv_lane ? 4u : (unsigned)(PLD * 4), (c0 + (lane & 15)) << 2);
-            else potrf_panel16_chain_ls<c0>(lb, sb, inv_lane ? 4u : (unsigned)(PLD * 4), (c0 + (lane & 15)) << 2);
-        } else if (wave == 0) {
-            float a[16];
-#pragma unroll
-            for (int j = 0; j < 16; j++) a[j] = A[(c0 + j) * PLD + lane];
-#pragma unroll
-            for (int j = 0; j < 16; j++) asm volatile("" : "+v"(a[j]));
-            if (stamps && p == 0 && lane == 0) stamps[14] = (long long)__builtin_amdgcn_s_memtime();
-            if constexpr (FV == 8) {
-                potrf_panel16_chain<c0>(a, (c0 + (lane & 15)) << 2);
-            } else {
-                static_for<0, 16>([&](auto kc) {
-                    constexpr int k = decltype(kc)::value;
-                    const float d = lane_bcast(fmaxf(a[k], 1e-20f), c0 + k);
-                    const float inv = __builtin_amdgcn_rsqf(d);
-                    a[k] *= inv;
-                    static_for<k + 1, 16>([&](auto jc) {
-                        constexpr int j = decltype(jc)::value;
-                        a[j] = __builtin_fmaf(-a[k], lane_bcast(a[k], c0 + j), a[j]);
-                    });
-                });
-            }
-            if (stamps && p == 0 && lane == 0) stamps[15] = (long long)__builtin_amdgcn_s_memtime();
-            if (lane >= c0) {
-#pragma unroll
-                for (int j = 0; j < 16; j++) A[(c0 + j) * PLD + lane] = (lane - c0 >= j) ? a[j] : 0.f;
-            }
-            if constexpr (p >= 1) {
-                if (lane < 16) {
-#pragma unroll
-                    for (int j = 0; j < 16; j++) Tinv[p * 16 * ILD + lane * ILD + j] = a[j];
-                }
-            }
-        } else if (p == 0) {
-#pragma unroll
-            for (int q = 0; q < 4; q++) {
-                const int e = (tid - 64) + 192 * q;
-                const int c = 16 + (e >> 4), r = e & 15;
-                A[c * PLD + r] = ((c & 15) == r) ? 1.f : 0.f;
-            }
-        } else if (p == 1) {
-            if (wave == 1) potrf_inverse16(A, Tinv, 0, lane);
-            if (wave == 2) potrf_tile_update(A, 0, 1, 1, lane);
-            if (wave == 3) {
-                potrf_tile_update(A, 0, 2, 1, lane);
-                potrf_tile_update(A, 0, 2, 2, lane);
-            }
-        } else if (p == 2) {
-            if (wave == 1) potrf_tile_update(A, 16, 1, 1, lane);
-        }
-        if (wave != 0) idle(pc, wave);
-        POTRF_WSTAMP(2 * p);
-        POTRF_BAR();
-        POTRF_STAMP(2 + 2 * p);
-        if (p < 3) {
-            if (wave < 3 - p) potrf_tile_update(A, c0, wave, 0, lane);
-            POTRF_WSTAMP(2 * p + 1);
-            POTRF_BAR();
-        }
-        POTRF_STAMP(3 + 2 * p);
-    });
-    POTRF_STAMP(10);
-    bad = __ballot(!(A[lane * PLD + lane] > 2e-10f)) != 0ull;
-    return bad;
-#undef POTRF_BAR
 }
 
 __device__ __attribute__((noinline)) unsigned long long potrf64_signed(float* A, float* Tinv, int tid) {
@@ -922,7 +647,7 @@
 }
 
 #define EKF_PERSIST_FUSED_DYN_LDS (28 * 1024)
-const int* launch_persist_fused(ekfvio_filter* f, const UpdatePlan& p, bool zero_flags) {
+const int* launch_persist_fused(ekfvio_filter* f, const UpdatePlan& p, bool zero_flags, bool pre00) {
     const int m_pad = p.m_pad, n_pad = p.n_pad;
     ProfScope ps(f, PC_CHOL, (double)m_pad * m_pad * m_pad / 3.0 + (double)(n_pad + m_pad / 2) * m_pad * m_pad);
     if (!f->persist_attr_set) {
@@ -932,6 +657,7 @@
     }
     PersistArgs pa = persist_args(f, p, f->Laug, f->ld_aug, f->Km, f->ldp, f->Saug, f->Linv);
     pa.gain = p.gain == GAIN_SWEEP, pa.t2 = p.t2_by_sweep;
+    pa.pre00 = pre00 ? f->pre00_words : nullptr;
     if (zero_flags) (void)hipMemsetAsync(f->sweep_sync, 0, sizeof(int) * persist_flag_words(m_pad, n_pad), f->stream);
     hipLaunchKernelGGL(chol_persist_kernel, dim3(pa.grid.total()), dim3(256), EKF_PERSIST_FUSED_DYN_LDS,
                        f->stream, pa, make_gather_args(f, p));
diff --git a/ekf_vio_amd/csrc/chol_persist.inc b/ekf_vio_amd/csrc/chol_persist.inc
--- a/ekf_vio_amd/csrc/chol_persist.inc
+++ b/ekf_vio_amd/csrc/chol_persist.inc
@@ -36,6 +36,7 @@
     float* T2;
     int ldt;
     int nstate;
+    int* pre00;
 #ifdef EKFVIO_TEST_HOOKS
     int delay_wg;
     int delay_point;
@@ -706,6 +707,21 @@
             unsigned zoff = 0;
             asm volatile("" : "+v"(zoff));
             const int m = ga.m_dev ? ga.m_dev[zoff] : ga.m;
+            int pre_word = 0;
+            float4 pre_l[4], pre_i = make_float4(0.f, 0.f, 0.f, 0.f);
+            unsigned long long pre_s = 0ull;
+            if (a.pre00) {
+                pre_word = a.pre00[zoff];
+#pragma unroll
+                for (int it = 0; it < 4; it++) {
+                    const int e = tid + it * 256;
+                    pre_l[it] = *reinterpret_cast<const float4*>(L + (size_t)(e >> 4) * ldl + (e & 15) * 4);
+                }
+                pre_i = *reinterpret_cast<const float4*>(a.Linv + tid * 4);
+                pre_s = a.Lsign[zoff];
+            }
+            bool pre_hit = false;
+            if (!a.pre00 || !(pre_hit = __builtin_amdgcn_readfirstlane(pre_word) != 0)) {
             {
                 GTile t0;
                 int all_hit = 0;
@@ -759,6 +775,21 @@
                 if (bad0) atomicOr(a.info, 1);
             }
             asm volatile("" ::: "memory");
+            } else {
+#pragma unroll
+                for (int it = 0; it < 4; it++) {
+                    const int e = tid + it * 256;
+                    *reinterpret_cast<float4*>(Lk + (e >> 4) * PLD + (e & 15) * 4) = pre_l[it];
+                }
+                {
+                    float* t = Tinv + (tid >> 6) * 16 * ILD + ((tid >> 2) & 15) * ILD + (tid & 3) * 4;
+                    t[0] = pre_i.x, t[1] = pre_i.y, t[2] = pre_i.z, t[3] = pre_i.w;
+                }
+                neg = sign_mask_value(pre_s);
+                if (tid == 0) atomicAdd(reinterpret_cast<unsigned long long*>(a.pre00 + 2), 1ull);
+                if (a.dbg && tid == 0) a.dbg[890] = 1;
+                __syncthreads();
+            }
             PSTAMP(3);
         } else {
             load_tile(Lk, L, ldl, tid);
diff --git a/ekf_vio_amd/csrc/common.h b/ekf_vio_amd/csrc/common.h
--- a/ekf_vio_amd/csrc/common.h
+++ b/ekf_vio_amd/csrc/common.h
@@ -119,6 +119,7 @@
     float* Km = nullptr;
     float* Wt = nullptr;
     float* Gm = nullptr;
+    int* pre00_words = nullptr;
     int* info = nullptr;
     float gate_chi2 = 0.f;
     float* gate_d2 = nullptr;
@@ -259,9 +260,17 @@
     int count_total = 0;
 };
 BookArgs make_book_args(ekfvio_filter* f, int m, const float* d_z, const float* d_R, const uint8_t* d_pass, const int* d_frame_counter);
+struct Pre00Args {
+    int enabled = 0;
+    float* L = nullptr;
+    int ldl = 0;
+    float* Linv = nullptr;
+    unsigned long long* Lsign = nullptr;
+    int* words = nullptr;
+};
 void launch_linearize(ekfvio_filter* f, float dt, const BookArgs* book = nullptr);
 void launch_build_dense_F(ekfvio_filter* f, float* Fdense);
-void launch_predict(ekfvio_filter* f, float dt, const BookArgs* book = nullptr);
+bool launch_predict(ekfvio_filter* f, float dt, const BookArgs* book = nullptr, const UpdatePlan* next = nullptr);
 struct UpdateInputs {
     int m = 0;
     const float *z = nullptr, *R = nullptr;
@@ -275,6 +284,7 @@
     int publish_seq = 0;
     int (*between)(ekfvio_filter*, int kyp_blocks) = nullptr;
     bool recoverable = true;
+    bool pre00 = false;
 };
 struct UpdateResult {
     bool published = false;
@@ -314,7 +324,7 @@
 }
 int launch_update_gemms_scratch(ekfvio_filter* f, const UpdatePlan& p, int reps);
 const int* launch_chol_sweep(ekfvio_filter* f, const UpdatePlan& p, float* Saug, float* Laug, float* Linv, int ld, bool zero_flags);
-const int* launch_persist_fused(ekfvio_filter* f, const UpdatePlan& p, bool zero_flags);
+const int* launch_persist_fused(ekfvio_filter* f, const UpdatePlan& p, bool zero_flags, bool pre00 = false);
 void launch_joseph_g(ekfvio_filter* f, int m, int m_pad, int n_pad, bool m_on_device, const float* T = nullptr);
 inline float* t2_buffer(ekfvio_filter* f) { return f->Fdense; }
 void launch_gain2_tiles(ekfvio_filter* f, const UpdatePlan& p);
diff --git a/ekf_vio_amd/csrc/ekf_kernels.hip b/ekf_vio_amd/csrc/ekf_kernels.hip
--- a/ekf_vio_amd/csrc/ekf_kernels.hip
+++ b/ekf_vio_amd/csrc/ekf_kernels.hip
@@ -1,4 +1,5 @@
 #include <algorithm>
+#include <type_traits>
 #include <utility>
 
 #include "common.h"
@@ -6,6 +7,8 @@
 namespace {
 
 #include "motion_model.inc"
+#include "potrf64.inc"
+#include "gather_body.inc"
 
 template <int NT, bool EFF = false>
 __device__ __forceinline__ void bookkeeping_body(const BookArgs& a) {
@@ -183,19 +186,207 @@
     return (fabsf(acc) > EKF_FLUSH_THRESH) ? acc : 0.f;
 }
 
+__device__ __forceinline__ float predict_xb_elem(const float* Bf, const float* Df, const float* Pbb, const float* Pfb, int r, int b) {
+    float acc = 0.f;
+#pragma unroll
+    for (int c = 0; c < 9; c++) acc = acc + Bf[c * 3 + r] * Pbb[c * 9 + b];
+#pragma unroll
+    for (int q = 0; q < 3; q++) acc = acc + Df[q * 3 + r] * Pfb[q * 9 + b];
+    return acc;
+}
+__device__ __forceinline__ float predict_xg_elem(const float* Bf, const float* Df, const float* Pbg, const float (&Pfg)[3][3], int r, int s) {
+    float acc = 0.f;
+#pragma unroll
+    for (int c = 0; c < 9; c++) acc = acc + Bf[c * 3 + r] * Pbg[c * 3 + s];
+#pragma unroll
+    for (int q = 0; q < 3; q++) acc = acc + Df[q * 3 + r] * Pfg[q][s];
+    return acc;
+}
+__device__ __forceinline__ float predict_pair_elem(const float* Xb, const float* Bg, const float* Dg, const float (&Xg)[3][3], int r, int s) {
+    float acc = 0.f;
+#pragma unroll
+    for (int c = 0; c < 9; c++) acc = acc + Xb[r * 9 + c] * Bg[c * 3 + s];
+#pragma unroll
+    for (int q = 0; q < 3; q++) acc = acc + Xg[r][q] * Dg[q * 3 + s];
+    return acc;
+}
+
+struct alignas(16) Pre00Lds {
+    float A[PB * PLD];
+    float Tinv[INV_LDS];
+};
+template <bool LIN>
+__device__ __forceinline__ void pre00_body(const Pre00Args& pre, const BookArgs& book, const float* __restrict__ P, int ld, int N,
+                                           const float* __restrict__ FB, const float* __restrict__ FD, float dt, const float* __restrict__ mu,
+                                           float* sm, BaseMotion* s_bm, Pre00Lds& t, long long* dbg) {
+    constexpr int NL = PRE00_LANDMARKS;
+    const int tid = threadIdx.x;
+#define RSTAMP_(slot)                                                                            \
+    do {                                                                                         \
+        if (dbg && tid == 0) dbg[940 + (slot)] = (long long)__builtin_amdgcn_s_memtime();        \
+    } while (0)
+    float* sPbb = sm;
+    float* sPbg = sm + 96;
+    float* sPfb = sPbg + NL * 27;
+    float* sB = sPfb + NL * 27;
+    float* sD = sB + NL * 27;
+    float* sXb = sD + NL * 9;
+    const uint8_t* pass = book.pass;
+    const float* R = book.R;
+    if (book.frame_counter) {
+        const int fi = *book.frame_counter;
+        pass += (size_t)fi * N;
+        R += (size_t)fi * 4 * N;
+    }
+    const bool ok = N >= NL && (tid >= NL || pass[tid] != 0);
+    if (N < NL) {
+        if (tid == 0) pre.words[0] = 0;
+        return;
+    }
+    const float pbb = (tid < 81) ? P[(size_t)(7 + tid % 9) * ld + 7 + tid / 9] : 0.f;
+    float pg[4], pf[4], fb[4] = {0.f, 0.f, 0.f, 0.f}, fd[2] = {0.f, 0.f};
+#pragma unroll
+    for (int it = 0; it < 4; it++) {
+        const int e = min(tid + 256 * it, NL * 27 - 1), l = e / 27, w = e % 27;
+        pg[it] = P[(size_t)(EKF_BASE + 3 * l + w % 3) * ld + 7 + w / 3];
+        pf[it] = P[(size_t)(7 + w % 9) * ld + EKF_BASE + 3 * l + w / 9];
+        if (!LIN) fb[it] = FB[e];
+    }
+    if (!LIN) {
+#pragma unroll
+        for (int it = 0; it < 2; it++) fd[it] = FD[min(tid + 256 * it, NL * 9 - 1)];
+    }
+    const int lf = tid % NL;
+    float Pfg[4][3][3];
+    float4 Rg[4];
+#pragma unroll
+    for (int k = 0; k < 4; k++) {
+        const int lg = tid / NL + 8 * k;
+#pragma unroll
+        for (int sIdx = 0; sIdx < 3; sIdx++) {
+            const float3 c3 = *reinterpret_cast<const float3*>(P + (size_t)(EKF_BASE + 3 * lg + sIdx) * ld + EKF_BASE + 3 * lf);
+            Pfg[k][0][sIdx] = c3.x;
+            Pfg[k][1][sIdx] = c3.y;
+            Pfg[k][2][sIdx] = c3.z;
+        }
+        Rg[k] = *reinterpret_cast<const float4*>(R + 4 * lg);
+    }
+    float lu[2] = {0.f, 0.f}, lv[2] = {0.f, 0.f}, lrho[2] = {1.f, 1.f};
+    if (LIN) {
+#pragma unroll
+        for (int sl = 0; sl < 2; sl++) {
+            const int task = tid + 256 * sl;
+            if (task < NL * 12) {
+                const int lmk = task / 12;
+                lu[sl] = mu[EKF_BASE + 3 * lmk];
+                lv[sl] = mu[EKF_BASE + 3 * lmk + 1];
+                lrho[sl] = mu[EKF_BASE + 3 * lmk + 2];
+            }
+        }
+        if (tid >= 192 && tid < 192 + 19) {
+            float b[EKF_BASE];
+#pragma unroll
+            for (int i = 0; i < EKF_BASE; i++) b[i] = mu[i];
+            s_bm[tid - 192] = lin_base_motion(b, tid - 192, dt);
+        }
+    }
+    if (!__syncthreads_and(ok)) {
+        if (tid == 0) pre.words[0] = 0;
+        return;
+    }
+    RSTAMP_(1);
+    if (tid < 81) sPbb[tid] = pbb;
+#pragma unroll
+    for (int it = 0; it < 4; it++) {
+        const int e = tid + 256 * it;
+        if (e < NL * 27) {
+            sPbg[e] = pg[it];
+            sPfb[e] = pf[it];
+            if (!LIN) sB[e] = fb[it];
+        }
+    }
+    if (!LIN) {
+#pragma unroll
+        for (int it = 0; it < 2; it++)
+            if (tid + 256 * it < NL * 9) sD[tid + 256 * it] = fd[it];
+    }
+    __syncthreads();
+    if (LIN) {
+        const float td = two_delta();
+#pragma unroll
+        for (int sl = 0; sl < 2; sl++) {
+            const int task = tid + 256 * sl;
+            if (task < NL * 12) {
+                const int l = task / 12, e = task % 12;
+                float o[3];
+                lin_column(s_bm, lu[sl], lv[sl], lrho[sl], e, td, o);
+                float* dst = (e < 9) ? (sB + l * 27 + e * 3) : (sD + l * 9 + (e - 9) * 3);
+                dst[0] = o[0];
+                dst[1] = o[1];
+                dst[2] = o[2];
+            }
+        }
+        __syncthreads();
+    }
+    RSTAMP_(2);
+    for (int e = tid; e < NL * 27; e += 256) {
+        const int l = e / 27, r = (e % 27) / 9, b = e % 9;
+        sXb[e] = predict_xb_elem(sB + l * 27, sD + l * 9, sPbb, sPfb + l * 27, r, b);
+    }
+    __syncthreads();
+    RSTAMP_(3);
+#pragma unroll
+    for (int k = 0; k < 4; k++) {
+        const int lg = tid / NL + 8 * k;
+        float Xg[3][3];
+#pragma unroll
+        for (int r = 0; r < 2; r++)
+#pragma unroll
+            for (int q = 0; q < 3; q++) Xg[r][q] = predict_xg_elem(sB + lf * 27, sD + lf * 9, sPbg + lg * 27, Pfg[k], r, q);
+#pragma unroll
+        for (int sIdx = 0; sIdx < 2; sIdx++) {
+            const float rd = sIdx == 0 ? Rg[k].x : Rg[k].w, ro = sIdx == 0 ? Rg[k].y : Rg[k].z;
+#pragma unroll
+            for (int r = 0; r < 2; r++) {
+                const float acc = predict_pair_elem(sXb + lf * 27, sB + lg * 27, sD + lg * 9, Xg, r, sIdx);
+                const float v = predict_finish(acc, EKF_BASE + 3 * lf + r, EKF_BASE + 3 * lg + sIdx, dt);
+                const int c = 2 * lf + r, rr = 2 * lg + sIdx;
+                t.A[c * PLD + rr] = gather_a_elem(v, rr, c, PB, rd, ro);
+            }
+        }
+    }
+    __syncthreads();
+    RSTAMP_(4);
+    const bool bad = potrf64_lds<EKF_POTRF_FV>(t.A, t.Tinv, tid);
+    RSTAMP_(5);
+    if (bad) {
+        if (tid == 0) pre.words[0] = 0;
+        return;
+    }
+    store_tile_lower(t.A, pre.L, pre.ldl, tid);
+    store_inv(t.Tinv, pre.Linv, tid);
+    if (tid == 0) {
+        pre.Lsign[0] = 0ull;
+        pre.words[0] = 1;
+    }
+    RSTAMP_(6);
+#undef RSTAMP_
+}
+
 template <bool LIN>
 __global__ __launch_bounds__(256) void predict_fused_kernel(const float* __restrict__ P, int ld, int N, int n,
                                                             const float* __restrict__ FA, const float* __restrict__ FB,
                                                             const float* __restrict__ FD, float dt,
                                                             float* __restrict__ Pout, int tiles_side, int chunks,
                                                             const float* __restrict__ mu, float* __restrict__ mu_next, BookArgs book,
-                                                            long long* dbg) {
+                                                            Pre00Args pre, long long* dbg) {
     const int tid = threadIdx.x;
     const int ntile = tiles_side * tiles_side;
+    const int bx = (int)blockIdx.x - (pre.enabled ? 1 : 0);
 #define PSTAMP_(slot)                                                                                               \
     do {                                                                                                            \
         if (dbg && tid == 0) {                                                                                      \
-            const int b_ = (int)blockIdx.x;                                                                         \
+            const int b_ = bx;                                                                                      \
             const int w_ = b_ == 0 ? 0 : b_ == 1 ? 1 : b_ == ntile ? 2 : b_ == ntile + 1 ? 3 : b_ == ntile + chunks + 1 ? 4 : -1; \
             if (w_ >= 0) dbg[900 + 8 * w_ + (slot)] = (long long)__builtin_amdgcn_s_memtime();                      \
         }                                                                                                           \
@@ -209,10 +400,15 @@
         bookkeeping_body<256>(book);
         return;
     }
+    if (bx < 0) {
+        __shared__ Pre00Lds s_pre;
+        pre00_body<LIN>(pre, book, P, ld, N, FB, FD, dt, mu, sm, s_bm, s_pre, dbg);
+        return;
+    }
     if (LIN) {
         if (tid < EKF_BASE) s_base[tid] = mu[tid];
     }
-    if ((int)blockIdx.x < ntile) {
+    if (bx < ntile) {
         float* sPbb = sm;
         float* sPbg = sm + 96;
         float* sPfb = sPbg + PT * 27;
@@ -221,7 +417,7 @@
         float* sDf = sBg + PT * 27;
         float* sDg = sDf + PT * 9;
         float* sXb = sDg + PT * 9;
-        const int tI = blockIdx.x / tiles_side, tJ = blockIdx.x % tiles_side;
+        const int tI = bx / tiles_side, tJ = bx % tiles_side;
         const int f0 = tI * PT, g0 = tJ * PT;
         if (tid < 81) sPbb[tid] = P[(size_t)(7 + tid % 9) * ld + 7 + tid / 9];
         float lu[2] = {0.f, 0.f}, lv[2] = {0.f, 0.f}, lrho[2] = {1.f, 1.f};
@@ -316,12 +512,7 @@
         PSTAMP_(2);
         for (int e = tid; e < PT * 27; e += 256) {
             const int l = e / 27, r = (e % 27) / 9, b = e % 9;
-            float acc = 0.f;
-#pragma unroll
-            for (int c = 0; c < 9; c++) acc = acc + sBf[l * 27 + c * 3 + r] * sPbb[c * 9 + b];
-#pragma unroll
-            for (int q = 0; q < 3; q++) acc = acc + sDf[l * 9 + q * 3 + r] * sPfb[l * 27 + q * 9 + b];
-            sXb[e] = acc;
+            sXb[e] = predict_xb_elem(sBf + l * 27, sDf + l * 9, sPbb, sPfb + l * 27, r, b);
         }
         __syncthreads();
         PSTAMP_(3);
@@ -340,24 +531,13 @@
 #pragma unroll
         for (int r = 0; r < 3; r++)
 #pragma unroll
-            for (int sIdx = 0; sIdx < 3; sIdx++) {
-                float acc = 0.f;
-#pragma unroll
-                for (int c = 0; c < 9; c++) acc = acc + sBf[lf * 27 + c * 3 + r] * sPbg[lg * 27 + c * 3 + sIdx];
-#pragma unroll
-                for (int q = 0; q < 3; q++) acc = acc + sDf[lf * 9 + q * 3 + r] * Pfg[q][sIdx];
-                Xg[r][sIdx] = acc;
-            }
+            for (int sIdx = 0; sIdx < 3; sIdx++) Xg[r][sIdx] = predict_xg_elem(sBf + lf * 27, sDf + lf * 9, sPbg + lg * 27, Pfg, r, sIdx);
 #pragma unroll
         for (int sIdx = 0; sIdx < 3; sIdx++) {
             float o3[3];
 #pragma unroll
             for (int r = 0; r < 3; r++) {
-                float acc = 0.f;
-#pragma unroll
-                for (int c = 0; c < 9; c++) acc = acc + sXb[lf * 27 + r * 9 + c] * sBg[lg * 27 + c * 3 + sIdx];
-#pragma unroll
-                for (int q = 0; q < 3; q++) acc = acc + Xg[r][q] * sDg[lg * 9 + q * 3 + sIdx];
+                const float acc = predict_pair_elem(sXb + lf * 27, sBg + lg * 27, sDg + lg * 9, Xg, r, sIdx);
                 const int i = EKF_BASE + 3 * f + r, j = EKF_BASE + 3 * g + sIdx;
                 o3[r] = predict_finish(acc, i, j, dt);
             }
@@ -366,7 +546,7 @@
         PSTAMP_(4);
         return;
     }
-    const int wb = (int)blockIdx.x - ntile;
+    const int wb = bx - ntile;
     float* sA = sm;
     float* sLB = sm + 3072;
     float* sLD = sLB + PC * 27;
@@ -554,8 +734,6 @@
     bookkeeping_body<1024, true>(a);
 }
 
-#include "gather_body.inc"
-
 __global__ __launch_bounds__(256) void gather_kernel(GatherArgs a) {
     __shared__ float tile[64 * 65];
     gather_body(a, blockIdx.x, tile);
@@ -653,7 +831,7 @@
                        Fdense);
 }
 
-void launch_predict(ekfvio_filter* f, float dt, const BookArgs* book) {
+bool launch_predict(ekfvio_filter* f, float dt, const BookArgs* book, const UpdatePlan* next) {
     const int tiles_side = (f->N + PT - 1) / PT;
     const bool pre = f->prelinearized && f->cfg.predict_mode != EKFVIO_PREDICT_DENSE;
     f->prelinearized = false;
@@ -662,6 +840,7 @@
     if (!lin_in_predict && !pre) launch_linearize(f, dt, book);
     const int n = f->n, ld = f->ldp;
     dim3 grid((n + 255) / 256, n);
+    bool carried = false;
     if (f->cfg.predict_mode == EKFVIO_PREDICT_DENSE) {
         launch_build_dense_F(f, f->Fdense);
         const int np = round_up(n, 32);
@@ -678,15 +857,20 @@
         const int chunks = (f->N + PC - 1) / PC;
         BookArgs b;
         if (book && (lin_in_predict || pre)) b = *book;
+        Pre00Args pa;
+        carried = next && pre00_role(f->tune, plan_shape(f), *next, b.enabled != 0, f->gate_chi2 > 0.f);
+        if (carried) pa.enabled = 1, pa.L = f->Laug, pa.ldl = f->ld_aug, pa.Linv = f->Linv, pa.Lsign = f->Lsign, pa.words = f->pre00_words;
+        const dim3 pgrid(ts * ts + 1 + 2 * chunks + (b.enabled ? 1 : 0) + (carried ? 1 : 0));
         if (lin_in_predict)
-            hipLaunchKernelGGL(predict_fused_kernel<true>, dim3(ts * ts + 1 + 2 * chunks + (b.enabled ? 1 : 0)), dim3(256), 0, f->stream,
-                               f->P, ld, f->N, n, f->FA, f->FB, f->FD, dt, f->P2, ts, chunks, f->mu, f->mu_next, b, f->sweep_dbg);
+            hipLaunchKernelGGL(predict_fused_kernel<true>, pgrid, dim3(256), 0, f->stream,
+                               f->P, ld, f->N, n, f->FA, f->FB, f->FD, dt, f->P2, ts, chunks, f->mu, f->mu_next, b, pa, f->sweep_dbg);
         else
-            hipLaunchKernelGGL(predict_fused_kernel<false>, dim3(ts * ts + 1 + 2 * chunks + (b.enabled ? 1 : 0)), dim3(256), 0, f->stream, f->P, ld, f->N, n,
-                               f->FA, f->FB, f->FD, dt, f->P2, ts, chunks, f->mu, f->mu_next, b, f->sweep_dbg);
+            hipLaunchKernelGGL(predict_fused_kernel<false>, pgrid, dim3(256), 0, f->stream, f->P, ld, f->N, n,
+                               f->FA, f->FB, f->FD, dt, f->P2, ts, chunks, f->mu, f->mu_next, b, pa, f->sweep_dbg);
         std::swap(f->P, f->P2);
     }
     std::swap(f->mu, f->mu_next);
+    return carried;
 }
 
 UpdateResult launch_update(ekfvio_filter* f, const UpdateInputs& in) {
@@ -722,7 +906,7 @@
         return out;
     }
     const bool zero_flags = p.persistent() && !p.fused_gather && !f->sweep_flags_clean;
-    const int* abort = p.sweep == SWEEP_PERSIST_FUSED ? launch_persist_fused(f, p, zero_flags)
+    const int* abort = p.sweep == SWEEP_PERSIST_FUSED ? launch_persist_fused(f, p, zero_flags, in.pre00 && in.bookkeeping_done && !gate)
                                                       : launch_chol_sweep(f, p, f->Saug, f->Laug, f->Linv, f->ld_aug, zero_flags);
     if (in.publish_seq) launch_publish_status(f, in.publish_seq), out.published = true;
     GemmEpi e2;
diff --git a/ekf_vio_amd/csrc/plan.h b/ekf_vio_amd/csrc/plan.h
--- a/ekf_vio_amd/csrc/plan.h
+++ b/ekf_vio_amd/csrc/plan.h
@@ -36,6 +36,7 @@
     int lin_overlap = 1;
     int sym_joseph = 1;
     int fuse_linearize = 1;
+    int pre00 = 1;
 };
 
 inline Tuning tuning_from_env() {
@@ -66,6 +67,7 @@
         {"EKFVIO_LIN_OVERLAP", FLAG, &Tuning::lin_overlap, nullptr},
         {"EKFVIO_SYM_JOSEPH", FLAG, &Tuning::sym_joseph, nullptr},
         {"EKFVIO_FUSE_LINEARIZE", FLAG, &Tuning::fuse_linearize, nullptr},
+        {"EKFVIO_PRE00", FLAG, &Tuning::pre00, nullptr},
     };
     Tuning t;
     for (const Entry& k : table) {
@@ -286,4 +288,9 @@
         p.lin_blocks = lin_blocks;
     return p;
 }
-#endif
+
+#define PRE00_LANDMARKS (EKF_TILE / 2)
+inline bool pre00_role(const Tuning& t, const PlanShape& s, const UpdatePlan& next, bool book_in_predict, bool gate) {
+    return t.pre00 && book_in_predict && !gate && next.sweep == SWEEP_PERSIST_FUSED && s.N >= PRE00_LANDMARKS && next.m_pad >= EKF_TILE;
+}
+#endif
diff --git a/ekf_vio_amd/csrc/potrf64.inc b/ekf_vio_amd/csrc/potrf64.inc
--- /dev/null
+++ b/ekf_vio_amd/csrc/potrf64.inc
@@ -0,0 +1,278 @@
+typedef float f32x16 __attribute__((ext_vector_type(16)));
+typedef float f32x4 __attribute__((ext_vector_type(4)));
+
+#define PB 64
+#ifndef PLD
+#define PLD 68
+#endif
+#define ILD 17
+#define INV_LDS (4 * 16 * ILD)
+
+__device__ __forceinline__ float lane_bcast(float v, int src_lane) {
+    return __int_as_float(__builtin_amdgcn_readlane(__float_as_int(v), src_lane));
+}
+__device__ __forceinline__ double lane_bcast_d(double v, int src_lane) {
+    const int lo = __builtin_amdgcn_readlane(__double2loint(v), src_lane);
+    const int hi = __builtin_amdgcn_readlane(__double2hiint(v), src_lane);
+    return __hiloint2double(hi, lo);
+}
+
+template <int B, int E, class F>
+__device__ __forceinline__ void static_for(F&& f) {
+    if constexpr (B < E) {
+        f(std::integral_constant<int, B>{});
+        static_for<B + 1, E>(f);
+    }
+}
+template <int R>
+__device__ __forceinline__ void dpp_fnma(float& acc, float a, float b) {
+    asm volatile("v_fmac_f32_dpp %0, -%1, %2 row_newbcast:%3 row_mask:0xf bank_mask:0xf" : "+v"(acc) : "v"(a), "v"(b), "n"(R));
+}
+template <int R>
+__device__ __forceinline__ float dpp_mul(float a, float b) {
+    float r;
+    asm volatile("s_nop 1\n\tv_mul_f32_dpp %0, %1, %2 row_newbcast:%3 row_mask:0xf bank_mask:0xf" : "=v"(r) : "v"(a), "v"(b), "n"(R));
+    return r;
+}
+
+__device__ __forceinline__ void load_tile(float* T, const float* __restrict__ G, int ld, int tid) {
+#pragma unroll
+    for (int it = 0; it < 4; it++) {
+        const int e = tid + it * 256;
+        const int c = e >> 4, r4 = (e & 15) * 4;
+        const float4 v = *reinterpret_cast<const float4*>(G + (size_t)c * ld + r4);
+        float* t = T + c * PLD + r4;
+#if PLD % 4 == 0
+        *reinterpret_cast<float4*>(t) = v;
+#else
+        t[0] = v.x; t[1] = v.y; t[2] = v.z; t[3] = v.w;
+#endif
+    }
+}
+__device__ __forceinline__ void store_tile(const float* T, float* __restrict__ G, int ld, int tid) {
+#pragma unroll
+    for (int it = 0; it < 4; it++) {
+        const int e = tid + it * 256;
+        const int c = e >> 4, r4 = (e & 15) * 4;
+        const float* t = T + c * PLD + r4;
+#if PLD % 4 == 0
+        *reinterpret_cast<float4*>(G + (size_t)c * ld + r4) = *reinterpret_cast<const float4*>(t);
+#else
+        *reinterpret_cast<float4*>(G + (size_t)c * ld + r4) = make_float4(t[0], t[1], t[2], t[3]);
+#endif
+    }
+}
+__device__ __forceinline__ unsigned long long sign_mask_request(const unsigned long long* p) {
+    unsigned z;
+    asm volatile("v_mov_b32 %0, 0" : "=v"(z));
+    return p[z];
+}
+__device__ __forceinline__ unsigned long long sign_mask_value(unsigned long long v) {
+    const unsigned lo = __builtin_amdgcn_readfirstlane((unsigned)v), hi = __builtin_amdgcn_readfirstlane((unsigned)(v >> 32));
+    return ((unsigned long long)hi << 32) | lo;
+}
+__device__ __forceinline__ void store_tile_signed(const float* T, float* __restrict__ G, int ld, int tid, unsigned long long neg) {
+#pragma unroll
+    for (int it = 0; it < 4; it++) {
+        const int e = tid + it * 256;
+        const int c = e >> 4, r4 = (e & 15) * 4;
+        const float* t = T + c * PLD + r4;
+        const float sg = ((neg >> c) & 1ull) ? -1.f : 1.f;
+        *reinterpret_cast<float4*>(G + (size_t)c * ld + r4) = make_float4(sg * t[0], sg * t[1], sg * t[2], sg * t[3]);
+    }
+}
+__device__ __forceinline__ void store_tile_lower(const float* T, float* __restrict__ G, int ld, int tid) {
+#pragma unroll
+    for (int it = 0; it < 4; it++) {
+        const int e = tid + it * 256;
+        const int c = e >> 4, r4 = (e & 15) * 4;
+        const float* t = T + c * PLD + r4;
+#if PLD % 4 == 0
+        const float4 q = *reinterpret_cast<const float4*>(t);
+        *reinterpret_cast<float4*>(G + (size_t)c * ld + r4) =
+            make_float4(r4 >= c ? q.x : 0.f, r4 + 1 >= c ? q.y : 0.f, r4 + 2 >= c ? q.z : 0.f, r4 + 3 >= c ? q.w : 0.f);
+#else
+        *reinterpret_cast<float4*>(G + (size_t)c * ld + r4) =
+            make_float4(r4 >= c ? t[0] : 0.f, r4 + 1 >= c ? t[1] : 0.f, r4 + 2 >= c ? t[2] : 0.f, r4 + 3 >= c ? t[3] : 0.f);
+#endif
+    }
+}
+template <int C0, int NC, int NT, bool LOWER>
+__device__ __forceinline__ void store_cols(const float* T, float* __restrict__ G, int ld, int t) {
+    static_assert(PLD % 4 == 0, "vector LDS reads");
+#pragma unroll
+    for (int it = 0; it < (NC * 16 + NT - 1) / NT; it++) {
+        const int e = t + it * NT;
+        if ((NC * 16) % NT != 0 && e >= NC * 16) break;
+        const int c = C0 + (e >> 4), r4 = (e & 15) * 4;
+        const float4 q = *reinterpret_cast<const float4*>(T + c * PLD + r4);
+        *reinterpret_cast<float4*>(G + (size_t)c * ld + r4) =
+            LOWER ? make_float4(r4 >= c ? q.x : 0.f, r4 + 1 >= c ? q.y : 0.f, r4 + 2 >= c ? q.z : 0.f, r4 + 3 >= c ? q.w : 0.f) : q;
+    }
+}
+__device__ __forceinline__ void store_inv_blocks(const float* Tinv, float* __restrict__ G, int p0, int t) {
+    const int p = p0 + (t >> 6), c = (t >> 2) & 15, r4 = (t & 3) * 4;
+    const float* s = Tinv + p * 16 * ILD + c * ILD + r4;
+    *reinterpret_cast<float4*>(G + (p0 * 64 + t) * 4) = make_float4(s[0], s[1], s[2], s[3]);
+}
+struct NoIdleWork {
+    template <class PC>
+    __device__ __forceinline__ void operator()(PC, int) const {}
+};
+__device__ __forceinline__ void load_inv(float* Tinv, const float* __restrict__ G, int tid) {
+    const float4 v = *reinterpret_cast<const float4*>(G + tid * 4);
+    const int p = tid >> 6, c = (tid >> 2) & 15, r4 = (tid & 3) * 4;
+    float* t = Tinv + p * 16 * ILD + c * ILD + r4;
+    t[0] = v.x; t[1] = v.y; t[2] = v.z; t[3] = v.w;
+}
+__device__ __forceinline__ void store_inv(const float* Tinv, float* __restrict__ G, int tid) {
+    const int p = tid >> 6, c = (tid >> 2) & 15, r4 = (tid & 3) * 4;
+    const float* t = Tinv + p * 16 * ILD + c * ILD + r4;
+    *reinterpret_cast<float4*>(G + tid * 4) = make_float4(t[0], t[1], t[2], t[3]);
+}
+
+__device__ __forceinline__ f32x4 mma16(const float* As, int a_si, int a_sq, const float* Bs, int b_sj, int b_sq, int lane) {
+    f32x4 acc = {0.f, 0.f, 0.f, 0.f};
+    const int li = lane & 15, lk = lane >> 4;
+    const float* ap = As + li * a_si + lk * a_sq;
+    const float* bp = Bs + li * b_sj + lk * b_sq;
+#pragma unroll
+    for (int q = 0; q < 16; q += 4) acc = __builtin_amdgcn_mfma_f32_16x16x4f32(bp[q * b_sq], ap[q * a_sq], acc, 0, 0, 0);
+    return acc;
+}
+
+#define POTRF_STAMP(i)                                                         \
+    do {                                                                       \
+        if (stamps && tid == 0) stamps[i] = (long long)__builtin_amdgcn_s_memtime(); \
+    } while (0)
+
+#define POTRF_WSTAMP(i)                                                                               \
+    do {                                                                                              \
+        if (stamps && lane == 0) stamps[16 + wave * 16 + (i)] = (long long)__builtin_amdgcn_s_memtime(); \
+    } while (0)
+
+__device__ __forceinline__ void potrf_tile_update(float* A, int c0, int ti, int tj, int lane) {
+    const int li = lane & 15, lk = lane >> 4;
+    const int rb = c0 + 16 + 16 * ti, cb = c0 + 16 + 16 * tj;
+    const f32x4 u = mma16(A + c0 * PLD + rb, 1, PLD, A + c0 * PLD + cb, 1, PLD, lane);
+    float t[4];
+#pragma unroll
+    for (int g = 0; g < 4; g++) t[g] = A[(cb + 4 * lk + g) * PLD + rb + li];
+#pragma unroll
+    for (int g = 0; g < 4; g++) A[(cb + 4 * lk + g) * PLD + rb + li] = t[g] - u[g];
+}
+
+__device__ __forceinline__ void potrf_inverse16(const float* A, float* Tinv, int b, int lane) {
+    const int o = 16 * b, li = lane & 15;
+    float lrow[16], acc[16], x[16];
+#pragma unroll
+    for (int q = 0; q < 16; q++) lrow[q] = A[(o + q) * PLD + o + li];
+    const float dd = A[(o + li) * PLD + o + li];
+    float dinv_own = __builtin_amdgcn_rcpf(dd);
+    dinv_own = __builtin_fmaf(__builtin_fmaf(-dd, dinv_own, 1.f), dinv_own, dinv_own);
+#pragma unroll
+    for (int r = 0; r < 16; r++) acc[r] = (r == li) ? 1.f : 0.f;
+    static_for<0, 16>([&](auto qc) {
+        constexpr int q = decltype(qc)::value;
+        const float xq = dpp_mul<q>(dinv_own, acc[q]);
+        x[q] = xq;
+        static_for<q + 1, 16>([&](auto rc) {
+            constexpr int r = decltype(rc)::value;
+            dpp_fnma<r>(acc[r], lrow[q], xq);
+        });
+    });
+    if (lane < 16) {
+#pragma unroll
+        for (int r = 0; r < 16; r++) Tinv[b * 16 * ILD + li * ILD + r] = x[r];
+    }
+}
+
+#include "potrf_chain.inc"
+
+template <int FV = EKF_POTRF_FV, class Idle = NoIdleWork, bool RAW_BARRIER = false>
+__device__ __forceinline__ bool potrf64_lds(float* A, float* Tinv, int tid, long long* stamps = nullptr, Idle idle = Idle()) {
+#define POTRF_BAR()                                                                                  \
+    do {                                                                                             \
+        if constexpr (RAW_BARRIER) asm volatile("s_waitcnt lgkmcnt(0)\n\ts_barrier" ::: "memory");   \
+        else __syncthreads();                                                                        \
+    } while (0)
+    const int lane = tid & 63;
+    const int wave = tid >> 6;
+    bool bad = false;
+    POTRF_STAMP(1);
+    static_for<0, 4>([&](auto pc) {
+        constexpr int P = decltype(pc)::value;
+        constexpr int p = P;
+        constexpr int c0 = 16 * p;
+        if (FV >= 10 && wave == 0) {
+            const unsigned lb = static_cast<unsigned>(reinterpret_cast<size_t>(A + c0 * PLD + lane));
+            const bool inv_lane = p >= 1 && lane < 16;
+            const unsigned sb = inv_lane ? static_cast<unsigned>(reinterpret_cast<size_t>(Tinv + p * 16 * ILD + lane * ILD)) : lb;
+            if constexpr (FV == 12) potrf_panel16_chain_ls3<c0>(lb, sb, inv_lane ? 4u : (unsigned)(PLD * 4), (c0 + (lane & 15)) << 2);
+            else if constexpr (FV == 13) potrf_panel16_chain_ls3w<c0>(lb, sb, inv_lane ? 4u : (unsigned)(PLD * 4), (c0 + (lane & 15)) << 2);
+            else potrf_panel16_chain_ls<c0>(lb, sb, inv_lane ? 4u : (unsigned)(PLD * 4), (c0 + (lane & 15)) << 2);
+        } else if (wave == 0) {
+            float a[16];
+#pragma unroll
+            for (int j = 0; j < 16; j++) a[j] = A[(c0 + j) * PLD + lane];
+#pragma unroll
+            for (int j = 0; j < 16; j++) asm volatile("" : "+v"(a[j]));
+            if (stamps && p == 0 && lane == 0) stamps[14] = (long long)__builtin_amdgcn_s_memtime();
+            if constexpr (FV == 8) {
+                potrf_panel16_chain<c0>(a, (c0 + (lane & 15)) << 2);
+            } else {
+                static_for<0, 16>([&](auto kc) {
+                    constexpr int k = decltype(kc)::value;
+                    const float d = lane_bcast(fmaxf(a[k], 1e-20f), c0 + k);
+                    const float inv = __builtin_amdgcn_rsqf(d);
+                    a[k] *= inv;
+                    static_for<k + 1, 16>([&](auto jc) {
+                        constexpr int j = decltype(jc)::value;
+                        a[j] = __builtin_fmaf(-a[k], lane_bcast(a[k], c0 + j), a[j]);
+                    });
+                });
+            }
+            if (stamps && p == 0 && lane == 0) stamps[15] = (long long)__builtin_amdgcn_s_memtime();
+            if (lane >= c0) {
+#pragma unroll
+                for (int j = 0; j < 16; j++) A[(c0 + j) * PLD + lane] = (lane - c0 >= j) ? a[j] : 0.f;
+            }
+            if constexpr (p >= 1) {
+                if (lane < 16) {
+#pragma unroll
+                    for (int j = 0; j < 16; j++) Tinv[p * 16 * ILD + lane * ILD + j] = a[j];
+                }
+            }
+        } else if (p == 0) {
+#pragma unroll
+            for (int q = 0; q < 4; q++) {
+                const int e = (tid - 64) + 192 * q;
+                const int c = 16 + (e >> 4), r = e & 15;
+                A[c * PLD + r] = ((c & 15) == r) ? 1.f : 0.f;
+            }
+        } else if (p == 1) {
+            if (wave == 1) potrf_inverse16(A, Tinv, 0, lane);
+            if (wave == 2) potrf_tile_update(A, 0, 1, 1, lane);
+            if (wave == 3) {
+                potrf_tile_update(A, 0, 2, 1, lane);
+                potrf_tile_update(A, 0, 2, 2, lane);
+            }
+        } else if (p == 2) {
+            if (wave == 1) potrf_tile_update(A, 16, 1, 1, lane);
+        }
+        if (wave != 0) idle(pc, wave);
+        POTRF_WSTAMP(2 * p);
+        POTRF_BAR();
+        POTRF_STAMP(2 + 2 * p);
+        if (p < 3) {
+            if (wave < 3 - p) potrf_tile_update(A, c0, wave, 0, lane);
+            POTRF_WSTAMP(2 * p + 1);
+            POTRF_BAR();
+        }
+        POTRF_STAMP(3 + 2 * p);
+    });
+    POTRF_STAMP(10);
+    bad = __ballot(!(A[lane * PLD + lane] > 2e-10f)) != 0ull;
+    return bad;
+#undef POTRF_BAR
+}
diff --git a/ekf_vio_amd/filter.py b/ekf_vio_amd/filter.py
--- a/ekf_vio_amd/filter.py
+++ b/ekf_vio_amd/filter.py
@@ -254,8 +254,10 @@
     def counters(self):
         c = (C.c_int64 * 8)()
         self._chk(self.lib.ekfvio_get_counters(self.h, c))
+        p = C.c_int64(0)
+        self._chk(self.lib.ekfvio_get_pre00_updates(self.h, C.byref(p)))
         return dict(persistent=int(c[0]), schur=int(c[1]), recoveries=int(c[2]), mode=int(c[3]), early_output_frames=int(c[4]), t2_updates=int(c[5]),
-                    graph_steps=int(c[6]), prelinearized_steps=int(c[7]))
+                    graph_steps=int(c[6]), prelinearized_steps=int(c[7]), pre00_updates=int(p.value))
 
     def _need_hooks(self):
         if not self.hooks:
diff --git a/include/ekfvio.h b/include/ekfvio.h
--- a/include/ekfvio.h
+++ b/include/ekfvio.h
@@ -138,6 +138,7 @@
 EKFVIO_API int ekfvio_profile_update_gemms(ekfvio_filter* f, int32_t reps, double* avg_launch_us, double* flops_per_launch);
 
 EKFVIO_API int ekfvio_get_counters(ekfvio_filter* f, int64_t counters[8]);
+EKFVIO_API int ekfvio_get_pre00_updates(ekfvio_filter* f, int64_t* updates);
 
 #ifdef __cplusplus
 }
diff --git a/include/ekfvio_test_hooks.h b/include/ekfvio_test_hooks.h
--- a/include/ekfvio_test_hooks.h
+++ b/include/ekfvio_test_hooks.h
@@ -20,6 +20,8 @@
                                float* L_out, float* X_out, int32_t* info);
 EKFVIO_API int ekfvio_test_plan(int32_t num_cus, int32_t max_features, int32_t N, int32_t m, int32_t m_on_device, int32_t sole_handle,
                                 int32_t latched_off, int32_t dense_predict, float next_dt, int32_t plan[12]);
+EKFVIO_API int ekfvio_test_pre00_plan(int32_t num_cus, int32_t max_features, int32_t N, int32_t m, int32_t m_on_device, int32_t sole_handle,
+                                      int32_t latched_off, int32_t dense_predict, int32_t book_in_predict, int32_t gate, int32_t* carried);
 EKFVIO_API int ekfvio_test_persist_grid(int32_t num_cus, int32_t max_features, int32_t N, int32_t m, int32_t m_on_device, int32_t sole_handle,
                                         int32_t latched_off, int32_t dense_predict, float next_dt, int32_t* roles, int32_t max_blocks,
                                         int32_t out[10]);
```

Result: slower. 10800 (-2.4%).
